# ViTAE-Transformer/SAMRS

Measured on AMD Instinct MI355X. Metric: images/sec (1024^2, vit_h, 32 boxes/img) SAM box->mask, higher is better.
Workload: dtype f16

## Files before the change

include/samrs_hip.h:

```cpp
#ifndef SAMRS_HIP_H
#define SAMRS_HIP_H

#include <stdint.h>

#ifdef __cplusplus
extern "C" {
#endif

#define SAMRS_ABI_VERSION 5

enum samrs_status {
    SAMRS_OK = 0,
    SAMRS_ERR_NOT_SET = -1,
    SAMRS_ERR_BAD_SHAPE = -2,
    SAMRS_ERR_BAD_ARG = -3,
    SAMRS_ERR_HIP = -4,
    SAMRS_ERR_BAD_WEIGHTS = -5,
    SAMRS_ERR_CAPACITY = -6,
    SAMRS_ERR_PRECISION = -7,
    SAMRS_ERR_RANGE = -8
};

enum samrs_precision {
    SAMRS_PREC_BF16 = 0,
    SAMRS_PREC_F16 = 1
};

typedef struct samrs_config {
    int32_t embed_dim;
    int32_t depth;
    int32_t num_heads;
    int32_t n_global;
    int32_t global_attn_indexes[8];
    int32_t img_size;
    int32_t patch_size;
    int32_t window_size;
    int32_t out_chans;
    int32_t max_images;
    int32_t max_prompts;
    int32_t max_points;
    int32_t precision;
} samrs_config;

typedef struct samrs_engine samrs_engine_t;

samrs_engine_t* samrs_create(const samrs_config* cfg, int device, char* err, int err_len);
void samrs_destroy(samrs_engine_t* e);
const char* samrs_last_error(const samrs_engine_t* e);
int samrs_abi_version(void);

int samrs_load_weight(samrs_engine_t* e, const char* name, const float* host_data,
                      const int64_t* shape, int ndim);
int samrs_finalize_weights(samrs_engine_t* e, void* stream);

int samrs_set_images(samrs_engine_t* e, const uint8_t* images, int n_images, int in_h, int in_w,
                     int slot0, void* stream);
int samrs_set_images_ragged(samrs_engine_t* e, const uint8_t* const* images, const int* in_h,
                            const int* in_w, int n_images, int slot0, void* stream);
int samrs_get_embedding(samrs_engine_t* e, int slot, float* out_chw, void* stream);
int samrs_set_embedding(samrs_engine_t* e, int slot, const float* emb_chw, void* stream);
int samrs_reset_image(samrs_engine_t* e, int slot);
int samrs_get_slot_info(const samrs_engine_t* e, int slot, int32_t* is_set, int32_t* split, int32_t* split_depth);

int samrs_predict(samrs_engine_t* e, int slot, int n_prompts,
                  const float* boxes, const float* point_coords, const int32_t* point_labels,
                  int n_points, const float* mask_input, int multimask, int return_logits,
                  int in_h, int in_w, int orig_h, int orig_w,
                  void* masks_out, float* iou_out, float* lowres_out, void* stream);

int samrs_predict_multi(samrs_engine_t* e, int n_images, const int* slots, const int* prompt_offsets,
                        const float* boxes, const float* point_coords, const int32_t* point_labels, int n_points,
                        const float* mask_input, int multimask, int return_logits,
                        const int* in_hw, const int* orig_hw, void* const* masks_out, float* iou_out, float* lowres_out,
                        void* stream);

int samrs_paint(samrs_engine_t* e, const uint8_t* masks, const int32_t* labels, int n,
                int orig_h, int orig_w, uint8_t* seg_mask, int64_t* areas_out,
                int64_t* class_pixels, int64_t* class_instances, int n_classes, void* stream);

int samrs_select_best(samrs_engine_t* e, const uint8_t* masks, const float* iou, int n, int n_sel, int h, int w,
                      uint8_t* best_out, float* quality_out, int64_t* areas_out, void* stream);

int samrs_gt_match(samrs_engine_t* e, const uint8_t* masks, int n, int h, int w, const uint8_t* label_rgb,
                   const uint8_t* colors, int64_t* inter_out, int64_t* gt_area_out, uint8_t* gt_masks_out, void* stream);

int samrs_rle_encode(samrs_engine_t* e, const uint8_t* masks, int n, int h, int w, uint8_t* out, int64_t out_capacity,
                     int64_t* cursor, int64_t* table, void* stream);

int samrs_scene_claim(samrs_engine_t* e, const uint8_t* masks, const int32_t* ranks, const int32_t* labels, int n, int h, int w,
                      int x0, int y0, int H, int W, int32_t* order, int64_t* areas_out,
                      int64_t* class_pixels, int64_t* class_instances, int n_classes, void* stream);
int samrs_scene_resolve(samrs_engine_t* e, const int32_t* order, const int32_t* labels_by_rank, int n_ranks, int H, int W,
                        uint8_t* seg, void* stream);
int samrs_rle_encode_placed(samrs_engine_t* e, const uint8_t* masks, int n, int h, int w, int x0, int y0, int H, int W,
                            uint8_t* out, int64_t out_capacity, int64_t* cursor, int64_t* table, void* stream);

enum samrs_region_mode { SAMRS_REGION_HOLES = 1, SAMRS_REGION_ISLANDS = 2, SAMRS_REGION_BOTH = 3 };
int samrs_clean_masks(samrs_engine_t* e, uint8_t* masks, int n, int h, int w, int min_area, int mode,
                      int64_t* areas_out, int64_t* changed_out, void* stream);

int samrs_png_encode_labels(samrs_engine_t* e, const uint8_t* maps, int n, int h, int w, const uint8_t* lut, uint8_t* out,
                            int64_t out_capacity, int64_t* cursor, int64_t* table, void* stream);

int samrs_resample_pass_u8(const uint8_t* in, uint8_t* out, const int32_t* bounds, const int32_t* coef,
                           int ksize, int in_len, int out_len, int other, int horizontal, void* stream);

int samrs_set_option(samrs_engine_t* e, const char* name, int value);
int samrs_get_option(const samrs_engine_t* e, const char* name, int* value);

int samrs_audit_site_count(const samrs_engine_t* e, int* n_sites);
int samrs_audit_site_name(const samrs_engine_t* e, int site, char* name, int name_len, int* columns);
int samrs_audit_read_profile(samrs_engine_t* e, int64_t* rows, int reset);
int samrs_audit_read_columns(samrs_engine_t* e, int site, double* sumsq, float* max_abs, int64_t* n_rows);

int samrs_rbox_mask_prompt(const int32_t* pts, int n, int n_vertices, int h, int w, int th, int tw,
                           int img_size, int out_size, float* out, void* stream);
enum samrs_fill_rule { SAMRS_FILL_CV2_LE_451 = 0, SAMRS_FILL_CV2_GE_452 = 1 };
int samrs_rbox_mask_prompt_rule(const int32_t* pts, int n, int n_vertices, int h, int w, int th, int tw,
                                int img_size, int out_size, int fill_rule, float* out, void* stream);


#ifdef __cplusplus
}
#endif
#endif
```

include/samrs_hip_internal.h:

```cpp
#ifndef SAMRS_HIP_INTERNAL_H
#define SAMRS_HIP_INTERNAL_H

#include "samrs_hip.h"

#ifdef __cplusplus
extern "C" {
#endif

int samrs_debug_encoder_prefix(samrs_engine_t* e, const uint8_t* images, int n_images, int in_h,
                               int in_w, int n_blocks, float* x_out, void* stream);

int samrs_debug_outlier_columns(samrs_engine_t* e, int block, int gemm, int32_t* out32);

void samrs_debug_set_gemm_variant(int variant);
void samrs_debug_set_gemm_skew(int xcd_units, int cu_units);
int samrs_debug_has_experiments(void);

int samrs_debug_copy_buffer(samrs_engine_t* e, const char* name, void* dst, size_t bytes, void* stream);

int samrs_debug_time_dominant_kernel(samrs_engine_t* e, int enable);
int samrs_debug_dominant_kernel_time(samrs_engine_t* e, float* avg_ms, int* launches, int* M, int* N, int* K);

int samrs_k_gemm(int prec, const void* A_et, const void* B_et, void* C, const float* bias,
                 const float* add2d, int add2d_period, int M, int N, int K,
                 int out_f32, int gelu, int accumulate, void* stream);
int samrs_k_gemm_f32(const float* A, int lda, const float* W, const float* bias, float* C, int ldc,
                     int M, int N, int K, int relu, int accumulate, void* stream);
int samrs_k_gemm_stats(int prec, const void* A_et, const void* B_et, float* C, const float* bias, void* xh_et, float* stats,
                       int M, int N, int K, void* stream);
int samrs_k_ln_rowstat(const float* stats, float* rowstat, int rows, float eps, void* stream);
int samrs_k_gemm_fold(int prec, const void* xh_et, const void* Wf_et, void* C_et, const float* bias_f, const float* cvec,
                      const float* rowstat, int M, int N, int K, int gelu, void* stream);
int samrs_k_ln_fold_weight(int prec, const float* W, const float* gamma, const float* beta, const float* bias, void* Wf_et,
                           float* cvec, float* bias_f, int N, int K, void* stream);
int samrs_k_rowstats_convert(int prec, const float* X, void* xh_et, float* stats, int rows, int D, void* stream);
int samrs_k_convert(int prec, const float* in, void* out_et, int64_t n, void* stream);
int samrs_k_layernorm(int prec, const float* X, const float* gamma, const float* beta, float eps,
                      void* out_et, float* out_f32, int rows_out, int D, int window_mode,
                      int n_images, int grid, int window, void* stream);
int samrs_k_window_attention(int prec, const void* qkv_et, const float* qkv_bias, const float* rel_h,
                             const float* rel_w, void* out_et, int n_images, int grid, int window,
                             int heads, int head_dim, void* stream);
int samrs_k_global_attention(int prec, const void* qkv_et, const float* rel_h, const float* rel_w,
                             void* out_et, int n_images, int grid, int heads, int head_dim,
                             void* stream);
int samrs_k_neck_im2col(const void* in_et, void* A_et, int n_images, int grid, int C, void* stream);
int samrs_k_postprocess(const float* lowres, int n_masks, int in_h, int in_w, int orig_h,
                        int orig_w, int img_size, int return_logits, void* out, void* stream);
int samrs_k_gemm_gln(int prec, const void* A_et, const void* B_et, void* C_et, const float* bias,
                     const float* gamma_beta, int M, int N, int K, const void* A_lo_et, const void* B_lo_et, void* stream);
int samrs_k_gemm_split3(int prec, const void* A_et, const void* A_lo_et, const void* B_et, const void* B_lo_et, void* C,
                        const float* bias, int M, int N, int K, int out_f32, int accumulate, int split_from_n, void* stream);
int samrs_k_upscale2_masks(int prec, const void* u1, const void* w_et, const void* w_lo_et, const float* bias,
                           const float* hyper, float* low, int n, int grid, int n_mask_tokens,
                           int sel0, int n_sel, void* stream);
int samrs_k_upscaler_fused(int prec, const void* keys_et, const void* keys_lo_et, const void* w1_et, const void* w1_lo_et,
                           const float* b1, const float* ln, const void* w2_et, const void* w2_lo_et, const float* b2,
                           const float* hyper, float* low, int n, int grid, int n_mask_tokens, int sel0, int n_sel, void* stream);
int samrs_k_prompt_tokens(const float* boxes, const float* point_coords, const int32_t* point_labels, int n_prompts, int n_points,
                          float img_size, const float* gauss, const float* point_emb, const float* not_a_point, const float* iou_token,
                          const float* mask_tokens, float* tokens, float* tokens2, int T, void* stream);
int samrs_k_dense_pe(const float* gauss, float* pe, int grid, void* stream);
int samrs_k_mask_embed(const float* w0, const float* b0, const float* ln1w, const float* ln1b, const float* w3, const float* b3,
                       const float* ln4w, const float* ln4b, const float* w6, const float* b6, const float* mask_in, float* dense,
                       int n, int grid, void* stream);
int samrs_k_fill_slot_table(const int32_t* start_host, const int32_t* slot_host, int n_runs, int32_t* out, void* stream);
int samrs_k_make_keys(int prec, const float* emb, const float* dense, const float* vec, float* out_f32, void* out_et, int n_batches,
                      int tokens, int C, const int32_t* slot_of, void* stream);
int samrs_k_token_self_attn(const float* q, const float* k, const float* v, float* o, int n, int T, int C, int heads, void* stream);
int64_t samrs_k_t2i_workspace_floats(int n, int T);
int samrs_k_t2i_attention(int prec, const float* qp, const void* kp_et, const void* vp_et, int ld, int64_t bstride, float* out,
                          float* workspace, int n, int T, int tokens, int Ci, int heads, const int32_t* slot_of, void* stream);
int samrs_k_i2t_attention(int prec, const void* qi_et, int ld, int64_t bstride, const float* kt, const float* vt, void* out_et, int n,
                          int T, int tokens, int Ci, int heads, void* stream);
int samrs_k_i2t_fused(int prec, const void* qi_et, int ld, int64_t q_bstride, const float* kt, const float* vt, const void* w_et,
                      const void* w_lo_et, const float* bias, const float* resid, int64_t r_bstride, const float* gamma,
                      const float* beta, float eps, float* outF, void* outE, void* outE_lo, int n, int T, int tokens, int Ci, int C,
                      const int32_t* slot_of, void* stream);
int samrs_k_group_ln_gelu(int prec, const float* in, const float* gamma, const float* beta, float eps, void* out_et, int64_t rows,
                          int groups, int gsize, void* stream);
int samrs_k_mask_product(int prec, const void* up2_et, const float* hyper, float* low, int n, int grid, int n_mask_tokens, int sel0,
                         int n_sel, void* stream);
int samrs_k_attention_mx(int prec, int global, const void* qkv_et, const float* qkv_bias, const float* rel_h, const float* rel_w,
                         void* out_et, void* out_lo_et, int n_images, int grid, int heads, int head_dim, void* q_hi, void* q_lo,
                         void* s_hi, void* s_lo, void* stream);
int64_t samrs_k_mx_scale_bytes(int rows, int Kp, int is_b);
int samrs_k_layernorm_mx(int prec, const float* X, const float* gamma, const float* beta, float eps, void* out_et, int rows, int D,
                         void* q_hi, void* q_lo, void* s_hi, void* s_lo, void* stream);
int samrs_k_mx4_pack(int prec, const float* x, const void* hi_in, const void* lo_in, void* out_hi, void* q_hi, void* q_lo, void* s_hi,
                     void* s_lo, int rows, int K, int G, int GP, int is_b, void* stream);
int samrs_k_gemm_mx(int prec, const void* A, const void* B, void* C, const float* bias, int M, int N, int K, int Kp, const void* a4_lo,
                    const void* a4_hi, const void* sa_lo, const void* sa_hi, const void* b4_hi, const void* b4_lo, const void* sb_hi,
                    const void* sb_lo, int out_f32, int accumulate, int split_from_n, void* stream);
int samrs_k_gemm_mx_gelu_mxout(int prec, const void* A, const void* B, void* C_et, const float* bias, int M, int N, int K, int Kp,
                               const void* a4_lo, const void* a4_hi, const void* sa_lo, const void* sa_hi, const void* b4_hi, const void* b4_lo,
                               const void* sb_hi, const void* sb_lo, int gelu, void* o4_hi, void* o4_lo, void* so_hi, void* so_lo, void* stream);
int samrs_k_convert_split(int prec, const float* in, void* out_hi_et, void* out_lo_et, int64_t n, void* stream);
int samrs_k_range_profile(int prec, const void* x_et, long n, int cols, int ld, int64_t* row48, void* stream);
int samrs_k_column_stats(int prec, const void* x_et, int M, int K, int ld, float* partials, double* sumsq, uint32_t* maxbits, void* stream);
int samrs_k_audit_rows_per_partial(void);
int samrs_k_region_labels(const uint8_t* masks, int n, int h, int w, int complement, int32_t* labels_out, void* stream);

#ifdef __cplusplus
}
#endif
#endif
```

samrs_amd/csrc/decoder_kernels.hip:

```cpp
#include "common.h"
#include "kernels.h"

namespace {

constexpr float TWO_PI = 6.283185307179586f;

__device__ __forceinline__ float pe_channel(const float* __restrict__ gauss, float cx01, float cy01, int ch, int half) {
    const int f = ch < half ? ch : ch - half;
    const float vx = 2.0f * cx01 - 1.0f, vy = 2.0f * cy01 - 1.0f;
    const float a = TWO_PI * (vx * gauss[f] + vy * gauss[half + f]);
    return ch < half ? sinf(a) : cosf(a);
}

__global__ void prompt_tokens_kernel(PromptParams p, float* __restrict__ tokens, float* __restrict__ tokens2, int T, int C) {
    const int j = blockIdx.x, b = blockIdx.y, ch = threadIdx.x;
    const int half = C / 2;
    const bool has_pts = p.point_coords != nullptr;
    const bool has_box = p.boxes != nullptr;
    const int npt = has_pts ? p.n_points + (has_box ? 0 : 1) : 0;
    float v;
    if (j == 0) {
        v = p.iou_token[ch];
    } else if (j < 5) {
        v = p.mask_tokens[(j - 1) * C + ch];
    } else if (j < 5 + npt) {
        const int k = j - 5;
        int label = -1;
        float x = 0.f, y = 0.f;
        if (k < p.n_points) {
            label = p.point_labels[b * p.n_points + k];
            x = p.point_coords[(b * p.n_points + k) * 2 + 0] + 0.5f;
            y = p.point_coords[(b * p.n_points + k) * 2 + 1] + 0.5f;
        }
        if (label == -1) {
            v = p.not_a_point[ch];
        } else {
            v = pe_channel(p.gauss, x / p.img_size, y / p.img_size, ch, half);
            if (label == 0) v += p.point_emb[0][ch];
            else if (label == 1) v += p.point_emb[1][ch];
        }
    } else {
        const int corner = j - 5 - npt;
        const float x = p.boxes[b * 4 + 2 * corner + 0] + 0.5f;
        const float y = p.boxes[b * 4 + 2 * corner + 1] + 0.5f;
        v = pe_channel(p.gauss, x / p.img_size, y / p.img_size, ch, half) + p.point_emb[2 + corner][ch];
    }
    tokens[((size_t)b * T + j) * C + ch] = v;
    if (tokens2) tokens2[((size_t)b * T + j) * C + ch] = v;
}

__global__ void dense_pe_kernel(const float* __restrict__ gauss, float* __restrict__ pe, int g, int C) {
    const int t = blockIdx.x, ch = threadIdx.x;
    const int y = t / g, x = t % g;
    pe[(size_t)t * C + ch] = pe_channel(gauss, ((float)x + 0.5f) / (float)g, ((float)y + 0.5f) / (float)g, ch, C / 2);
}

__global__ __launch_bounds__(256) void mask_embed_kernel(MaskEmbedParams p, const float* __restrict__ mask_in,
                                                         float* __restrict__ dense, int grid) {
    __shared__ float act2[16][16];
    const int t = threadIdx.x;
    const int b = blockIdx.y;
    const int tok0 = blockIdx.x * 16;
    {
        const int tl = t >> 4, c2 = t & 15;
        const int tok = tok0 + tl;
        const int ty = tok / grid, tx = tok % grid;
        const int S = 4 * grid;
        const float* in = mask_in + (size_t)b * S * S + (size_t)(4 * ty) * S + 4 * tx;
        float out2 = p.b3[c2];
#pragma unroll
        for (int sy = 0; sy < 2; ++sy)
#pragma unroll
            for (int sx = 0; sx < 2; ++sx) {
                float a[4];
                float mean = 0.f;
#pragma unroll
                for (int c = 0; c < 4; ++c) {
                    float s = p.b0[c];
#pragma unroll
                    for (int ky = 0; ky < 2; ++ky)
#pragma unroll
                        for (int kx = 0; kx < 2; ++kx)
// ... 154 lines not shown
        const int key_ = (k0_) + 4 * u_ + kq;                                                    \
        dk_[u_] = dv_[u_] = make_uint4(0u, 0u, 0u, 0u);                                          \
        if (key_ < kend) {                                                                       \
            dk_[u_] = *reinterpret_cast<const uint4*>(kb + (size_t)key_ * ld);                   \
            dv_[u_] = *reinterpret_cast<const uint4*>(vb + (size_t)key_ * ld);                   \
        }                                                                                        \
    }
    T2I_LOAD(kk, vv, kbeg)
    for (int k0 = kbeg; k0 < kend; k0 += 4 * U) {
        T2I_LOAD(kn, vn, k0 + 4 * U)
#pragma unroll
        for (int u = 0; u < U; ++u) {
            const bool valid = k0 + 4 * u + kq < kend;
            const uint32_t kw[4] = {kk[u].x, kk[u].y, kk[u].z, kk[u].w};
            const uint32_t vw[4] = {vv[u].x, vv[u].y, vv[u].z, vv[u].w};
            float kf[8], vf[8];
#pragma unroll
            for (int c = 0; c < 4; ++c) {
                kf[2 * c] = ET<PREC>::to_float((uint16_t)(kw[c] & 0xffffu));
                kf[2 * c + 1] = ET<PREC>::to_float((uint16_t)(kw[c] >> 16));
                vf[2 * c] = ET<PREC>::to_float((uint16_t)(vw[c] & 0xffffu));
                vf[2 * c + 1] = ET<PREC>::to_float((uint16_t)(vw[c] >> 16));
            }
#pragma unroll
            for (int t = 0; t < T2I_TG; ++t) {
                float sc = 0.f;
#pragma unroll
                for (int c = 0; c < 8; ++c) sc += q[t][c] * kf[c];
                sc += __builtin_bit_cast(float, __builtin_amdgcn_update_dpp(0, __builtin_bit_cast(int, sc), 0xB1, 0xF, 0xF, true));
                sc = valid ? sc : T2I_NEG;
                const float mn = fmaxf(m[t], sc);
                const float corr = __builtin_amdgcn_exp2f(m[t] - mn);
                const float pj = valid ? __builtin_amdgcn_exp2f(sc - mn) : 0.f;
                l[t] = l[t] * corr + pj;
#pragma unroll
                for (int c = 0; c < 8; ++c) acc[t][c] = acc[t][c] * corr + pj * vf[c];
                m[t] = mn;
            }
        }
#pragma unroll
        for (int u = 0; u < U; ++u) { kk[u] = kn[u]; vv[u] = vn[u]; }
    }
#undef T2I_LOAD
#pragma unroll
    for (int off = 16; off <= 32; off <<= 1) {
#pragma unroll
        for (int t = 0; t < T2I_TG; ++t) {
            const float mo = __shfl_xor(m[t], off, 64), lo = __shfl_xor(l[t], off, 64);
            const float mn = fmaxf(m[t], mo);
            const float fs = __builtin_amdgcn_exp2f(m[t] - mn), fo = __builtin_amdgcn_exp2f(mo - mn);
            l[t] = l[t] * fs + lo * fo;
#pragma unroll
            for (int c = 0; c < 8; ++c) acc[t][c] = acc[t][c] * fs + __shfl_xor(acc[t][c], off, 64) * fo;
            m[t] = mn;
        }
    }
    if (lane < 16) {
#pragma unroll
        for (int t = 0; t < T2I_TG; ++t) {
            float* r = sm[wave][t][ch];
            r[0] = m[t]; r[1] = l[t];
#pragma unroll
            for (int c = 0; c < 8; ++c) r[2 + c] = acc[t][c];
        }
    }
    __syncthreads();
    if (threadIdx.x < T2I_TG * 16) {
        const int t = threadIdx.x >> 4, c16 = threadIdx.x & 15;
        float mm = sm[0][t][c16][0];
#pragma unroll
        for (int w = 1; w < 4; ++w) mm = fmaxf(mm, sm[w][t][c16][0]);
        float ll = 0.f, a[8] = {0.f, 0.f, 0.f, 0.f, 0.f, 0.f, 0.f, 0.f};
#pragma unroll
        for (int w = 0; w < 4; ++w) {
            const float f = __builtin_amdgcn_exp2f(sm[w][t][c16][0] - mm);
            ll += sm[w][t][c16][1] * f;
#pragma unroll
            for (int c = 0; c < 8; ++c) a[c] += sm[w][t][c16][2 + c] * f;
        }
        float* r = part + ((((size_t)b * gridDim.z + blockIdx.z) * gridDim.x + split) * (T2I_TG * 16) + threadIdx.x) * T2I_REC;
        r[0] = mm; r[1] = ll;
#pragma unroll
        for (int c = 0; c < 8; ++c) r[2 + c] = a[c];
    }
}

__global__ __launch_bounds__(T2I_TG * 16) void t2i_merge_kernel(const float* __restrict__ part, float* __restrict__ o,
                                                                int splits, int T, int Ci) {
    const int b = blockIdx.x, tg = blockIdx.y;
    const int t = tg * T2I_TG + (threadIdx.x >> 4), ch = threadIdx.x & 15;
    if (t >= T) return;
    const float* base = part + (((size_t)b * gridDim.y + tg) * splits * (T2I_TG * 16) + threadIdx.x) * T2I_REC;
    const size_t sstride = (size_t)(T2I_TG * 16) * T2I_REC;
    float mm = T2I_NEG;
    for (int s = 0; s < splits; ++s) mm = fmaxf(mm, base[s * sstride]);
    float ll = 0.f, a[8] = {0.f, 0.f, 0.f, 0.f, 0.f, 0.f, 0.f, 0.f};
    for (int s = 0; s < splits; ++s) {
        const float* r = base + s * sstride;
        const float f = __builtin_amdgcn_exp2f(r[0] - mm);
        ll += r[1] * f;
#pragma unroll
        for (int c = 0; c < 8; ++c) a[c] += r[2 + c] * f;
    }
    const float inv = 1.0f / ll;
    float* orow = o + ((size_t)b * T + t) * Ci + ch * 8;
#pragma unroll
    for (int c = 0; c < 8; ++c) orow[c] = a[c] * inv;
}

constexpr int I2T_HS = 20;
template <int PREC>
__global__ __launch_bounds__(256) void i2t_attention_kernel(const uint16_t* __restrict__ qi, int ld, long bstride,
                                                            const float* __restrict__ kt, const float* __restrict__ vt,
                                                            uint16_t* __restrict__ out, int T, int tokens, int Ci) {
    constexpr int HD = 16;
    extern __shared__ float sm[];
    const int heads = Ci / HD;
    const int RS = heads * I2T_HS;
    float* sk = sm;
    float* sv = sm + T * RS;
    const int b = blockIdx.y;
    for (int i = threadIdx.x; i < T * Ci; i += 256) {
        const int j = i / Ci, c = i % Ci;
        sk[j * RS + (c / HD) * I2T_HS + c % HD] = kt[(size_t)b * T * Ci + i];
        sv[j * RS + (c / HD) * I2T_HS + c % HD] = vt[(size_t)b * T * Ci + i];
    }
    __syncthreads();
    const int tok = blockIdx.x * (256 / heads) + threadIdx.x / heads;
    const int h = threadIdx.x % heads;
    if (tok >= tokens) return;
    const uint16_t* qrow = qi + ((size_t)b * bstride + tok) * ld + h * HD;
    const uint4 q0 = *reinterpret_cast<const uint4*>(qrow);
    const uint4 q1 = *reinterpret_cast<const uint4*>(qrow + 8);
    const uint32_t qw[8] = {q0.x, q0.y, q0.z, q0.w, q1.x, q1.y, q1.z, q1.w};
    float qf[HD];
#pragma unroll
    for (int c = 0; c < 8; ++c) {
        qf[2 * c] = ET<PREC>::to_float((uint16_t)(qw[c] & 0xffffu)) * 0.25f;
        qf[2 * c + 1] = ET<PREC>::to_float((uint16_t)(qw[c] >> 16)) * 0.25f;
    }
    float m = -INFINITY, l = 0.f, acc[HD];
#pragma unroll
    for (int c = 0; c < HD; ++c) acc[c] = 0.f;
    for (int j = 0; j < T; ++j) {
        float kr[HD], vr[HD];
#pragma unroll
        for (int c4 = 0; c4 < HD / 4; ++c4) {
            const float4 k4 = *reinterpret_cast<const float4*>(sk + j * RS + h * I2T_HS + 4 * c4);
            const float4 v4 = *reinterpret_cast<const float4*>(sv + j * RS + h * I2T_HS + 4 * c4);
            kr[4 * c4] = k4.x; kr[4 * c4 + 1] = k4.y; kr[4 * c4 + 2] = k4.z; kr[4 * c4 + 3] = k4.w;
            vr[4 * c4] = v4.x; vr[4 * c4 + 1] = v4.y; vr[4 * c4 + 2] = v4.z; vr[4 * c4 + 3] = v4.w;
        }
        float s = 0.f;
#pragma unroll
        for (int c = 0; c < HD; ++c) s += qf[c] * kr[c];
        const float mn = fmaxf(m, s);
        const float corr = __expf(m - mn), pj = __expf(s - mn);
        l = l * corr + pj;
#pragma unroll
        for (int c = 0; c < HD; ++c) acc[c] = acc[c] * corr + pj * vr[c];
        m = mn;
    }
    const float inv = 1.0f / l;
    uint4 o0, o1;
    o0.x = pack2<PREC>(acc[0] * inv, acc[1] * inv);   o0.y = pack2<PREC>(acc[2] * inv, acc[3] * inv);
    o0.z = pack2<PREC>(acc[4] * inv, acc[5] * inv);   o0.w = pack2<PREC>(acc[6] * inv, acc[7] * inv);
// ... 294 lines not shown
    for (int g = 0; g < U2_GROUPS_PER_WAVE; ++g) {
        uint4 c0 = a0, c1 = a1, l0 = make_uint4(0u, 0u, 0u, 0u), l1 = l0;
        if constexpr (SPLIT) {
            split2_pack<PREC>(f[0].x, f[0].y, c0.x, l0.x); split2_pack<PREC>(f[0].z, f[0].w, c0.y, l0.y);
            split2_pack<PREC>(f[1].x, f[1].y, c0.z, l0.z); split2_pack<PREC>(f[1].z, f[1].w, c0.w, l0.w);
            split2_pack<PREC>(f[2].x, f[2].y, c1.x, l1.x); split2_pack<PREC>(f[2].z, f[2].w, c1.y, l1.y);
            split2_pack<PREC>(f[3].x, f[3].y, c1.z, l1.z); split2_pack<PREC>(f[3].z, f[3].w, c1.w, l1.w);
        }
        if (g + 1 < U2_GROUPS_PER_WAVE) {
            if constexpr (SPLIT) {
                const float* nb = fbase + (size_t)(g + 1) * 16 * 64;
                f[0] = *reinterpret_cast<const float4*>(nb); f[1] = *reinterpret_cast<const float4*>(nb + 4);
                f[2] = *reinterpret_cast<const float4*>(nb + 32); f[3] = *reinterpret_cast<const float4*>(nb + 36);
            } else {
                a0 = *reinterpret_cast<const uint4*>(abase + (size_t)(g + 1) * 16 * 64);
                a1 = *reinterpret_cast<const uint4*>(abase + (size_t)(g + 1) * 16 * 64 + 32);
            }
        }
        float part[NSEL][4];
#pragma unroll
        for (int c = 0; c < NSEL; ++c)
#pragma unroll
            for (int q = 0; q < 4; ++q) part[c][q] = 0.f;
#pragma unroll
        for (int i = 0; i < 8; ++i) {
            f32x4_t acc = {0.f, 0.f, 0.f, 0.f};
            if constexpr (SPLIT) {
                acc = ET<PREC>::mfma16(wf[i][0], l0, acc);
                acc = ET<PREC>::mfma16(wf[i][1], l1, acc);
                acc = ET<PREC>::mfma16(wl[i][0], c0, acc);
                acc = ET<PREC>::mfma16(wl[i][1], c1, acc);
            }
            acc = ET<PREC>::mfma16(wf[i][0], c0, acc);
            acc = ET<PREC>::mfma16(wf[i][1], c1, acc);
            const float2_t g01 = gelu_erf2(float2_t{acc[0] + bv[i][0], acc[1] + bv[i][1]});
            const float2_t g23 = gelu_erf2(float2_t{acc[2] + bv[i][2], acc[3] + bv[i][3]});
#pragma unroll
            for (int c = 0; c < NSEL; ++c) {
                const float* h = hy[c] + (i & 1) * 4;
                part[c][i >> 1] += h[0] * g01.x + h[1] * g01.y + h[2] * g23.x + h[3] * g23.y;
            }
        }
        const int row = row0 + g * 16 + fr;
        const int t = row >> 2, s1 = row & 3;
        const int y = t / grid, x = t % grid;
        const int Y = 4 * y + 2 * (s1 >> 1) + (fq >> 1), X = 4 * x + 2 * (s1 & 1) + (fq & 1);
#pragma unroll
        for (int c = 0; c < NSEL; ++c) {
            float mine = 0.f;
#pragma unroll
            for (int q = 0; q < 4; ++q) {
                float v = part[c][q];
                v += __shfl_xor(v, 16, 64);
                v += __shfl_xor(v, 32, 64);
                mine = (q == fq) ? v : mine;
            }
            low[(((size_t)b * NSEL + c) * S + Y) * S + X] = mine;
        }
    }
}

struct Lin {
    int i0, i1;
    float w0, w1;
};
__device__ __forceinline__ Lin lin_coord(int dst, float scale, int in_size) {
    float src = scale * ((float)dst + 0.5f) - 0.5f;
    src = src < 0.f ? 0.f : src;
    Lin r;
    r.i0 = (int)src;
    r.i0 = r.i0 < in_size - 1 ? r.i0 : in_size - 1;
    r.i1 = r.i0 + (r.i0 < in_size - 1 ? 1 : 0);
    r.w1 = src - (float)r.i0;
    r.w0 = 1.0f - r.w1;
    return r;
}
__device__ __forceinline__ float stage1(const float* __restrict__ low, int LS, float s1, int Y1, int X1) {
    const Lin ly = lin_coord(Y1, s1, LS), lx = lin_coord(X1, s1, LS);
    const float* r0 = low + (size_t)ly.i0 * LS;
    const float* r1 = low + (size_t)ly.i1 * LS;
    return ly.w0 * (lx.w0 * r0[lx.i0] + lx.w1 * r0[lx.i1]) + ly.w1 * (lx.w0 * r1[lx.i0] + lx.w1 * r1[lx.i1]);
}

__global__ __launch_bounds__(256) void postprocess_kernel(const float* __restrict__ low_all, int LS, int in_h, int in_w,
                                                          int H, int W, int img_size, int return_logits,
                                                          void* __restrict__ out) {
    const int W4 = (W + 3) / 4;
    const long t = (long)blockIdx.x * 256 + threadIdx.x;
    if (t >= (long)W4 * H) return;
    const int Y = (int)(t / W4), X0 = (int)(t % W4) * 4;
    const int mi = blockIdx.y;
    const float* low = low_all + (size_t)mi * LS * LS;
    const float s1 = (float)LS / (float)img_size;
    const bool identity = (H == in_h) && (W == in_w);
    float v[4];
    if (identity && 4 * LS == img_size && X0 + 3 < W) {
        const Lin ly = lin_coord(Y, s1, LS);
        const float* r0 = low + (size_t)ly.i0 * LS;
        const float* r1 = low + (size_t)ly.i1 * LS;
        const Lin la = lin_coord(X0, s1, LS), lb = lin_coord(X0 + 1, s1, LS), lc = lin_coord(X0 + 2, s1, LS), ld = lin_coord(X0 + 3, s1, LS);
        const float a00 = r0[la.i0], a01 = r0[la.i1], a10 = r1[la.i0], a11 = r1[la.i1];
        const float c00 = r0[lc.i0], c01 = r0[lc.i1], c10 = r1[lc.i0], c11 = r1[lc.i1];
        v[0] = ly.w0 * (la.w0 * a00 + la.w1 * a01) + ly.w1 * (la.w0 * a10 + la.w1 * a11);
        v[1] = ly.w0 * (lb.w0 * a00 + lb.w1 * a01) + ly.w1 * (lb.w0 * a10 + lb.w1 * a11);
        v[2] = ly.w0 * (lc.w0 * c00 + lc.w1 * c01) + ly.w1 * (lc.w0 * c10 + lc.w1 * c11);
        v[3] = ly.w0 * (ld.w0 * c00 + ld.w1 * c01) + ly.w1 * (ld.w0 * c10 + ld.w1 * c11);
    } else if (identity) {
#pragma unroll
        for (int e = 0; e < 4; ++e) v[e] = (X0 + e < W) ? stage1(low, LS, s1, Y, X0 + e) : 0.f;
    } else {
        const float sy = (float)in_h / (float)H, sx = (float)in_w / (float)W;
        const Lin ly = lin_coord(Y, sy, in_h);
#pragma unroll
        for (int e = 0; e < 4; ++e) {
            if (X0 + e < W) {
                const Lin lx = lin_coord(X0 + e, sx, in_w);
                const float a = lx.w0 * stage1(low, LS, s1, ly.i0, lx.i0) + lx.w1 * stage1(low, LS, s1, ly.i0, lx.i1);
                const float b = lx.w0 * stage1(low, LS, s1, ly.i1, lx.i0) + lx.w1 * stage1(low, LS, s1, ly.i1, lx.i1);
                v[e] = ly.w0 * a + ly.w1 * b;
            } else {
                v[e] = 0.f;
            }
        }
    }
    const size_t obase = ((size_t)mi * H + Y) * W + X0;
    if (return_logits) {
        float* o = reinterpret_cast<float*>(out) + obase;
        for (int e = 0; e < 4 && X0 + e < W; ++e) o[e] = v[e];
    } else {
        uint8_t* o = reinterpret_cast<uint8_t*>(out) + obase;
        if ((W & 3) == 0) {
            const uint32_t pk = (v[0] > 0.f ? 1u : 0u) | (v[1] > 0.f ? 1u << 8 : 0u) | (v[2] > 0.f ? 1u << 16 : 0u) |
                                (v[3] > 0.f ? 1u << 24 : 0u);
            *reinterpret_cast<uint32_t*>(o) = pk;
        } else {
            for (int e = 0; e < 4 && X0 + e < W; ++e) o[e] = v[e] > 0.f ? 1 : 0;
        }
    }
}

__global__ void paint_kernel(const uint8_t* __restrict__ masks, const int32_t* __restrict__ labels, int n, long hw,
                             uint8_t* __restrict__ seg) {
    const long p = (long)blockIdx.x * blockDim.x + threadIdx.x;
    if (p >= hw) return;
    for (int j = n - 1; j >= 0; --j) {
        if (masks[(size_t)j * hw + p]) {
            seg[p] = (uint8_t)labels[j];
            return;
        }
    }
}
__global__ void area_kernel(const uint8_t* __restrict__ masks, long hw, unsigned long long* __restrict__ areas) {
    const int j = blockIdx.y;
    const uint8_t* m = masks + (size_t)j * hw;
    unsigned int cnt = 0;
    for (long p = (long)blockIdx.x * blockDim.x + threadIdx.x; p < hw; p += (long)gridDim.x * blockDim.x) cnt += m[p] ? 1u : 0u;
    float c = (float)cnt;
    c = wave_sum(c);
    if ((threadIdx.x & 63) == 0 && c > 0.f) atomicAdd(&areas[j], (unsigned long long)c);
}
constexpr int PA_CHUNK = 64;
__device__ __forceinline__ uint32_t nonzero_bytes(uint32_t w) {
    return (((w & 0x7F7F7F7Fu) + 0x7F7F7F7Fu) | w) & 0x80808080u;
}
__global__ __launch_bounds__(256) void paint_area_kernel(const uint8_t* __restrict__ masks, const int32_t* __restrict__ labels,
                                                         int n, long hw, uint8_t* __restrict__ seg,
                                                         unsigned long long* __restrict__ areas) {
    __shared__ unsigned int cnt_s[PA_CHUNK];
    const long p0 = ((long)blockIdx.x * 256 + threadIdx.x) * 16;
    const bool in = p0 < hw;
    uint32_t done[4] = {0u, 0u, 0u, 0u}, res[4] = {0u, 0u, 0u, 0u};
    for (int jhi = n; jhi > 0; jhi -= PA_CHUNK) {
        const int jlo = jhi > PA_CHUNK ? jhi - PA_CHUNK : 0;
        if (threadIdx.x < PA_CHUNK) cnt_s[threadIdx.x] = 0u;
        __syncthreads();
        for (int j = jhi - 1; j >= jlo; --j) {
            unsigned int cnt = 0;
            if (in) {
                const uint4 m = *reinterpret_cast<const uint4*>(masks + (size_t)j * hw + p0);
                const uint32_t w[4] = {m.x, m.y, m.z, m.w};
                const uint32_t lab = (uint32_t)(uint8_t)labels[j] * 0x01010101u;
#pragma unroll
                for (int k = 0; k < 4; ++k) {
                    const uint32_t t = nonzero_bytes(w[k]);
                    cnt += __popc(t);
                    const uint32_t mm = (t >> 7) * 0xFFu, fresh = mm & ~done[k];
                    res[k] = (res[k] & ~fresh) | (fresh & lab);
                    done[k] |= mm;
                }
            }
            float c = wave_sum((float)cnt);
            if ((threadIdx.x & 63) == 0 && c > 0.f) atomicAdd(&cnt_s[j - jlo], (unsigned int)c);
        }
        __syncthreads();
        if (threadIdx.x < jhi - jlo && cnt_s[threadIdx.x]) atomicAdd(&areas[jlo + threadIdx.x], (unsigned long long)cnt_s[threadIdx.x]);
        __syncthreads();
    }
    if (in && (done[0] | done[1] | done[2] | done[3])) {
        uint4* sp = reinterpret_cast<uint4*>(seg + p0);
        uint4 o = *sp;
        o.x = (o.x & ~done[0]) | res[0]; o.y = (o.y & ~done[1]) | res[1];
        o.z = (o.z & ~done[2]) | res[2]; o.w = (o.w & ~done[3]) | res[3];
        *sp = o;
    }
}
__global__ __launch_bounds__(256) void select_best_kernel(const uint8_t* __restrict__ masks, const float* __restrict__ iou, int nsel,
                                                          long hw, uint8_t* __restrict__ out, float* __restrict__ quality,
                                                          unsigned long long* __restrict__ areas) {
    const int j = blockIdx.y;
    int best = 0;
    float bq = iou[(size_t)j * nsel];
    for (int c = 1; c < nsel; ++c) {
        const float q = iou[(size_t)j * nsel + c];
        if (q > bq) { bq = q; best = c; }
    }
    if (blockIdx.x == 0 && threadIdx.x == 0) quality[j] = bq;
    const uint8_t* src = masks + ((size_t)j * nsel + best) * hw;
    uint8_t* dst = out + (size_t)j * hw;
    unsigned int cnt = 0;
    const bool vec = (hw % 16 == 0) && ((((uintptr_t)src) | ((uintptr_t)dst)) & 15) == 0;
    if (vec) {
        const long n16 = hw / 16;
        for (long i = (long)blockIdx.x * 256 + threadIdx.x; i < n16; i += (long)gridDim.x * 256) {
            const uint4 m = reinterpret_cast<const uint4*>(src)[i];
            reinterpret_cast<uint4*>(dst)[i] = m;
            cnt += __popc(nonzero_bytes(m.x)) + __popc(nonzero_bytes(m.y)) + __popc(nonzero_bytes(m.z)) + __popc(nonzero_bytes(m.w));
        }
    } else {
        for (long i = (long)blockIdx.x * 256 + threadIdx.x; i < hw; i += (long)gridDim.x * 256) {
            const uint8_t m = src[i];
            dst[i] = m;
            cnt += m ? 1u : 0u;
        }
    }
    const float c = wave_sum((float)cnt);
    if ((threadIdx.x & 63) == 0 && c > 0.f) atomicAdd(&areas[j], (unsigned long long)c);
}

constexpr int GM_CHUNK = 64;
__global__ __launch_bounds__(256) void gt_match_kernel(const uint8_t* __restrict__ masks, int n, long hw,
                                                       const uint8_t* __restrict__ label_rgb, const uint8_t* __restrict__ colors,
                                                       unsigned long long* __restrict__ inter, unsigned long long* __restrict__ gt_area,
                                                       uint8_t* __restrict__ gt_masks) {
    __shared__ unsigned int cnt_s[GM_CHUNK];
    const long p0 = ((long)blockIdx.x * 256 + threadIdx.x) * 16;
    const bool full = p0 + 16 <= hw;
    uint32_t key[16];
    if (full && (((uintptr_t)(label_rgb + p0 * 3)) & 15) == 0) {
        const uint4* lp = reinterpret_cast<const uint4*>(label_rgb + p0 * 3);
        const uint4 a = lp[0], b = lp[1], c = lp[2];
        const uint32_t wv[12] = {a.x, a.y, a.z, a.w, b.x, b.y, b.z, b.w, c.x, c.y, c.z, c.w};
#pragma unroll
        for (int k = 0; k < 16; ++k) {
            uint32_t v = 0;
#pragma unroll
            for (int ch = 0; ch < 3; ++ch) {
                const int byte = 3 * k + ch;
                v |= ((wv[byte >> 2] >> (8 * (byte & 3))) & 0xFFu) << (8 * ch);
            }
            key[k] = v;
        }
    } else {
#pragma unroll
        for (int k = 0; k < 16; ++k) {
            const long p = p0 + k;
            key[k] = p < hw ? (uint32_t)label_rgb[p * 3] | ((uint32_t)label_rgb[p * 3 + 1] << 8) | ((uint32_t)label_rgb[p * 3 + 2] << 16)
                            : 0xFFFFFFFFu;
        }
    }
    for (int jlo = 0; jlo < n; jlo += GM_CHUNK) {
        const int jhi = jlo + GM_CHUNK < n ? jlo + GM_CHUNK : n;
        if (threadIdx.x < GM_CHUNK) cnt_s[threadIdx.x] = 0u;
        __syncthreads();
        for (int j = jlo; j < jhi; ++j) {
            const uint32_t want = (uint32_t)colors[3 * j] | ((uint32_t)colors[3 * j + 1] << 8) | ((uint32_t)colors[3 * j + 2] << 16);
// ... 170 lines not shown
            if (Y >= th || X >= tw) { pv[a][c] = -1000.0; continue; }
            const RTap ay = rbox_tap(Y, h, th), ax = rbox_tap(X, w, tw);
            const double m00 = rbox_inside(P, ax.i0, ay.i0) ? 1000.0 : -1000.0;
            const double m01 = rbox_inside(P, ax.i1, ay.i0) ? 1000.0 : -1000.0;
            const double m10 = rbox_inside(P, ax.i0, ay.i1) ? 1000.0 : -1000.0;
            const double m11 = rbox_inside(P, ax.i1, ay.i1) ? 1000.0 : -1000.0;
            const double r0 = m00 * (double)ax.w0 + m01 * (double)ax.w1;
            const double r1 = m10 * (double)ax.w0 + m11 * (double)ax.w1;
            pv[a][c] = r0 * (double)ay.w0 + r1 * (double)ay.w1;
        }
    const double t0 = pv[0][0] * (double)bx.w0 + pv[0][1] * (double)bx.w1;
    const double t1 = pv[1][0] * (double)bx.w0 + pv[1][1] * (double)bx.w1;
    out[(size_t)b * out_size * out_size + pix] = (float)(t0 * (double)by.w0 + t1 * (double)by.w1);
}

}

hipError_t launch_resample_pass(const uint8_t* in, uint8_t* out, const int32_t* bounds, const int32_t* coef, int ksize,
                                int in_len, int out_len, int other, int horizontal, hipStream_t s) {
    const long total = (long)out_len * other * 3;
    resample_pass_kernel<<<(int)((total + 255) / 256), 256, 0, s>>>(in, out, bounds, coef, ksize, in_len, out_len, other, horizontal);
    return hipGetLastError();
}

hipError_t launch_prompt_tokens(const PromptParams& p, float* tokens, float* tokens2, int T, hipStream_t s) {
    dim3 g(T, p.n_prompts), b(256);
    prompt_tokens_kernel<<<g, b, 0, s>>>(p, tokens, tokens2, T, 256);
    return hipGetLastError();
}
hipError_t launch_dense_pe(const float* gauss, float* pe, int grid, hipStream_t s) {
    dense_pe_kernel<<<grid * grid, 256, 0, s>>>(gauss, pe, grid, 256);
    return hipGetLastError();
}
hipError_t launch_mask_embed(const MaskEmbedParams& p, const float* mask_in, float* dense, int n, int grid, hipStream_t s) {
    dim3 g(grid * grid / 16, n);
    mask_embed_kernel<<<g, 256, 0, s>>>(p, mask_in, dense, grid);
    return hipGetLastError();
}
hipError_t launch_fill_slot_table(const int* start, const int* slot, int n_runs, int* out, hipStream_t s) {
    for (int k0 = 0; k0 < n_runs; k0 += SLOT_RUNS_MAX) {
        SlotRuns r{};
        const int nr = n_runs - k0 < SLOT_RUNS_MAX ? n_runs - k0 : SLOT_RUNS_MAX;
        for (int k = 0; k < nr; ++k) { r.start[k] = start[k0 + k]; r.slot[k] = slot[k0 + k]; }
        r.start[nr] = start[k0 + nr];
        fill_slot_table_kernel<<<nr, 64, 0, s>>>(r, out);
    }
    return hipGetLastError();
}
hipError_t launch_make_keys(int prec, const float* emb, const float* dense, const float* vec, float* out_f32,
                            void* out_et, int n_batches, int tokens, int C, hipStream_t s, const int* slot_of) {
    const long per4 = (long)tokens * C / 4, tot4 = per4 * n_batches;
    const int blocks = (int)((tot4 + 255) / 256);
    if (prec == PREC_BF16)
        make_keys_kernel<PREC_BF16><<<blocks, 256, 0, s>>>(emb, slot_of, dense, vec, out_f32, (uint16_t*)out_et, per4, tot4, C / 4);
    else
        make_keys_kernel<PREC_F16><<<blocks, 256, 0, s>>>(emb, slot_of, dense, vec, out_f32, (uint16_t*)out_et, per4, tot4, C / 4);
    return hipGetLastError();
}
hipError_t launch_add_f32(const float* a, const float* b, float* out, long n, hipStream_t s) {
    if (n % 4) return hipErrorInvalidValue;
    add_f32_kernel<<<(int)((n / 4 + 255) / 256), 256, 0, s>>>(a, b, out, n / 4);
    return hipGetLastError();
}
hipError_t launch_token_self_attn(const float* q, const float* k, const float* v, float* o, int n, int T, int C,
                                  int heads, hipStream_t s) {
    if (C / heads != 32 || T > TOK_MAX) return hipErrorInvalidValue;
    token_self_attn_kernel<32><<<n, 256, 3 * T * C * sizeof(float), s>>>(q, k, v, o, T, C, heads);
    return hipGetLastError();
}
size_t t2i_workspace_floats(int n, int T) {
    return (size_t)n * ((T + T2I_TG - 1) / T2I_TG) * T2I_MAX_SPLITS * (T2I_TG * 16) * T2I_REC;
}
hipError_t launch_t2i_attention(int prec, const float* qp, const void* kp, const void* vp, int ld, long bstride,
                                float* o, float* workspace, int n, int T, int tokens, int Ci, int heads, hipStream_t s,
                                const int* slot_of) {
    if (Ci != 128 || heads != 8 || T > TOK_MAX || !workspace) return hipErrorInvalidValue;
    int splits = (tokens + 255) / 256;
    splits = splits < 1 ? 1 : (splits > T2I_MAX_SPLITS ? T2I_MAX_SPLITS : splits);
    const int kpw = ((tokens + splits * 4 - 1) / (splits * 4) + 15) / 16 * 16;
    const int tgs = (T + T2I_TG - 1) / T2I_TG;
    dim3 g(splits, n, tgs), b(256);
    const uint16_t* k = (const uint16_t*)kp;
    const uint16_t* v = (const uint16_t*)vp;
    if (prec == PREC_BF16) t2i_partial_kernel<PREC_BF16><<<g, b, 0, s>>>(qp, k, v, ld, bstride, slot_of, workspace, T, tokens, Ci, kpw);
    else t2i_partial_kernel<PREC_F16><<<g, b, 0, s>>>(qp, k, v, ld, bstride, slot_of, workspace, T, tokens, Ci, kpw);
    t2i_merge_kernel<<<dim3(n, tgs), T2I_TG * 16, 0, s>>>(workspace, o, splits, T, Ci);
    return hipGetLastError();
}
hipError_t launch_i2t_attention(int prec, const void* qi, int ld, long bstride, const float* kt, const float* vt,
                                void* out, int n, int T, int tokens, int Ci, int heads, hipStream_t s) {
    if (Ci / heads != 16 || 256 % heads) return hipErrorInvalidValue;
    const int per = 256 / heads;
    dim3 g((tokens + per - 1) / per, n), b(256);
    const size_t sh = 2 * (size_t)T * heads * I2T_HS * sizeof(float);
    if (prec == PREC_BF16)
        i2t_attention_kernel<PREC_BF16><<<g, b, sh, s>>>((const uint16_t*)qi, ld, bstride, kt, vt, (uint16_t*)out, T, tokens, Ci);
    else
        i2t_attention_kernel<PREC_F16><<<g, b, sh, s>>>((const uint16_t*)qi, ld, bstride, kt, vt, (uint16_t*)out, T, tokens, Ci);
    return hipGetLastError();
}
hipError_t launch_i2t_fused(int prec, const void* qi, int ld, long q_bstride, const float* kt, const float* vt, const void* w,
                            const void* w_lo, const float* bias, const float* resid, long r_bstride, const float* gamma,
                            const float* beta, float eps, float* outF, void* outE, void* outE_lo, int n, int T, int tokens, int Ci,
                            int C, hipStream_t s, const int* slot_of) {
    if (Ci != 128 || C != 256 || T < 1 || T > TOK_MAX || tokens % I2TF_ROWS) return hipErrorInvalidValue;
    const int groups = tokens / I2TF_ROWS;
    int gpb = 4;
    while (gpb > 1 && groups % gpb) gpb >>= 1;
    dim3 g(groups / gpb, n), b(256);
    const bool split = w_lo != nullptr;
    const size_t sh = (size_t)(2 * T * 8 * I2T_HS + 3 * 256 + 2 * 4 * I2TF_ROWS) * sizeof(float) +
                      (size_t)(split ? 2 : 1) * I2TF_ROWS * I2TF_AST * 2;
#define I2TF_LAUNCH(P, S)                                                                                                       \
    i2t_fused_kernel<P, S><<<g, b, sh, s>>>((const uint16_t*)qi, ld, q_bstride, slot_of, kt, vt, (const uint16_t*)w, (const uint16_t*)w_lo, \
                                           bias, resid, r_bstride, gamma, beta, eps, outF, (uint16_t*)outE, (uint16_t*)outE_lo, T, \
                                           tokens, gpb)
    if (prec == PREC_BF16) { if (split) I2TF_LAUNCH(PREC_BF16, true); else I2TF_LAUNCH(PREC_BF16, false); }
    else { if (split) I2TF_LAUNCH(PREC_F16, true); else I2TF_LAUNCH(PREC_F16, false); }
#undef I2TF_LAUNCH
    return hipGetLastError();
}
hipError_t launch_group_ln_gelu(int prec, const float* in, const float* gamma, const float* beta, float eps,
                                void* out, long rows, int groups, int gsize, hipStream_t s) {
    if (groups != 4 || gsize != 64) return hipErrorInvalidValue;
    const int blocks = (int)((rows + 3) / 4);
    if (prec == PREC_BF16) group_ln_gelu_kernel<PREC_BF16><<<blocks, 256, 0, s>>>(in, gamma, beta, eps, (uint16_t*)out, rows);
    else group_ln_gelu_kernel<PREC_F16><<<blocks, 256, 0, s>>>(in, gamma, beta, eps, (uint16_t*)out, rows);
    return hipGetLastError();
}
hipError_t launch_mask_product(int prec, const void* up2, const float* hyper, float* low, int n, int grid,
                               int n_mask_tokens, int sel0, int n_sel, hipStream_t s) {
    if (n_sel > 4 || n_sel < 1) return hipErrorInvalidValue;
    const int S = 4 * grid;
    dim3 g(S * S / 256, n), b(256);
    if (prec == PREC_BF16) mask_product_kernel<PREC_BF16><<<g, b, 0, s>>>((const uint16_t*)up2, hyper, low, grid, n_mask_tokens, sel0, n_sel);
    else mask_product_kernel<PREC_F16><<<g, b, 0, s>>>((const uint16_t*)up2, hyper, low, grid, n_mask_tokens, sel0, n_sel);
    return hipGetLastError();
}
hipError_t launch_upscale2_masks(int prec, const void* u1, const void* w, const void* w_lo, const float* bias, const float* hyper,
                                 float* low, int n, int grid, int n_mask_tokens, int sel0, int n_sel, hipStream_t s) {
    const int rows_per_block = 4 * 16 * U2_GROUPS_PER_WAVE;
    if ((grid * grid * 4) % rows_per_block || (n_sel != 1 && n_sel != 3)) return hipErrorInvalidValue;
    dim3 g(grid * grid * 4 / rows_per_block, n), b(256);
    const uint16_t* ww = (const uint16_t*)w;
    const uint16_t* wl = (const uint16_t*)w_lo;
#define U2_LAUNCH(P, NS, SP) upscale2_mask_kernel<P, NS, SP><<<g, b, 0, s>>>(u1, ww, wl, bias, hyper, low, grid, n_mask_tokens, sel0)
#define U2_SEL(P, SP) do { if (n_sel == 1) U2_LAUNCH(P, 1, SP); else U2_LAUNCH(P, 3, SP); } while (0)
    if (prec == PREC_BF16) { if (w_lo) U2_SEL(PREC_BF16, true); else U2_SEL(PREC_BF16, false); }
    else { if (w_lo) U2_SEL(PREC_F16, true); else U2_SEL(PREC_F16, false); }
#undef U2_SEL
#undef U2_LAUNCH
    return hipGetLastError();
}
hipError_t launch_postprocess(const float* low, int n_masks, int in_h, int in_w, int orig_h, int orig_w,
                              int img_size, int return_logits, void* out, hipStream_t s) {
    const long work = (long)((orig_w + 3) / 4) * orig_h;
    dim3 g((unsigned)((work + 255) / 256), n_masks), b(256);
    postprocess_kernel<<<g, b, 0, s>>>(low, img_size / 4, in_h, in_w, orig_h, orig_w, img_size, return_logits, out);
    return hipGetLastError();
}
hipError_t launch_paint(const uint8_t* masks, const int32_t* labels, int n, int h, int w, uint8_t* seg,
                        unsigned long long* areas, unsigned long long* class_pixels,
                        unsigned long long* class_instances, int n_classes, hipStream_t s) {
    const long hw = (long)h * w;
    const bool fused = seg && areas && hw % 16 == 0 && (((uintptr_t)masks | (uintptr_t)seg) & 15) == 0;
    if (seg && !fused) paint_kernel<<<(int)((hw + 255) / 256), 256, 0, s>>>(masks, labels, n, hw, seg);
    if (areas) {
        HIP_CHECK_RET(hipMemsetAsync(areas, 0, sizeof(unsigned long long) * n, s));
        if (fused) {
            paint_area_kernel<<<(int)((hw / 16 + 255) / 256), 256, 0, s>>>(masks, labels, n, hw, seg, areas);
        } else {
            dim3 g(64, n);
            area_kernel<<<g, 256, 0, s>>>(masks, hw, areas);
        }
        if (class_pixels || class_instances)
            class_stats_kernel<<<1, 64, 0, s>>>(areas, labels, n, class_pixels, class_instances, n_classes);
    }
    return hipGetLastError();
}

hipError_t launch_select_best(const uint8_t* masks, const float* iou, int n, int nsel, int h, int w, uint8_t* out, float* quality,
                              unsigned long long* areas, hipStream_t s) {
    if (n < 1 || nsel < 1 || h < 1 || w < 1) return hipErrorInvalidValue;
    const long hw = (long)h * w;
    HIP_CHECK_RET(hipMemsetAsync(areas, 0, sizeof(unsigned long long) * n, s));
    int chunks = (int)((hw / 16 + 255) / 256);
    chunks = chunks < 1 ? 1 : (chunks > 64 ? 64 : chunks);
    select_best_kernel<<<dim3(chunks, n), 256, 0, s>>>(masks, iou, nsel, hw, out, quality, areas);
    return hipGetLastError();
}

hipError_t launch_gt_match(const uint8_t* masks, int n, int h, int w, const uint8_t* label_rgb, const uint8_t* colors,
                           unsigned long long* inter, unsigned long long* gt_area, uint8_t* gt_masks, hipStream_t s) {
    const long hw = (long)h * w;
    if (n < 1 || h < 1 || w < 1 || hw >= (1l << 30)) return hipErrorInvalidValue;
    HIP_CHECK_RET(hipMemsetAsync(inter, 0, sizeof(unsigned long long) * n, s));
    HIP_CHECK_RET(hipMemsetAsync(gt_area, 0, sizeof(unsigned long long) * n, s));
    const int blocks = (int)(((hw + 15) / 16 + 255) / 256);
    gt_match_kernel<<<blocks, 256, 0, s>>>(masks, n, hw, label_rgb, colors, inter, gt_area, gt_masks);
    return hipGetLastError();
}

hipError_t launch_rbox_prompt(const int32_t* pts, int n, int nv, int h, int w, int th, int tw, int img_size, int out_size,
                              float* out, hipStream_t s, int fill_rule) {
    if (n < 1 || nv < 3 || nv > RBOX_MAXV || h < 1 || w < 1 || th < 1 || tw < 1 || th > img_size || tw > img_size || out_size < 1 ||
        fill_rule < 0 || fill_rule > 1)
        return hipErrorInvalidValue;
    dim3 g((out_size * out_size + 255) / 256, n), b(256);
    rbox_prompt_kernel<<<g, b, 0, s>>>(pts, nv, h, w, th, tw, img_size, out_size, out, fill_rule);
    return hipGetLastError();
}
```

samrs_amd/csrc/engine.hip:

```cpp
#include <algorithm>
#include <cmath>
#include <cstdarg>
#include <cstdio>
#include <cstring>
#include <map>
#include <mutex>
#include <utility>
#include <cstdlib>
#include <string>
#include <vector>

#include "../../include/samrs_hip.h"
#include "../../include/samrs_hip_internal.h"
#include "common.h"
#include "kernels.h"

namespace {

struct DevTensor {
    float* p = nullptr;
    std::vector<int64_t> shape;
    size_t numel = 0;
};

// ... 1230 lines not shown
static int encode_stack(samrs_engine_t* e, const uint8_t* images, int n, int in_h, int in_w, int slot0, void* stream,
                        int n_blocks, bool do_neck) {
    if (!e || !images) return fail(e, SAMRS_ERR_BAD_ARG, "samrs_set_images: null argument");
    if (n < 1 || n > e->cfg.max_images) return fail(e, SAMRS_ERR_CAPACITY, "n_images/slot out of range (max_images=%d)", e->cfg.max_images);
    std::vector<const uint8_t*> ptr(n);
    std::vector<int> hs(n, in_h), ws(n, in_w);
    for (int i = 0; i < n; ++i) ptr[i] = images + (size_t)i * (in_h > 0 ? in_h : 0) * (in_w > 0 ? in_w : 0) * 3;
    return encode(e, ptr.data(), hs.data(), ws.data(), n, slot0, stream, n_blocks, do_neck);
}

int samrs_set_images(samrs_engine_t* e, const uint8_t* images, int n, int in_h, int in_w, int slot0, void* stream) {
    return encode_stack(e, images, n, in_h, in_w, slot0, stream, 1 << 30, true);
}

int samrs_set_images_ragged(samrs_engine_t* e, const uint8_t* const* images, const int* in_h, const int* in_w, int n,
                            int slot0, void* stream) {
    return encode(e, images, in_h, in_w, n, slot0, stream, 1 << 30, true);
}

int samrs_debug_encoder_prefix(samrs_engine_t* e, const uint8_t* images, int n, int in_h, int in_w, int n_blocks,
                               float* x_out, void* stream) {
    if (!x_out) return fail(e, SAMRS_ERR_BAD_ARG, "samrs_debug_encoder_prefix: null output");
    const int rc = encode_stack(e, images, n, in_h, in_w, 0, stream, n_blocks, false);
    if (rc) return rc;
    CK(e, hipMemcpyAsync(x_out, e->X, sizeof(float) * (size_t)n * e->tokens * e->D, hipMemcpyDeviceToDevice, (hipStream_t)stream));
    return SAMRS_OK;
}

int samrs_get_embedding(samrs_engine_t* e, int slot, float* out_chw, void* stream) {
    if (!e || !out_chw) return fail(e, SAMRS_ERR_BAD_ARG, "samrs_get_embedding: null argument");
    if (slot < 0 || slot >= e->cfg.max_images) return fail(e, SAMRS_ERR_CAPACITY, "slot out of range");
    if (!e->slot_set[slot]) return fail(e, SAMRS_ERR_NOT_SET, "An image must be set with .set_image(...) to generate an embedding.");
    ON_DEVICE(e);
    CK(e, launch_transpose_f32(e->EMB + (size_t)slot * e->tokens * e->C, out_chw, e->tokens, e->C, (hipStream_t)stream));
    return SAMRS_OK;
}

static int prepare_slot_keys(samrs_engine_t* e, int slot0, int n, hipStream_t s) {
    const int C = e->C, Ci = C / 2, tokens = e->tokens, prec = e->prec;
    const DecLayer& L = e->layers[0];
    for (int i = 0; i < n; ++i) {
        const size_t o = (size_t)(slot0 + i) * tokens * C;
        CK(e, launch_make_keys(prec, e->EMB + o, nullptr, W(e, "prompt_encoder.no_mask_embed.weight"), e->K0F + o, e->K0E + o, 1, tokens, C, s));
    }
    CK(e, launch_gemm_et(prec, e->K0E + (size_t)slot0 * tokens * C, L.kvq_w, e->KVQ0 + (size_t)slot0 * tokens * 3 * Ci, L.kvq_b, L.kvq_pe,
                         tokens, n * tokens, 3 * Ci, C, false, false, false, s));
    return SAMRS_OK;
}

int samrs_set_embedding(samrs_engine_t* e, int slot, const float* emb_chw, void* stream) {
    if (!e || !emb_chw) return fail(e, SAMRS_ERR_BAD_ARG, "samrs_set_embedding: null argument");
    if (!e->finalized) return fail(e, SAMRS_ERR_BAD_WEIGHTS, "weights not finalized");
    if (slot < 0 || slot >= e->cfg.max_images) return fail(e, SAMRS_ERR_CAPACITY, "slot out of range");
    ON_DEVICE(e);
    CK(e, launch_transpose_f32(emb_chw, e->EMB + (size_t)slot * e->tokens * e->C, e->C, e->tokens, (hipStream_t)stream));
    { const int rc = prepare_slot_keys(e, slot, 1, (hipStream_t)stream); if (rc != SAMRS_OK) return rc; }
    e->slot_set[slot] = 1;
    e->slot_split[slot] = -1;
    e->slot_depth[slot] = 0;
    return SAMRS_OK;
}

int samrs_get_slot_info(const samrs_engine_t* e, int slot, int32_t* is_set, int32_t* split, int32_t* split_depth) {
    if (!e) return SAMRS_ERR_BAD_ARG;
    if (slot < 0 || slot >= e->cfg.max_images) return SAMRS_ERR_CAPACITY;
    if (is_set) *is_set = e->slot_set[slot];
    if (split) *split = e->slot_set[slot] ? e->slot_split[slot] : 0;
    if (split_depth) *split_depth = e->slot_set[slot] ? e->slot_depth[slot] : 0;
    return SAMRS_OK;
}

int samrs_reset_image(samrs_engine_t* e, int slot) {
    if (!e) return SAMRS_ERR_BAD_ARG;
    if (slot < 0 || slot >= e->cfg.max_images) return fail(e, SAMRS_ERR_CAPACITY, "slot out of range");
    e->slot_set[slot] = 0;
    return SAMRS_OK;
}

struct PredictImage {
    int slot, p0, p1, in_h, in_w, orig_h, orig_w;
    void* masks;
};

static int predict_chunk(samrs_engine_t* e, const PredictImage* seg, int n_seg, int n, const float* boxes, const float* point_coords,
                         const int32_t* point_labels, int n_points, const float* mask_input, int multimask,
                         int return_logits, float* iou_out, float* lowres_out, void* stream);

static std::string slot_note(int slot) { return " (slot " + std::to_string(slot) + ")"; }

static int check_multimask_grade(samrs_engine_t* e, int slot, bool multi) {
    if (e->allow_reduced || !e->grade_multimask || slot < 0 || slot >= e->cfg.max_images || !e->slot_set[slot]) return SAMRS_OK;
    const int sm = e->slot_split[slot];
    const int need_depth = sm < 0 ? 0 : (sm & (SPLIT_ATTN | SPLIT_MLP | SPLIT_LIN2)) ? e->cfg.depth : (3 * e->cfg.depth + 3) / 4;
    if (sm >= 0 && (!(sm & e->grade_multimask) || e->slot_depth[slot] < need_depth ||
                    (e->split & (SPLIT_OI | SPLIT_UP)) != (SPLIT_OI | SPLIT_UP)))
        return fail(e, SAMRS_ERR_PRECISION, "multimask_output=True on an embedding encoded with split=%d over %d of %d blocks (decoder split=%d): "
                    "this model's multimask outputs need a block-GEMM split bit (64 or 16) at its automatic depth and the decoder "
                    "bits 4 | 8 to hold IoU >= 0.999; re-encode the image in the engine's default mode, or set option "
                    "\"allow_reduced\" = 1%s", sm, e->slot_depth[slot], need_depth, e->split, multi ? slot_note(slot).c_str() : "");
    return SAMRS_OK;
}

static int check_predict(samrs_engine_t* e, const PredictImage* im, int n_img, bool multi, const float* boxes, const float* point_coords,
                         const int32_t* point_labels, int n_points, const float* mask_input) {
    if (!e->finalized) return fail(e, SAMRS_ERR_BAD_WEIGHTS, "weights not finalized");
    const samrs_config& c = e->cfg;
    for (int i = 0; i < n_img; ++i) {
        const int slot = im[i].slot;
        if (slot < 0 || slot >= c.max_images)
            return multi ? fail(e, SAMRS_ERR_CAPACITY, "image %d: slot %d out of range (max_images=%d)", i, slot, c.max_images)
                         : fail(e, SAMRS_ERR_CAPACITY, "slot out of range");
        if (!e->slot_set[slot])
            return multi ? fail(e, SAMRS_ERR_NOT_SET, "An image must be set with .set_image(...) before mask prediction "
                                "(image %d: slot %d is not set).", i, slot)
                         : fail(e, SAMRS_ERR_NOT_SET, "An image must be set with .set_image(...) before mask prediction.");
    }
    if (!boxes && !point_coords && !mask_input) return fail(e, SAMRS_ERR_BAD_ARG, "at least one prompt (points, boxes or mask_input) is required");
    if (point_coords && !point_labels) return fail(e, SAMRS_ERR_BAD_ARG, "point_labels must be supplied if point_coords is supplied.");
    if (point_coords && (n_points < 1 || n_points > c.max_points)) return fail(e, SAMRS_ERR_CAPACITY, "n_points=%d exceeds max_points=%d", n_points, c.max_points);
    for (int i = 0; i < n_img; ++i)
        if (im[i].in_h < 1 || im[i].in_w < 1 || im[i].in_h > c.img_size || im[i].in_w > c.img_size || im[i].orig_h < 1 || im[i].orig_w < 1)
            return multi ? fail(e, SAMRS_ERR_BAD_SHAPE, "image %d: bad input/original size", i) : fail(e, SAMRS_ERR_BAD_SHAPE, "bad input/original size");
    return SAMRS_OK;
}

static int predict_images(samrs_engine_t* e, const PredictImage* im, int n_img, const float* boxes, const float* point_coords,
                          const int32_t* point_labels, int n_points, const float* mask_input, int multimask, int return_logits,
                          float* iou_out, float* lowres_out, void* stream) {
    const int cap = e->cfg.max_prompts;
    const size_t nsel = multimask ? 3 : 1;
    const int np = point_coords ? n_points : 0;
    const int n = n_img ? im[n_img - 1].p1 : 0;
    std::vector<PredictImage> seg;
    int first = 0;
    for (int off = 0; off < n; off += cap) {
        const int m = (n - off) < cap ? (n - off) : cap;
        seg.clear();
        for (int i = first; i < n_img && im[i].p0 < off + m; ++i) {
            const int a = im[i].p0 > off ? im[i].p0 : off, b = im[i].p1 < off + m ? im[i].p1 : off + m;
            if (b <= a) continue;
            PredictImage sgm = im[i];
            const size_t mask_stride = nsel * (size_t)im[i].orig_h * (size_t)im[i].orig_w * (return_logits ? 4 : 1);
            sgm.p0 = a - off; sgm.p1 = b - off;
            sgm.masks = im[i].masks ? (void*)((unsigned char*)im[i].masks + (size_t)(a - im[i].p0) * mask_stride) : nullptr;
            seg.push_back(sgm);
        }
        while (first < n_img && im[first].p1 <= off + m) ++first;
        const int rc = predict_chunk(
            e, seg.data(), (int)seg.size(), m, boxes ? boxes + (size_t)off * 4 : nullptr,
            point_coords ? point_coords + (size_t)off * np * 2 : nullptr, point_labels ? point_labels + (size_t)off * np : nullptr,
            n_points, mask_input ? mask_input + (size_t)off * 256 * 256 : nullptr, multimask, return_logits,
            iou_out ? iou_out + (size_t)off * nsel : nullptr, lowres_out ? lowres_out + (size_t)off * nsel * 256 * 256 : nullptr, stream);
        if (rc) return rc;
    }
    return SAMRS_OK;
}

int samrs_predict(samrs_engine_t* e, int slot, int n, const float* boxes, const float* point_coords,
                  const int32_t* point_labels, int n_points, const float* mask_input, int multimask,
                  int return_logits, int in_h, int in_w, int orig_h, int orig_w, void* masks_out, float* iou_out,
                  float* lowres_out, void* stream) {
    if (!e) return SAMRS_ERR_BAD_ARG;
    if (n < 1) return fail(e, SAMRS_ERR_BAD_ARG, "n_prompts must be >= 1");
    if (multimask) { const int rc = check_multimask_grade(e, slot, false); if (rc != SAMRS_OK) return rc; }
    const PredictImage im{slot, 0, n, in_h, in_w, orig_h, orig_w, masks_out};
    { const int rc = check_predict(e, &im, 1, false, boxes, point_coords, point_labels, n_points, mask_input); if (rc != SAMRS_OK) return rc; }
    return predict_images(e, &im, 1, boxes, point_coords, point_labels, n_points, mask_input, multimask, return_logits, iou_out,
                          lowres_out, stream);
}

int samrs_predict_multi(samrs_engine_t* e, int n_images, const int* slots, const int* prompt_offsets, const float* boxes,
                        const float* point_coords, const int32_t* point_labels, int n_points, const float* mask_input, int multimask,
                        int return_logits, const int* in_hw, const int* orig_hw, void* const* masks_out, float* iou_out,
                        float* lowres_out, void* stream) {
    if (!e) return SAMRS_ERR_BAD_ARG;
    if (n_images < 1 || !slots || !prompt_offsets || !in_hw || !orig_hw)
        return fail(e, SAMRS_ERR_BAD_ARG, "samrs_predict_multi: n_images must be >= 1 and slots, prompt_offsets, in_hw, orig_hw non-null");
    if (prompt_offsets[0] != 0) return fail(e, SAMRS_ERR_BAD_ARG, "samrs_predict_multi: prompt_offsets[0] must be 0, got %d", prompt_offsets[0]);
    std::vector<PredictImage> im((size_t)n_images);
    for (int i = 0; i < n_images; ++i) {
        if (prompt_offsets[i + 1] < prompt_offsets[i])
            return fail(e, SAMRS_ERR_BAD_ARG, "samrs_predict_multi: prompt_offsets must not decrease (image %d: %d -> %d)", i,
                        prompt_offsets[i], prompt_offsets[i + 1]);
        im[i] = PredictImage{slots[i], prompt_offsets[i], prompt_offsets[i + 1], in_hw[2 * i], in_hw[2 * i + 1], orig_hw[2 * i],
                             orig_hw[2 * i + 1], masks_out ? masks_out[i] : nullptr};
    }
    if (multimask)
        for (int i = 0; i < n_images; ++i) { const int rc = check_multimask_grade(e, slots[i], true); if (rc != SAMRS_OK) return rc; }
    { const int rc = check_predict(e, im.data(), n_images, true, boxes, point_coords, point_labels, n_points, mask_input); if (rc != SAMRS_OK) return rc; }
    return predict_images(e, im.data(), n_images, boxes, point_coords, point_labels, n_points, mask_input, multimask, return_logits,
                          iou_out, lowres_out, stream);
}

static int predict_chunk(samrs_engine_t* e, const PredictImage* seg, int n_seg, int n, const float* boxes, const float* point_coords,
                         const int32_t* point_labels, int n_points, const float* mask_input, int multimask,
                         int return_logits, float* iou_out, float* lowres_out, void* stream) {
    const samrs_config& c = e->cfg;
    if (n < 1 || n > c.max_prompts) return fail(e, SAMRS_ERR_CAPACITY, "n_prompts=%d exceeds max_prompts=%d", n, c.max_prompts);
    hipStream_t s = (hipStream_t)stream;
    ON_DEVICE(e);
    const int C = e->C, Ci = C / 2, tokens = e->tokens, prec = e->prec, g = e->grid;
    const int npt = point_coords ? n_points + (boxes ? 0 : 1) : 0;
    const int T = 5 + npt + (boxes ? 2 : 0);
    const int BT = n * T;
    const int Mi = n * tokens;
    auto lin = [&](const float* A, int lda, const float* Wt, const float* b, float* Cout, int ldc, int M, int N, int K,
                   bool relu, bool acc) { return launch_gemm_f32(A, lda, Wt, b, Cout, ldc, M, N, K, relu, acc, s); };
    auto lin2 = [&](const float* A, const float* A2, int lda, const float* Wt, const float* b, float* Cout, int ldc, int M,
                    int N, int K) {
        F32Batch bt{};
        bt.A[0] = A; bt.A2[0] = A2; bt.W[0] = Wt; bt.bias[0] = b; bt.C[0] = Cout;
        return launch_gemm_f32_batch(bt, 1, lda, ldc, M, N, K, false, false, s);
    };
    auto ln_tok = [&](const float* gw, const float* gb) {
        return launch_layernorm(prec, e->Q, gw, gb, 1e-5f, nullptr, e->Q, BT, C, 0, g, 0, s);
    };

    PromptParams pp{};
    pp.boxes = boxes; pp.point_coords = point_coords; pp.point_labels = point_labels;
    pp.n_prompts = n; pp.n_points = point_coords ? n_points : 0;
    pp.img_size = (float)c.img_size;
    pp.gauss = W(e, "prompt_encoder.pe_layer.positional_encoding_gaussian_matrix");
    for (int i = 0; i < 4; ++i) pp.point_emb[i] = W(e, "prompt_encoder.point_embeddings." + std::to_string(i) + ".weight");
    pp.not_a_point = W(e, "prompt_encoder.not_a_point_embed.weight");
    pp.iou_token = W(e, "mask_decoder.iou_token.weight");
    pp.mask_tokens = W(e, "mask_decoder.mask_tokens.weight");
    CK(e, launch_prompt_tokens(pp, e->TOK0, e->Q, T, s));

    const bool shared0 = (mask_input == nullptr);
    const int* slot_tab = nullptr;
    const size_t slot0 = n_seg == 1 ? (size_t)seg[0].slot : 0;
    if (n_seg > 1) {
        if (!e->SLOT_OF) CK(e, dalloc(e, &e->SLOT_OF, (size_t)c.max_prompts));
        std::vector<int> start((size_t)n_seg + 1), slot((size_t)n_seg);
        for (int k = 0; k < n_seg; ++k) { start[k] = seg[k].p0; slot[k] = seg[k].slot; }
        start[n_seg] = seg[n_seg - 1].p1;
        CK(e, launch_fill_slot_table(start.data(), slot.data(), n_seg, e->SLOT_OF, s));
        slot_tab = e->SLOT_OF;
    }
    const float* emb = e->EMB + slot0 * tokens * C;
    const float* k0f = e->K0F + slot0 * tokens * C;
    const uint16_t* kvq0 = e->KVQ0 + slot0 * tokens * 3 * Ci;
    if (!shared0) {
        if (!e->DENSE) CK(e, dalloc(e, &e->DENSE, (size_t)c.max_prompts * tokens * C));
        MaskEmbedParams mp{W(e, "prompt_encoder.mask_downscaling.0.weight"), W(e, "prompt_encoder.mask_downscaling.0.bias"),
                           W(e, "prompt_encoder.mask_downscaling.1.weight"), W(e, "prompt_encoder.mask_downscaling.1.bias"),
                           W(e, "prompt_encoder.mask_downscaling.3.weight"), W(e, "prompt_encoder.mask_downscaling.3.bias"),
                           W(e, "prompt_encoder.mask_downscaling.4.weight"), W(e, "prompt_encoder.mask_downscaling.4.bias"),
                           W(e, "prompt_encoder.mask_downscaling.6.weight"), W(e, "prompt_encoder.mask_downscaling.6.bias")};
        CK(e, launch_mask_embed(mp, mask_input, e->DENSE, n, g, s));
        CK(e, launch_make_keys(prec, emb, e->DENSE, nullptr, e->KF, e->KE, n, tokens, C, s, slot_tab));
    }

    for (int li = 0; li < 2; ++li) {
        const DecLayer& L = e->layers[li];
        const bool sh = shared0 && li == 0;
        {
            F32Batch bt{};
            const float* pe = li > 0 ? e->TOK0 : nullptr;
            bt.A[0] = e->Q; bt.A2[0] = pe; bt.W[0] = L.self.qw; bt.bias[0] = L.self.qb; bt.C[0] = e->TQ;
            bt.A[1] = e->Q; bt.A2[1] = pe; bt.W[1] = L.self.kw; bt.bias[1] = L.self.kb; bt.C[1] = e->TK;
            bt.A[2] = e->Q; bt.A2[2] = nullptr; bt.W[2] = L.self.vw; bt.bias[2] = L.self.vb; bt.C[2] = e->TV;
            CK(e, launch_gemm_f32_batch(bt, 3, C, C, BT, C, C, false, false, s));
        }
        CK(e, launch_token_self_attn(e->TQ, e->TK, e->TV, e->TO, n, T, C, 8, s));
        CK(e, lin(e->TO, C, L.self.ow, L.self.ob, e->Q, C, BT, C, C, false, li > 0));
        CK(e, ln_tok(L.n1w, L.n1b));
        const long bstride = sh && !slot_tab ? 0 : tokens;
        const int* tab = sh ? slot_tab : nullptr;
        const uint16_t* kvq = sh ? kvq0 : e->KVQ;
        if (!sh) CK(e, launch_gemm_et(prec, e->KE, L.kvq_w, e->KVQ, L.kvq_b, L.kvq_pe, tokens, Mi, 3 * Ci, C, false, false, false, s));
        CK(e, lin2(e->Q, e->TOK0, C, L.t2i.qw, L.t2i.qb, e->QP, Ci, BT, Ci, C));
        CK(e, launch_t2i_attention(prec, e->QP, kvq, kvq + Ci, 3 * Ci, bstride, e->O128, e->T2IW, n, T, tokens, Ci, 8, s, tab));
        CK(e, lin(e->O128, Ci, L.t2i.ow, L.t2i.ob, e->Q, C, BT, C, Ci, false, true));
        CK(e, ln_tok(L.n2w, L.n2b));
        CK(e, lin(e->Q, C, L.m1w, L.m1b, e->MH, 2048, BT, 2048, C, true, false));
        CK(e, lin(e->MH, 2048, L.m2w, L.m2b, e->Q, C, BT, C, 2048, false, true));
        CK(e, ln_tok(L.n3w, L.n3b));
        {
            F32Batch bt{};
            bt.A[0] = e->Q; bt.A2[0] = e->TOK0; bt.W[0] = L.i2t.kw; bt.bias[0] = L.i2t.kb; bt.C[0] = e->KT;
            bt.A[1] = e->Q; bt.A2[1] = nullptr; bt.W[1] = L.i2t.vw; bt.bias[1] = L.i2t.vb; bt.C[1] = e->VT;
            CK(e, launch_gemm_f32_batch(bt, 2, C, Ci, BT, Ci, C, false, false, s));
        }
        if (e->decoder_fusion && tokens % 32 == 0) {
            CK(e, launch_i2t_fused(prec, kvq + 2 * Ci, 3 * Ci, bstride, e->KT, e->VT, L.i2t_ow,
                                   (e->split & SPLIT_OI) ? L.i2t_ow_lo : nullptr, L.i2t.ob, sh ? k0f : e->KF,
                                   bstride, L.n4w, L.n4b, 1e-5f, li == 1 ? nullptr : e->KF, e->KE,
                                   (li == 1 && (e->split & SPLIT_UP)) ? e->KE_lo : nullptr, n, T, tokens, Ci, C, s, tab));
        } else if (tab) {
            for (int k = 0; k < n_seg; ++k) {
                const size_t p0 = (size_t)seg[k].p0, ns = (size_t)(seg[k].p1 - seg[k].p0), sl = (size_t)seg[k].slot;
                CK(e, launch_i2t_attention(prec, e->KVQ0 + sl * tokens * 3 * Ci + 2 * Ci, 3 * Ci, 0, e->KT + p0 * T * Ci,
                                           e->VT + p0 * T * Ci, e->OI + p0 * tokens * Ci, (int)ns, T, tokens, Ci, 8, s));
                CK(e, launch_gemm_et(prec, e->OI + p0 * tokens * Ci, L.i2t_ow, e->KF + p0 * tokens * C, L.i2t.ob,
                                     e->K0F + sl * tokens * C, tokens, (int)ns * tokens, C, Ci, true, false, false, s));
            }
            CK(e, launch_layernorm(prec, e->KF, L.n4w, L.n4b, 1e-5f, e->KE, e->KF, Mi, C, 0, g, 0, s));
        } else {
            CK(e, launch_i2t_attention(prec, kvq + 2 * Ci, 3 * Ci, bstride, e->KT, e->VT, e->OI, n, T, tokens, Ci, 8, s));
            if (sh)
                CK(e, launch_gemm_et(prec, e->OI, L.i2t_ow, e->KF, L.i2t.ob, k0f, tokens, Mi, C, Ci, true, false, false, s));
            else
                CK(e, launch_gemm_et(prec, e->OI, L.i2t_ow, e->KF, L.i2t.ob, nullptr, 0, Mi, C, Ci, true, false, true, s));
            CK(e, launch_layernorm(prec, e->KF, L.n4w, L.n4b, 1e-5f, e->KE, e->KF, Mi, C, 0, g, 0, s));
        }
    }
    CK(e, lin2(e->Q, e->TOK0, C, e->fin.qw, e->fin.qb, e->QP, Ci, BT, Ci, C));
    CK(e, launch_gemm_et(prec, e->KE, e->fin_kv_w, e->KVQ, e->fin_kv_b, e->fin_pe, tokens, Mi, 2 * Ci, C, false, false, false, s));
    CK(e, launch_t2i_attention(prec, e->QP, e->KVQ, e->KVQ + Ci, 2 * Ci, tokens, e->O128, e->T2IW, n, T, tokens, Ci, 8, s));
    CK(e, lin(e->O128, Ci, e->fin.ow, e->fin.ob, e->Q, C, BT, C, Ci, false, true));
    CK(e, ln_tok(W(e, "mask_decoder.transformer.norm_final_attn.weight"), W(e, "mask_decoder.transformer.norm_final_attn.bias")));

    {
        const std::string hp = "mask_decoder.output_hypernetworks_mlps.", ip = "mask_decoder.iou_prediction_head.layers";
        const size_t hs = (size_t)c.max_prompts * C;
        F32Batch l0{}, l1{}, l2{};
        for (int i = 0; i < 5; ++i) {
            const std::string p = i < 4 ? hp + std::to_string(i) + ".layers" : ip;
            l0.A[i] = i < 4 ? e->Q + (size_t)(1 + i) * C : e->Q;
            l0.W[i] = W(e, p + ".0.weight"); l0.bias[i] = W(e, p + ".0.bias"); l0.C[i] = e->HY1 + i * hs;
            l1.A[i] = e->HY1 + i * hs;
            l1.W[i] = W(e, p + ".1.weight"); l1.bias[i] = W(e, p + ".1.bias"); l1.C[i] = e->HY2 + i * hs;
            if (i < 4) {
                l2.A[i] = e->HY2 + i * hs;
                l2.W[i] = W(e, p + ".2.weight"); l2.bias[i] = W(e, p + ".2.bias"); l2.C[i] = e->HYPER + i * (C / 8);
            }
        }
        CK(e, launch_gemm_f32_batch(l0, 5, T * C, C, n, C, C, true, false, s));
        CK(e, launch_gemm_f32_batch(l1, 5, C, C, n, C, C, true, false, s));
        CK(e, launch_gemm_f32_batch(l2, 4, C, 4 * (C / 8), n, C / 8, C, false, false, s));
        if (iou_out) {
            const int s0 = multimask ? 1 : 0, ns = multimask ? 3 : 1;
            CK(e, lin(e->HY2 + 4 * hs, C, W(e, ip + ".2.weight") + (size_t)s0 * C, W(e, ip + ".2.bias") + s0, iou_out, ns, n, ns, C, false, false));
        }
    }
    const bool fuse = e->decoder_fusion;
    const bool sp_up = fuse && (e->split & SPLIT_UP) && tokens % 32 == 0;
    const int sel0 = multimask ? 1 : 0, nsel = multimask ? 3 : 1;
    float* low = lowres_out ? lowres_out : e->LOW;
    const bool one_kernel = fuse && e->upscaler_fused && g % 16 == 0;
    if (one_kernel) {
        CK(e, launch_upscaler_fused(prec, e->KE, sp_up ? e->KE_lo : nullptr, e->up1_w, sp_up ? e->up1_w_lo : nullptr, e->up1_b, e->up_ln,
                                    e->up2_w, sp_up ? e->up2_w_lo : nullptr, e->up2_b, e->HYPER, low, n, g, 4, sel0, nsel, s));
    } else if (sp_up && Mi % 256 == 0 && (g * g * 4) % 1024 == 0) {
        CK(e, launch_gemm_et_gln(prec, e->KE, e->up1_w, e->U1raw, e->up1_b, e->up_ln, Mi, C, C, s, e->KE_lo, e->up1_w_lo));
    } else if (fuse && Mi % 256 == 0) {
        CK(e, launch_gemm_et_gln(prec, e->KE, e->up1_w, e->U1, e->up1_b, e->up_ln, Mi, C, C, s));
    } else {
        CK(e, launch_gemm_et(prec, e->KE, e->up1_w, e->U1raw, e->up1_b, nullptr, 0, Mi, C, C, true, false, false, s));
        CK(e, launch_group_ln_gelu(prec, e->U1raw, W(e, "mask_decoder.output_upscaling.1.weight"),
                                   W(e, "mask_decoder.output_upscaling.1.bias"), 1e-6f, e->U1, (long)Mi, 4, C / 4, s));
    }
    if (one_kernel) {
    } else if (sp_up && Mi % 256 == 0 && (g * g * 4) % 1024 == 0) {
        CK(e, launch_upscale2_masks(prec, e->U1raw, e->up2_w, e->up2_w_lo, e->up2_b, e->HYPER, low, n, g, 4, sel0, nsel, s));
    } else if (fuse && (g * g * 4) % 1024 == 0) {
        CK(e, launch_upscale2_masks(prec, e->U1, e->up2_w, nullptr, e->up2_b, e->HYPER, low, n, g, 4, sel0, nsel, s));
    } else {
        CK(e, launch_gemm_et(prec, e->U1, e->up2_w, e->U2, e->up2_b, nullptr, 0, Mi * 4, C / 2, C / 4, false, true, false, s));
        CK(e, launch_mask_product(prec, e->U2, e->HYPER, low, n, g, 4, sel0, nsel, s));
    }
    for (int k = 0; k < n_seg; ++k)
        if (seg[k].masks)
            CK(e, launch_postprocess(low + (size_t)seg[k].p0 * nsel * 256 * 256, (seg[k].p1 - seg[k].p0) * nsel, seg[k].in_h, seg[k].in_w,
                                     seg[k].orig_h, seg[k].orig_w, c.img_size, return_logits, seg[k].masks, s));
    return SAMRS_OK;
}

int samrs_paint(samrs_engine_t* e, const uint8_t* masks, const int32_t* labels, int n, int h, int w, uint8_t* seg,
                int64_t* areas, int64_t* cpix, int64_t* cins, int n_classes, void* stream) {
    if (!e || !masks || !labels || n < 1 || h < 1 || w < 1) return fail(e, SAMRS_ERR_BAD_ARG, "samrs_paint: bad argument");
    if ((cpix || cins) && !areas) return fail(e, SAMRS_ERR_BAD_ARG, "samrs_paint: class statistics need areas_out");
    ON_DEVICE(e);
    CK(e, launch_paint(masks, labels, n, h, w, seg, (unsigned long long*)areas, (unsigned long long*)cpix,
                       (unsigned long long*)cins, n_classes, (hipStream_t)stream));
    return SAMRS_OK;
}

void samrs_debug_set_gemm_variant(int v) { set_gemm_variant(v); }
void samrs_debug_set_gemm_skew(int xcd_units, int cu_units) { set_gemm_skew(xcd_units, cu_units); }
int samrs_debug_has_experiments(void) { return gemm_has_experiments() ? 1 : 0; }
int samrs_select_best(samrs_engine_t* e, const uint8_t* masks, const float* iou, int n, int n_sel, int h, int w, uint8_t* best_out,
                      float* quality_out, int64_t* areas_out, void* stream) {
    if (!e || !masks || !iou || !best_out || !quality_out || !areas_out || n < 1 || n_sel < 1 || h < 1 || w < 1)
        return fail(e, SAMRS_ERR_BAD_ARG, "samrs_select_best: bad argument");
    ON_DEVICE(e);
    CK(e, launch_select_best(masks, iou, n, n_sel, h, w, best_out, quality_out, (unsigned long long*)areas_out, (hipStream_t)stream));
    return SAMRS_OK;
}
int samrs_gt_match(samrs_engine_t* e, const uint8_t* masks, int n, int h, int w, const uint8_t* label_rgb, const uint8_t* colors,
                   int64_t* inter_out, int64_t* gt_area_out, uint8_t* gt_masks_out, void* stream) {
    if (!e || !masks || !label_rgb || !colors || !inter_out || !gt_area_out || n < 1 || h < 1 || w < 1)
        return fail(e, SAMRS_ERR_BAD_ARG, "samrs_gt_match: bad argument");
    if ((long long)h * w >= (1ll << 30)) return fail(e, SAMRS_ERR_BAD_ARG, "samrs_gt_match: h * w = %lld must stay below 2^30", (long long)h * w);
    ON_DEVICE(e);
    CK(e, launch_gt_match(masks, n, h, w, label_rgb, colors, (unsigned long long*)inter_out, (unsigned long long*)gt_area_out, gt_masks_out,
                          (hipStream_t)stream));
    return SAMRS_OK;
}

int samrs_set_option(samrs_engine_t* e, const char* name, int value) {
    if (!e || !name) return SAMRS_ERR_BAD_ARG;
    const std::string n(name);
    if (n == "decoder_fusion") e->decoder_fusion = value != 0;
    else if (n == "ln_fold") {
        if (value && !gemm_has_experiments())
            return fail(e, SAMRS_ERR_BAD_ARG, "ln_fold: the folded LayerNorm (measured slower: DESIGN.md 6) is built with make EXPERIMENTS=1 only");
        e->ln_fold = value != 0;
    }
    else if (n == "split") {
        if (e->finalized && (value & (SPLIT_ATTN_ANY | SPLIT_MLP | SPLIT_LIN2) & ~e->split_ready))
            return fail(e, SAMRS_ERR_BAD_ARG, "split bits 16 / 32 / 64 / 128 (block GEMMs) need their lo weights: set them before the weights are "
                                              "finalized (SAMRS_SPLIT or options={'split': ...})");
        e->split = value & SPLIT_ALL;
    }
    else if (n == "gemm_variant") e->gemm_variant = value;
    else if (n == "upscaler_fused") e->upscaler_fused = value != 0;
    else if (n == "split_passes") e->split_passes = value != 0;
    else if (n == "split_depth") e->split_depth = value > 0 ? value : 0;
    else if (n == "allow_reduced") e->allow_reduced = value != 0;
    else if (n == "gelu_fast") e->gelu_fast = value < 0 ? -1 : (value != 0);
    else if (n == "ln_tail") e->ln_tail = value > 0;
    else if (n == "operand_pad") e->operand_pad_on = value != 0;
    else if (n == "outlier_cols") e->outlier_on = value & 7;
    else if (n == "outlier_ratio_pct") {
        if (e->finalized) return fail(e, SAMRS_ERR_BAD_ARG, "outlier_ratio_pct: the columns are picked when the weights are finalized; set it before");
        if (value < 101) return fail(e, SAMRS_ERR_BAD_ARG, "outlier_ratio_pct must exceed 100 (a column's score as a percentage of the median score)");
        e->outlier_ratio_pct = value;
    }
    else if (n == "range_check") {
        if (value < 0 || value > 2) return fail(e, SAMRS_ERR_BAD_ARG, "range_check is 0 (off), 1 (count) or 2 (count, and samrs_set_images fails)");
        if (value && !e->range_counter) {
            ON_DEVICE(e);
            CK(e, dalloc(e, &e->range_counter, 1));
            CK(e, hipMemset(e->range_counter, 0, sizeof(unsigned long long)));
        }
        if (value == 2 && e->range_check != 2 && e->range_counter) {
            ON_DEVICE(e);
            CK(e, hipDeviceSynchronize());
            CK(e, hipMemcpy(&e->range_seen, e->range_counter, sizeof(unsigned long long), hipMemcpyDeviceToHost));
        }
        e->range_check = value;
    }
    else if (n == "saturated") {
        if (e->range_counter) {
            ON_DEVICE(e);
            CK(e, hipDeviceSynchronize());
            CK(e, hipMemset(e->range_counter, 0, sizeof(unsigned long long)));
        }
        e->range_seen = 0;
    }
    else if (n == "range_profile") {
        if (value < 0 || value > 2) return fail(e, SAMRS_ERR_BAD_ARG, "range_profile is 0 (off), 1 (range profile per site) or 2 (and column statistics)");
        e->range_profile = value;
        if (!value) e->audit_passes = 0;
    }
    else if (n == "audit_passes") {
        if (value < 0) return fail(e, SAMRS_ERR_BAD_ARG, "audit_passes is the number of encoder passes to profile (0 stops a running audit)");
        if (value > 0) {
// ... 319 lines not shown
    if (b.oc_n[gemm] > 0) {
        ON_DEVICE(e);
        CK(e, hipMemcpy(out32, b.oc_idx[gemm], sizeof(int32_t) * b.oc_n[gemm], hipMemcpyDeviceToHost));
    }
    return b.oc_n[gemm];
}
int samrs_audit_site_count(const samrs_engine_t* e, int* n_sites) {
    if (!e || !n_sites) return SAMRS_ERR_BAD_ARG;
    *n_sites = (int)e->audit_sites.size();
    return SAMRS_OK;
}
int samrs_audit_site_name(const samrs_engine_t* e, int site, char* name, int name_len, int* columns) {
    if (!e || !name || name_len < 1 || site < 0 || site >= (int)e->audit_sites.size()) return SAMRS_ERR_BAD_ARG;
    snprintf(name, (size_t)name_len, "%s", e->audit_sites[site].name.c_str());
    if (columns) *columns = e->audit_sites[site].columns;
    return SAMRS_OK;
}
int samrs_audit_read_profile(samrs_engine_t* e, int64_t* rows, int reset) {
    if (!e || !rows) return fail(e, SAMRS_ERR_BAD_ARG, "samrs_audit_read_profile: null argument");
    const size_t n = e->audit_sites.size() * AUDIT_PROFILE_WORDS;
    if (!e->audit_rows) {
        for (size_t i = 0; i < n; ++i) rows[i] = 0;
        return SAMRS_OK;
    }
    ON_DEVICE(e);
    CK(e, hipDeviceSynchronize());
    CK(e, hipMemcpy(rows, e->audit_rows, n * sizeof(int64_t), hipMemcpyDeviceToHost));
    return reset ? audit_reset(e) : SAMRS_OK;
}
int samrs_audit_read_columns(samrs_engine_t* e, int site, double* sumsq, float* max_abs, int64_t* n_rows) {
    if (!e || !sumsq || !max_abs || !n_rows) return fail(e, SAMRS_ERR_BAD_ARG, "samrs_audit_read_columns: null argument");
    if (site < 0 || site >= (int)e->audit_sites.size()) return fail(e, SAMRS_ERR_BAD_ARG, "samrs_audit_read_columns: site %d of %d", site, (int)e->audit_sites.size());
    const samrs_engine::AuditSite& a = e->audit_sites[site];
    if (a.columns == 0)
        return fail(e, SAMRS_ERR_BAD_ARG, "samrs_audit_read_columns: site %s has no column statistics (the block GEMMs' A operands have: qkv_in, proj_in, lin1_in, lin2_in)", a.name.c_str());
    if (!e->audit_sumsq || e->audit_col_rows[site] == 0)
        return fail(e, SAMRS_ERR_BAD_ARG, "samrs_audit_read_columns: no encoder pass has been profiled with option \"range_profile\" = 2 (or \"audit_passes\") since the last reset");
    ON_DEVICE(e);
    CK(e, hipDeviceSynchronize());
    std::vector<uint32_t> bits((size_t)a.columns);
    CK(e, hipMemcpy(sumsq, e->audit_sumsq + a.col_off, sizeof(double) * a.columns, hipMemcpyDeviceToHost));
    CK(e, hipMemcpy(bits.data(), e->audit_maxbits + a.col_off, sizeof(uint32_t) * a.columns, hipMemcpyDeviceToHost));
    for (int c = 0; c < a.columns; ++c) {
        uint32_t u;
        if (e->prec == PREC_BF16) u = bits[c] << 16;
        else {
            const uint32_t ex = bits[c] >> 10, m = bits[c] & 0x3ffu;
            if (ex == 31) u = 0x7f800000u | (m << 13);
            else if (ex) u = ((ex + 112) << 23) | (m << 13);
            else { const float f = (float)m * 5.9604644775390625e-8f ; memcpy(&u, &f, 4); }
        }
        memcpy(&max_abs[c], &u, 4);
    }
    *n_rows = (int64_t)e->audit_col_rows[site];
    return SAMRS_OK;
}
int samrs_k_range_profile(int prec, const void* x, long n, int cols, int ld, int64_t* row48, void* stream) {
    if (!x || !row48 || n < 0) return SAMRS_ERR_BAD_ARG;
    KRET(launch_range_profile(prec, x, n, cols, ld, reinterpret_cast<long long*>(row48), (hipStream_t)stream));
}
int samrs_k_column_stats(int prec, const void* x, int M, int K, int ld, float* partials, double* sumsq, uint32_t* maxbits, void* stream) {
    if (!x || !partials || !sumsq || !maxbits) return SAMRS_ERR_BAD_ARG;
    KRET(launch_column_stats(prec, x, M, K, ld, partials, sumsq, maxbits, (hipStream_t)stream));
}
int samrs_k_audit_rows_per_partial(void) { return AUDIT_ROWS_PER_PARTIAL; }
int samrs_rbox_mask_prompt(const int32_t* pts, int n, int n_vertices, int h, int w, int th, int tw, int img_size, int out_size,
                           float* out, void* stream) {
    if (!pts || !out) return SAMRS_ERR_BAD_ARG;
    KRET(launch_rbox_prompt(pts, n, n_vertices, h, w, th, tw, img_size, out_size, out, (hipStream_t)stream, SAMRS_FILL_CV2_LE_451));
}
int samrs_rbox_mask_prompt_rule(const int32_t* pts, int n, int n_vertices, int h, int w, int th, int tw, int img_size, int out_size,
                                int fill_rule, float* out, void* stream) {
    if (!pts || !out || (fill_rule != SAMRS_FILL_CV2_LE_451 && fill_rule != SAMRS_FILL_CV2_GE_452)) return SAMRS_ERR_BAD_ARG;
    KRET(launch_rbox_prompt(pts, n, n_vertices, h, w, th, tw, img_size, out_size, out, (hipStream_t)stream, fill_rule));
}
int samrs_k_neck_im2col(const void* in, void* A, int n_images, int grid, int C, void* stream) {
    if (!in || !A || n_images < 1 || grid < 1 || C < 8 || C % 8) return SAMRS_ERR_BAD_ARG;
    KRET(launch_neck_im2col(in, A, n_images, grid, C, (hipStream_t)stream));
}
int samrs_k_postprocess(const float* low, int n_masks, int in_h, int in_w, int orig_h, int orig_w, int img_size,
                        int return_logits, void* out, void* stream) {
    KRET(launch_postprocess(low, n_masks, in_h, in_w, orig_h, orig_w, img_size, return_logits, out, (hipStream_t)stream));
}
int samrs_k_region_labels(const uint8_t* masks, int n, int h, int w, int complement, int32_t* labels_out, void* stream) {
    KRET(launch_region_labels(masks, n, h, w, complement, labels_out, (hipStream_t)stream));
}
int samrs_k_gemm_gln(int prec, const void* A, const void* B, void* C, const float* bias, const float* gamma_beta, int M, int N,
                     int K, const void* A_lo, const void* B_lo, void* stream) {
    KRET(launch_gemm_et_gln(prec, A, B, C, bias, gamma_beta, M, N, K, (hipStream_t)stream, A_lo, B_lo));
}
int samrs_k_gemm_split3(int prec, const void* A, const void* A_lo, const void* B, const void* B_lo, void* C, const float* bias,
                        int M, int N, int K, int out_f32, int accumulate, int split_from_n, void* stream) {
    if (!gemm_split3_ok(M, N, K, out_f32 != 0)) return SAMRS_ERR_BAD_SHAPE;
    KRET(launch_gemm_et_split3(prec, A, A_lo, B, B_lo, C, bias, M, N, K, out_f32 != 0, accumulate != 0, (hipStream_t)stream, split_from_n));
}
int samrs_k_upscale2_masks(int prec, const void* u1, const void* w, const void* w_lo, const float* bias, const float* hyper,
                           float* low, int n, int grid, int n_mask_tokens, int sel0, int n_sel, void* stream) {
    KRET(launch_upscale2_masks(prec, u1, w, w_lo, bias, hyper, low, n, grid, n_mask_tokens, sel0, n_sel, (hipStream_t)stream));
}
int samrs_k_upscaler_fused(int prec, const void* keys, const void* keys_lo, const void* w1, const void* w1_lo, const float* b1,
                           const float* ln, const void* w2, const void* w2_lo, const float* b2, const float* hyper, float* low, int n,
                           int grid, int n_mask_tokens, int sel0, int n_sel, void* stream) {
    KRET(launch_upscaler_fused(prec, keys, keys_lo, w1, w1_lo, b1, ln, w2, w2_lo, b2, hyper, low, n, grid, n_mask_tokens, sel0, n_sel,
                               (hipStream_t)stream));
}
int64_t samrs_k_mx_scale_bytes(int rows, int Kp, int is_b) { return (int64_t)mx_scale_bytes(rows, Kp, is_b != 0); }
int samrs_k_mx4_pack(int prec, const float* x, const void* hi_in, const void* lo_in, void* out_hi, void* q_hi, void* q_lo, void* s_hi,
                     void* s_lo, int rows, int K, int G, int GP, int is_b, void* stream) {
    return launch_mx4_pack(prec, x, hi_in, lo_in, out_hi, q_hi, q_lo, s_hi, s_lo, rows, K, G, GP, (is_b & 1) != 0, (hipStream_t)stream,
                           (is_b & 2) ? 1 : (is_b & 4) ? 2 : 0) == hipSuccess
               ? SAMRS_OK : SAMRS_ERR_BAD_SHAPE;
}
int samrs_k_gemm_mx(int prec, const void* A, const void* B, void* C, const float* bias, int M, int N, int K, int Kp, const void* a4_lo,
                    const void* a4_hi, const void* sa_lo, const void* sa_hi, const void* b4_hi, const void* b4_lo, const void* sb_hi,
                    const void* sb_lo, int out_f32, int accumulate, int split_from_n, void* stream) {
    return launch_gemm_et_mx(prec, A, B, C, bias, M, N, K, Kp, a4_lo, a4_hi, sa_lo, sa_hi, b4_hi, b4_lo, sb_hi, sb_lo, out_f32 != 0,
                             accumulate != 0, split_from_n, (hipStream_t)stream) == hipSuccess ? SAMRS_OK : SAMRS_ERR_BAD_SHAPE;
}
int samrs_k_gemm_mx_gelu_mxout(int prec, const void* A, const void* B, void* C_et, const float* bias, int M, int N, int K, int Kp,
                               const void* a4_lo, const void* a4_hi, const void* sa_lo, const void* sa_hi, const void* b4_hi, const void* b4_lo,
                               const void* sb_hi, const void* sb_lo, int gelu, void* o4_hi, void* o4_lo, void* so_hi, void* so_lo, void* stream) {
    return launch_gemm_et_mx(prec, A, B, C_et, bias, M, N, K, Kp, a4_lo, a4_hi, sa_lo, sa_hi, b4_hi, b4_lo, sb_hi, sb_lo, false, false,
                             (gelu & 2) ? N : 0, (hipStream_t)stream, (gelu & 1) != 0, o4_hi, o4_lo, so_hi, so_lo) == hipSuccess
               ? SAMRS_OK : SAMRS_ERR_BAD_SHAPE;
}
int samrs_k_convert_split(int prec, const float* in, void* out_hi, void* out_lo, int64_t n, void* stream) {
    KRET(launch_convert(prec, in, out_hi, (long)n, (hipStream_t)stream, out_lo));
}
int samrs_k_prompt_tokens(const float* boxes, const float* point_coords, const int32_t* point_labels, int n_prompts, int n_points,
                          float img_size, const float* gauss, const float* point_emb, const float* not_a_point, const float* iou_token,
                          const float* mask_tokens, float* tokens, float* tokens2, int T, void* stream) {
    if (!tokens || !gauss || !point_emb || !not_a_point || !iou_token || !mask_tokens || n_prompts < 1) return SAMRS_ERR_BAD_ARG;
    if ((point_coords != nullptr) != (point_labels != nullptr) || (point_coords && n_points < 1)) return SAMRS_ERR_BAD_ARG;
    PromptParams pp{};
    pp.boxes = boxes; pp.point_coords = point_coords; pp.point_labels = point_labels;
    pp.n_prompts = n_prompts; pp.n_points = point_coords ? n_points : 0;
    pp.img_size = img_size;
    pp.gauss = gauss;
    for (int i = 0; i < 4; ++i) pp.point_emb[i] = point_emb + i * 256;
    pp.not_a_point = not_a_point; pp.iou_token = iou_token; pp.mask_tokens = mask_tokens;
    const int npt = point_coords ? n_points + (boxes ? 0 : 1) : 0;
    if (T != 5 + npt + (boxes ? 2 : 0)) return SAMRS_ERR_BAD_SHAPE;
    KRET(launch_prompt_tokens(pp, tokens, tokens2, T, (hipStream_t)stream));
}
int samrs_k_dense_pe(const float* gauss, float* pe, int grid, void* stream) {
    if (!gauss || !pe || grid < 1) return SAMRS_ERR_BAD_ARG;
    KRET(launch_dense_pe(gauss, pe, grid, (hipStream_t)stream));
}
int samrs_k_mask_embed(const float* w0, const float* b0, const float* ln1w, const float* ln1b, const float* w3, const float* b3,
                       const float* ln4w, const float* ln4b, const float* w6, const float* b6, const float* mask_in, float* dense,
                       int n, int grid, void* stream) {
    if (!mask_in || !dense || n < 1) return SAMRS_ERR_BAD_ARG;
    if (grid < 1 || (grid * grid) % 16) return SAMRS_ERR_BAD_SHAPE;
    const MaskEmbedParams mp{w0, b0, ln1w, ln1b, w3, b3, ln4w, ln4b, w6, b6};
    KRET(launch_mask_embed(mp, mask_in, dense, n, grid, (hipStream_t)stream));
}
int samrs_k_fill_slot_table(const int32_t* start_host, const int32_t* slot_host, int n_runs, int32_t* out, void* stream) {
    if (!start_host || !slot_host || !out || n_runs < 1) return SAMRS_ERR_BAD_ARG;
    KRET(launch_fill_slot_table(start_host, slot_host, n_runs, out, (hipStream_t)stream));
}
int samrs_k_make_keys(int prec, const float* emb, const float* dense, const float* vec, float* out_f32, void* out_et, int n_batches,
                      int tokens, int C, const int32_t* slot_of, void* stream) {
    if (!emb || (!dense && !vec) || !out_f32 || !out_et || n_batches < 1) return SAMRS_ERR_BAD_ARG;
    if (tokens < 1 || C < 4 || C % 4) return SAMRS_ERR_BAD_SHAPE;
    KRET(launch_make_keys(prec, emb, dense, vec, out_f32, out_et, n_batches, tokens, C, (hipStream_t)stream, slot_of));
}
// ... 36 lines not shown
```

samrs_amd/csrc/kernels.h:

```cpp
#pragma once
#include <hip/hip_runtime.h>
#include <stdint.h>

hipError_t launch_gemm_et(int prec, const void* A, const void* B, void* C, const float* bias,
                          const float* add2d, int add2d_period, int M, int N, int K, bool out_f32,
                          bool gelu, bool accumulate, hipStream_t s);
hipError_t launch_gemm_et_gln(int prec, const void* A, const void* B, void* C, const float* bias, const float* gamma_beta,
                              int M, int N, int K, hipStream_t s, const void* A_lo = nullptr, const void* B_lo = nullptr);
hipError_t launch_gemm_et_stats(int prec, const void* A, const void* B, float* C, const float* bias, void* Xh, float* stats,
                                int M, int N, int K, hipStream_t s);
hipError_t launch_gemm_et_fold(int prec, const void* Xh, const void* Wf, void* C, const float* bias_f, const float* cvec,
                               const float* rowstat, int M, int N, int K, bool gelu, hipStream_t s);
bool gemm_split3_ok(int M, int N, int K, bool out_f32 = false);
hipError_t launch_gemm_et_split3(int prec, const void* A, const void* A_lo, const void* B, const void* B_lo, void* C, const float* bias,
                                 int M, int N, int K, bool out_f32, bool accumulate, hipStream_t s, int split_from_n = 0,
                                 const float* add2d = nullptr, int add2d_period = 0);
void set_gemm_variant(int v);
bool gemm_has_experiments();
bool gemm_lntail_ok(int M, int N, int K);
hipError_t launch_gemm_et_lntail(int prec, const void* A, const void* B, float* C, const float* bias, int M, int N, int K,
                                 const float* gamma, const float* beta, float eps, void* out_et, unsigned int* counters, hipStream_t s);
int swap_gelu_form(int v);
int swap_gemm_ld(int ld);
bool gemm_ld_ok(int M, int N, int K, bool gelu);
// ... 15 lines not shown
hipError_t launch_gemm_f32_batch(const F32Batch& bt, int count, int lda, int ldc, int M, int N, int K, bool relu,
                                 bool accumulate, hipStream_t s);

hipError_t launch_patch_im2col(int prec, const uint8_t* img, void* A, int n_images, int in_h, int in_w,
                               int grid, int patch, hipStream_t s, void* A_lo = nullptr);
hipError_t launch_convert(int prec, const float* in, void* out, long n, hipStream_t s, void* out_lo = nullptr);
hipError_t launch_ln_fold_weight(int prec, const float* W, const float* gamma, const float* beta, const float* bias, void* Wf,
                                 float* cvec, float* bias_f, int N, int K, hipStream_t s);
hipError_t launch_rowstats_convert(int prec, const float* X, void* Xh, float* stats, int rows, int D, hipStream_t s);
hipError_t launch_ln_rowstat(const float* stats, float* rowstat, int rows, float eps, hipStream_t s);
hipError_t launch_layernorm(int prec, const float* X, const float* gamma, const float* beta, float eps,
                            void* out_et, float* out_f32, int rows_out, int D, int window_mode, int grid,
                            int window, hipStream_t s, void* out_lo = nullptr,
                            void* mx_q_hi = nullptr, void* mx_q_lo = nullptr, void* mx_s_hi = nullptr, void* mx_s_lo = nullptr,
                            int ld_out = 0 ,
                            const int* oc_idx = nullptr, int n_oc = 0);
hipError_t launch_outlier_weight_ext(int prec, const float* W, int N, int K, const int* idx, int n_oc, void* out, int ld, int col0, hipStream_t s);
hipError_t launch_outlier_side_weight(int prec, const float* W1, const float* b1, int D, const int* idx2, int n2, const int* idx1, int n1,
                                      void* out, int Ks, float* bias_out, hipStream_t s);
hipError_t launch_outlier_gather(const void* hi, const void* lo, int D, const int* idx, int n_oc, void* out, int rows, hipStream_t s);
hipError_t launch_outlier_side_gemm(int prec, const void* Y, int lda, const void* Ws, const float* bias, int M, int K, void* out, hipStream_t s);
hipError_t launch_weight_norms(const float* W, int N, int K, float* col_sq, float* row_sq, hipStream_t s);
hipError_t launch_window_attention(int prec, const void* qkv, const float* qkv_bias, const float* rel_h, const float* rel_w, void* out,
                                   int n_images, int grid, int window, int heads, int head_dim, hipStream_t s, void* out_lo = nullptr,
                                   void* mx_q_hi = nullptr, void* mx_q_lo = nullptr, void* mx_s_hi = nullptr, void* mx_s_lo = nullptr,
                                   uint32_t lo_heads = 0xffffffffu);
hipError_t launch_gelu_split(int prec, const float* in, void* hi, void* lo, long n, hipStream_t s);
hipError_t launch_range_scan(int prec, const void* x, long n, unsigned long long* counter, hipStream_t s,
                             int cols = 0, int ld = 0 );
hipError_t launch_global_attention(int prec, const void* qkv, const float* rel_h, const float* rel_w, void* out,
                                   int n_images, int grid, int heads, int head_dim, void* vt_ws, hipStream_t s, void* out_lo = nullptr,
                                   void* mx_q_hi = nullptr, void* mx_q_lo = nullptr, void* mx_s_hi = nullptr, void* mx_s_lo = nullptr);
hipError_t launch_neck_im2col(const void* in, void* A, int n_images, int grid, int C, hipStream_t s);
hipError_t launch_transpose_f32(const float* in, float* out, int rows, int cols, hipStream_t s);

constexpr int AUDIT_PROFILE_WORDS = 48;
constexpr int AUDIT_ROWS_PER_PARTIAL = 256;
hipError_t launch_range_profile(int prec, const void* x, long n, int cols, int ld, long long* row48, hipStream_t s);
size_t column_stats_partial_floats(int M, int K);
hipError_t launch_column_stats(int prec, const void* x, int M, int K, int ld, float* partials, double* sumsq, uint32_t* maxbits, hipStream_t s);

struct PromptParams {
    const float* boxes;
    const float* point_coords;
    const int32_t* point_labels;
    int n_prompts, n_points;
    float img_size;
    const float* gauss;
    const float* point_emb[4];
    const float* not_a_point;
    const float* iou_token;
    const float* mask_tokens;
};
hipError_t launch_prompt_tokens(const PromptParams& p, float* tokens, float* tokens2 , int T, hipStream_t s);
hipError_t launch_dense_pe(const float* gauss, float* pe , int grid, hipStream_t s);
struct MaskEmbedParams {
    const float *w0, *b0, *ln1w, *ln1b, *w3, *b3, *ln4w, *ln4b, *w6, *b6;
};
hipError_t launch_mask_embed(const MaskEmbedParams& p, const float* mask_in, float* dense, int n, int grid, hipStream_t s);
hipError_t launch_fill_slot_table(const int* start, const int* slot, int n_runs, int* out, hipStream_t s);
hipError_t launch_make_keys(int prec, const float* emb, const float* dense, const float* vec, float* out_f32,
                            void* out_et, int n_batches, int tokens, int C, hipStream_t s, const int* slot_of = nullptr);
hipError_t launch_add_f32(const float* a, const float* b, float* out, long n, hipStream_t s);
hipError_t launch_token_self_attn(const float* q, const float* k, const float* v, float* o, int n, int T, int C,
                                  int heads, hipStream_t s);
constexpr int T2I_MAX_SPLITS = 16;
size_t t2i_workspace_floats(int n_prompts, int T);
hipError_t launch_t2i_attention(int prec, const float* qp, const void* kp, const void* vp, int ld, long batch_stride_rows,
                                float* out, float* workspace, int n, int T, int tokens, int Ci, int heads, hipStream_t s,
                                const int* slot_of = nullptr);
hipError_t launch_i2t_attention(int prec, const void* qi, int ld, long batch_stride_rows, const float* kt,
                                const float* vt, void* out, int n, int T, int tokens, int Ci, int heads, hipStream_t s);
hipError_t launch_group_ln_gelu(int prec, const float* in, const float* gamma, const float* beta, float eps,
                                void* out, long rows, int groups, int gsize, hipStream_t s);
hipError_t launch_upscale2_masks(int prec, const void* u1, const void* w, const void* w_lo, const float* bias, const float* hyper,
                                 float* low, int n, int grid, int n_mask_tokens, int sel0, int n_sel, hipStream_t s);
hipError_t launch_mask_product(int prec, const void* up2, const float* hyper, float* low, int n, int grid,
                               int n_mask_tokens, int sel0, int n_sel, hipStream_t s);
hipError_t launch_postprocess(const float* low, int n_masks, int in_h, int in_w, int orig_h, int orig_w,
                              int img_size, int return_logits, void* out, hipStream_t s);
hipError_t launch_paint(const uint8_t* masks, const int32_t* labels, int n, int h, int w, uint8_t* seg,
                        unsigned long long* areas, unsigned long long* class_pixels,
                        unsigned long long* class_instances, int n_classes, hipStream_t s);
hipError_t launch_select_best(const uint8_t* masks, const float* iou, int n, int nsel, int h, int w, uint8_t* out, float* quality,
                              unsigned long long* areas, hipStream_t s);
hipError_t launch_gt_match(const uint8_t* masks, int n, int h, int w, const uint8_t* label_rgb, const uint8_t* colors,
                           unsigned long long* inter, unsigned long long* gt_area, uint8_t* gt_masks, hipStream_t s);
hipError_t launch_resample_pass(const uint8_t* in, uint8_t* out, const int32_t* bounds, const int32_t* coef, int ksize,
                                int in_len, int out_len, int other, int horizontal, hipStream_t s);
hipError_t launch_rbox_prompt(const int32_t* pts, int n, int nv, int h, int w, int th, int tw, int img_size, int out_size,
                              float* out, hipStream_t s,
                              int fill_rule = 0 );
hipError_t launch_i2t_fused(int prec, const void* qi, int ld, long q_bstride, const float* kt, const float* vt, const void* w,
                            const void* w_lo , const float* bias, const float* resid,
                            long r_bstride, const float* gamma, const float* beta, float eps, float* outF, void* outE,
                            void* outE_lo , int n, int T, int tokens, int Ci, int C, hipStream_t s,
                            const int* slot_of = nullptr);

bool gemm_mx_ok(int M, int N, int K, int Kp);
size_t mx_scale_bytes(int rows, int Kp, bool is_b);
hipError_t launch_gemm_et_mx(int prec, const void* A, const void* B, void* C, const float* bias, int M, int N, int K, int Kp,
                             const void* a4_lo, const void* a4_hi, const void* sa_lo, const void* sa_hi,
                             const void* b4_hi, const void* b4_lo, const void* sb_hi, const void* sb_lo,
                             bool out_f32, bool accumulate, int split_from_n, hipStream_t s,
                             bool gelu = false, void* o4_hi = nullptr, void* o4_lo = nullptr, void* so_hi = nullptr, void* so_lo = nullptr,
                             int ld = 0, bool ext = false);
hipError_t launch_mx4_pack(int prec, const float* x, const void* hi_in, const void* lo_in, void* out_hi, void* q_hi, void* q_lo,
                           void* s_hi, void* s_lo, int rows, int K, int G, int GP, bool is_b, hipStream_t s, int perm = 0 );

hipError_t launch_upscaler_fused(int prec, const void* keys, const void* keys_lo, const void* w1, const void* w1_lo, const float* b1,
                                 const float* ln, const void* w2, const void* w2_lo, const float* b2, const float* hyper, float* low,
                                 int n, int grid, int n_mask_tokens, int sel0, int n_sel, hipStream_t s);

size_t rle_scratch_bytes(int n, int h, int w);
hipError_t launch_rle_encode(const uint8_t* masks, int n, int h, int w, void* scratch, unsigned char* out, long long out_cap,
                             long long* cursor, long long* table, hipStream_t s);

size_t rle_placed_scratch_bytes(int n, int h, int w, int x0, int H, int W);
hipError_t launch_rle_encode_placed(const uint8_t* masks, int n, int h, int w, int x0, int y0, int H, int W, void* scratch,
                                    unsigned char* out, long long out_cap, long long* cursor, long long* table, hipStream_t s);

hipError_t launch_scene_claim(const uint8_t* masks, const int32_t* ranks, const int32_t* labels, int n, int h, int w, int x0, int y0,
                              int H, int W, int32_t* order, unsigned long long* areas, unsigned long long* class_pixels,
                              unsigned long long* class_instances, int n_classes, hipStream_t s);
hipError_t launch_scene_resolve(const int32_t* order, const int32_t* labels_by_rank, int n_ranks, int H, int W, uint8_t* seg,
                                hipStream_t s);

size_t png_scratch_bytes(int n, int h, int w);
hipError_t launch_png_encode(const uint8_t* maps, int n, int h, int w, const uint8_t* lut, void* scratch, unsigned char* out,
                             long long out_cap, long long* cursor, long long* table, hipStream_t s);

constexpr int REGION_CHUNK = 32;
size_t region_scratch_bytes(int n, int h, int w);
hipError_t launch_clean_masks(uint8_t* masks, int n, int h, int w, int min_area, int mode, void* scratch, long long* areas_out,
                              long long* changed_out, hipStream_t s);
hipError_t launch_region_labels(const uint8_t* masks, int n, int h, int w, int complement, int32_t* labels_out, hipStream_t s);
```

samrs_amd/driver.py:

```python
from __future__ import annotations

import contextlib
import os

import queue
import threading
from dataclasses import dataclass, field
from typing import Callable, Iterable, Iterator, List, Optional, Sequence, Tuple

import numpy as np
import torch


def shard(items: Sequence, rank: int, world: int) -> List:
    return list(sorted(items))[rank::world]


def box_chunks(n: int, batch_size: int) -> List[Tuple[int, int]]:
    out, start = [], 0
    end = min(n, start + batch_size)
    for _ in range(n // batch_size + 1):
        if start < end:
            out.append((start, end))
        start = end
        end = min(n, start + batch_size)
    return out


@dataclass
class ImageResult:
    seg_mask: torch.Tensor
    areas: torch.Tensor
    masks: Optional[torch.Tensor] = None


class SemanticGenerator:

    def __init__(self, predictor, n_classes: int, box_batch: int = 20):
        self.predictor = predictor
        self.n_classes = n_classes
        self.box_batch = box_batch
        dev = predictor.device
        self.class_pixels = torch.zeros(n_classes, dtype=torch.int64, device=dev)
        self.class_instances = torch.zeros(n_classes, dtype=torch.int64, device=dev)

    @torch.no_grad()
    def process_image(self, image: np.ndarray, boxes: np.ndarray, labels: np.ndarray, keep_masks: bool = False,
                      already_set: bool = False) -> ImageResult:
        p = self.predictor
        if not already_set:
            p.set_image(image)
        h, w = image.shape[:2]
        dev = p.device
        seg = torch.full((h, w), 255, dtype=torch.uint8, device=dev)
        gt = torch.from_numpy(np.asarray(boxes)).to(dev)
        lab = torch.from_numpy(np.asarray(labels).astype(np.int32)).to(dev)
        areas, kept = [], []
        for s, e in box_chunks(len(labels), self.box_batch):
            tb = p.transform.apply_boxes_torch(gt[s:e], (h, w))
            masks, _, _ = p.predict_torch(None, None, tb, None, multimask_output=False)
            a = p.model.engine.paint(masks[:, 0], lab[s:e], seg, self.class_pixels, self.class_instances)
            areas.append(a)
            if keep_masks:
                kept.append(masks[:, 0])
        return ImageResult(seg, torch.cat(areas) if areas else torch.zeros(0, dtype=torch.int64, device=dev),
                           torch.cat(kept) if kept else None)


def reduce_statistics(class_pixels: torch.Tensor, class_instances: torch.Tensor, group=None):
    import torch.distributed as dist
    if not (dist.is_available() and dist.is_initialized()) or dist.get_world_size(group) == 1:
        return class_pixels.clone(), class_instances.clone()
    buf = torch.cat([class_pixels, class_instances]).contiguous()
    dev = buf.device
    if dist.get_backend(group) != "nccl":
        buf = buf.cpu()
    dist.all_reduce(buf, op=dist.ReduceOp.SUM, group=group)
    buf = buf.to(dev)
    c = class_pixels.numel()
    return buf[:c].clone(), buf[c:].clone()


def agree_on_list(items: List, group=None, src: int = 0) -> List:
    import torch.distributed as dist
    if not (dist.is_available() and dist.is_initialized()) or dist.get_world_size(group) == 1:
        return list(items)
    box = [list(items) if dist.get_rank(group) == src else None]
    dist.broadcast_object_list(box, src=src, group=group)
    return box[0]


class InstancePrompter:

    MODES = ("point", "rbox_mask", "box")
# ... 291 lines not shown
    def _stage(self, b: int, items: List[WorkItem]):
        tiles = []
        same = True
        n_off = 0
        offs = []
        self.ev_in_free[b].synchronize()
        for i, it in enumerate(items):
            nb = len(it.labels)
            if nb > self.max_boxes:
                raise ValueError(f"{nb} boxes on one image > max_boxes={self.max_boxes}")
            self.pin_box[b][n_off:n_off + nb] = torch.as_tensor(np.asarray(it.boxes, dtype=np.float32).reshape(-1, self.BOX_WIDTH))
            self.pin_lab[b][n_off:n_off + nb] = torch.as_tensor(np.asarray(it.labels).astype(np.int32))
            offs.append((n_off, nb))
            n_off += nb
        with torch.cuda.stream(self.s_h2d):
            self.s_h2d.wait_event(self.ev_dec[b])
            self.dev_box[b][:n_off].copy_(self.pin_box[b][:n_off], non_blocking=True)
            self.dev_lab[b][:n_off].copy_(self.pin_lab[b][:n_off], non_blocking=True)
            for i, it in enumerate(items):
                img = it.image
                H, W = int(img.shape[0]), int(img.shape[1])
                native = (H == self.side and W == self.side)
                if isinstance(img, torch.Tensor) and img.is_cuda:
                    t = img
                    if native:
                        self.dev_in[b][i].copy_(t, non_blocking=True)
                        t = self.dev_in[b][i]
                elif native:
                    src = img if isinstance(img, torch.Tensor) else torch.from_numpy(np.ascontiguousarray(img))
                    if src.is_pinned():
                        self.dev_in[b][i].copy_(src, non_blocking=True)
                    else:
                        if self.pin_in is None:
                            self.pin_in = [torch.empty(self.batch, self.side, self.side, 3, dtype=torch.uint8).pin_memory()
                                           for _ in range(2)]
                        np.copyto(self.pin_in[b][i].numpy(), src.numpy())
                        self.dev_in[b][i].copy_(self.pin_in[b][i], non_blocking=True)
                    t = self.dev_in[b][i]
                else:
                    src = img if isinstance(img, torch.Tensor) else torch.from_numpy(np.ascontiguousarray(img))
                    t = src.to(self.dev)
                if not native:
                    t = self.transform.apply_image_device(t.contiguous())
                    t.record_stream(self.s_enc)
                    same = False
                tiles.append((t, (H, W)))
            self.ev_h2d[b].record(self.s_h2d)
        return tiles, same, offs

    def _encode(self, b: int, tiles, same: bool):
        n = len(tiles)
        with torch.cuda.stream(self.s_enc):
            self.s_enc.wait_event(self.ev_h2d[b])
            self.s_enc.wait_event(self.ev_dec[b])
            with self._mode():
                if same:
                    self.eng.set_images(self.dev_in[b][:n], b * self.batch)
                else:
                    self.eng.set_images_ragged([t for t, _ in tiles], b * self.batch)
            self.ev_enc[b].record(self.s_enc)
            self.ev_in_free[b].record(self.s_enc)

    multimask = False

    def _tile_prompts(self, b: int, tile, hw, off: int, nb: int):
        in_size = (int(tile.shape[0]), int(tile.shape[1]))
        return self._input_frame_boxes(self.dev_box[b][off:off + nb], hw, in_size), None, None, None

    def _decode_multi(self, b: int, tiles, offs):
        per = [self._tile_prompts(b, t, hw, off, nb) for (t, hw), (off, nb) in zip(tiles, offs)]
        args = [None if per[0][j] is None else torch.cat([p[j] for p in per]) for j in range(4)]
        masks, iou, _ = self.eng.predict_multi([b * self.batch + i for i in range(len(tiles))], [nb for _, nb in offs], *args,
                                               self.multimask, False, [(int(t.shape[0]), int(t.shape[1])) for t, _ in tiles],
                                               [tuple(hw) for _, hw in tiles])
        return list(zip(masks, iou))

    def _decode_tile(self, b: int, i: int, tile, hw, off: int, nb: int, out: _OutBuf, pre=None) -> None:
        eng, (H, W) = self.eng, hw
        in_size = (int(tile.shape[0]), int(tile.shape[1]))
        native = (H, W) == (self.side, self.side)
        seg = self.seg_dev[b][i] if native else torch.full((H, W), 255, dtype=torch.uint8, device=self.dev)
        kept = []
        for s, e in box_chunks(nb, self.box_batch):
            if pre is not None:
                masks = pre[0][s:e]
            else:
                tb = self._input_frame_boxes(self.dev_box[b][off + s:off + e], (H, W), in_size)
                masks, _, _ = eng.predict(b * self.batch + i, tb, None, None, None, False, False, in_size, (H, W))
            if self.min_region_area:
                eng.clean_masks(masks[:, 0], self.min_region_area, self.region_mode, areas_out=False,
                                changed_out=self.chg_dev[b][i, s:e])
            eng.paint(masks[:, 0], self.dev_lab[b][off + s:off + e], seg, self.class_pixels, self.class_instances,
                      areas_out=self.area_dev[b][i, s:e])
            if self.rle:
                eng.rle_encode(masks[:, 0], self.rle_dev[b], self.rle_cur[b], self.rle_tab[b][off + s:off + e])
            if self.keep_masks:
                kept.append(masks[:, 0].view(torch.uint8))
        if self.png and not native:
            eng.png_encode(seg, self.png_lut, self.png_dev[b], self.png_cur[b], self.png_tab[b][i:i + 1])
        if native:
            out.seg[i].copy_(seg, non_blocking=True)
        else:
            out.odd[i] = seg.cpu()
        out.masks[i] = torch.cat(kept).cpu() if (self.keep_masks and kept) else None

    def _input_frame_boxes(self, boxes: torch.Tensor, hw, in_size) -> torch.Tensor:
        if tuple(hw) == tuple(in_size):
            return boxes
        return self.transform.apply_boxes_torch(boxes, hw)

    def _decode(self, b: int, items, tiles, offs, out: _OutBuf):
        with torch.cuda.stream(self.s_dec):
            self.s_dec.wait_event(self.ev_enc[b])
            self.seg_dev[b].fill_(255)
            if self.rle:
                self.rle_cur[b].zero_()
            if self.png:
                self.png_cur[b].zero_()
            with self._mode():
                pre = self._decode_multi(b, tiles, offs) if self.batch_decode and sum(nb for _, nb in offs) else None
                for i, ((t, hw), (off, nb)) in enumerate(zip(tiles, offs)):
                    self._decode_tile(b, i, t, hw, off, nb, out, None if pre is None else pre[i])
            if self.png:
                self._encode_png(b, tiles)
            out.areas.copy_(self.area_dev[b], non_blocking=True)
            if self.min_region_area:
                out.changed.copy_(self.chg_dev[b], non_blocking=True)
            if self.rle:
                out.rle_tab.copy_(self.rle_tab[b], non_blocking=True)
                out.rle_cur.copy_(self.rle_cur[b], non_blocking=True)
            if self.png:
                out.png_tab.copy_(self.png_tab[b], non_blocking=True)
                out.png_cur.copy_(self.png_cur[b], non_blocking=True)
            self._extra_outputs(b, out)
            self.ev_dec[b].record(self.s_dec)
            out.done.record(self.s_dec)

    def _encode_png(self, b: int, tiles) -> None:
        native = [i for i, (_, hw) in enumerate(tiles) if tuple(hw) == (self.side, self.side)]
        runs: List[List[int]] = []
        for i in native:
            if runs and runs[-1][-1] == i - 1:
                runs[-1].append(i)
            else:
                runs.append([i])
        for r in runs:
            i0, i1 = r[0], r[-1] + 1
            self.eng.png_encode(self.seg_dev[b][i0:i1], self.png_lut, self.png_dev[b], self.png_cur[b], self.png_tab[b][i0:i1])

    def _extra_outputs(self, b: int, out: _OutBuf) -> None:
        pass

    def _fetch_extra(self, b: int, out: _OutBuf, n_boxes: int):
        return None

    def _extra_result(self, r: TileResult, i: int, off: int, nb: int, out: _OutBuf, extra) -> None:
        pass

    def _fetch_rle(self, b: int, out: _OutBuf, n_boxes: int):
        tab, out.rle_bytes = self._fetch_strings(self.rle_dev[b], out.rle_cur, out.rle_tab, out.rle_bytes, n_boxes)
        return tab, out.rle_bytes.numpy()

    def _fetch_png(self, b: int, out: _OutBuf, n_tiles: int):
        tab, out.png_bytes = self._fetch_strings(self.png_dev[b], out.png_cur, out.png_tab.view(-1, 2), out.png_bytes, 2 * n_tiles,
                                                 what="PNG buffer too small: a file", knob="png_buffer_mb")
        return tab.reshape(-1, 2, 2), out.png_bytes.numpy()

    def _fetch_strings(self, dev: torch.Tensor, cur: torch.Tensor, tab_host: torch.Tensor, host: torch.Tensor, n_boxes: int,
                       what: str = "RLE buffer too small: a mask", knob: str = "rle_buffer_mb"):
        total = int(cur[0])
        tab = tab_host[:n_boxes].numpy()
        if n_boxes and int(tab[:, 1].min()) < 0:
            need = int((-tab[:, 1] - 1).max())
            raise RuntimeError(f"{what} needs {need} bytes and the batch already holds {total}; raise "
                               f"{knob} (now {dev.numel() >> 20})")
        if host.numel() < total:
# ... 249 lines not shown
```

samrs_amd/engine.py:

```python
from __future__ import annotations

import contextlib
import ctypes as C
import os
from typing import Dict, List, Optional, Sequence, Tuple

import numpy as np
import torch

from .synth import SamConfig

_HERE = os.path.dirname(os.path.abspath(__file__))
LIB_PATH = os.path.join(_HERE, "csrc", "libsamrs_hip.so")

PREC_BF16, PREC_F16 = 0, 1
PRECISIONS = {"bf16": PREC_BF16, "f16": PREC_F16, "fp16": PREC_F16}

ABI_VERSION = 5
REGION_MODES = {"holes": 1, "islands": 2, "both": 3}
SPLIT_PATCH, SPLIT_NECK, SPLIT_OI, SPLIT_UP, SPLIT_DEFAULT = 1, 2, 4, 8, 15
SPLIT_ATTN, SPLIT_MLP, SPLIT_ATTN_V, SPLIT_LIN2, SPLIT_ALL = 16, 32, 64, 128, 255

OK, ERR_NOT_SET, ERR_BAD_SHAPE, ERR_BAD_ARG, ERR_HIP, ERR_BAD_WEIGHTS, ERR_CAPACITY, ERR_PRECISION, ERR_RANGE = 0, -1, -2, -3, -4, -5, -6, -7, -8


class samrs_config(C.Structure):
    _fields_ = [
        ("embed_dim", C.c_int32), ("depth", C.c_int32), ("num_heads", C.c_int32),
        ("n_global", C.c_int32), ("global_attn_indexes", C.c_int32 * 8),
        ("img_size", C.c_int32), ("patch_size", C.c_int32), ("window_size", C.c_int32),
        ("out_chans", C.c_int32), ("max_images", C.c_int32), ("max_prompts", C.c_int32),
        ("max_points", C.c_int32), ("precision", C.c_int32),
    ]


_lib = None

PREDICT_MULTI_ARGTYPES = [C.c_void_p, C.c_int, C.POINTER(C.c_int), C.POINTER(C.c_int), C.c_void_p, C.c_void_p, C.c_void_p, C.c_int,
                          C.c_void_p, C.c_int, C.c_int, C.POINTER(C.c_int), C.POINTER(C.c_int), C.POINTER(C.c_void_p), C.c_void_p,
                          C.c_void_p, C.c_void_p]


def load_library() -> C.CDLL:
    global _lib
    if _lib is not None:
        return _lib
    path = os.environ.get("SAMRS_LIB_PATH", LIB_PATH)
    if not os.path.exists(path):
        raise ImportError(
            f"{path} not found: build it with `make -C samrs_amd/csrc` (or __graft_entry__.build()). "
            "samrs_amd has no CPU / PyTorch fallback by design.")
    lib = C.CDLL(path)
    vp, ip, fp = C.c_void_p, C.c_int, C.c_float
    lib.samrs_abi_version.restype = ip
    lib.samrs_create.restype = vp
    lib.samrs_create.argtypes = [C.POINTER(samrs_config), ip, C.c_char_p, ip]
    lib.samrs_destroy.argtypes = [vp]
    lib.samrs_destroy.restype = None
    lib.samrs_last_error.argtypes = [vp]
    lib.samrs_last_error.restype = C.c_char_p
    lib.samrs_load_weight.argtypes = [vp, C.c_char_p, vp, C.POINTER(C.c_int64), ip]
    lib.samrs_finalize_weights.argtypes = [vp, vp]
    lib.samrs_set_images.argtypes = [vp, vp, ip, ip, ip, ip, vp]
    lib.samrs_set_images_ragged.argtypes = [vp, C.POINTER(vp), C.POINTER(ip), C.POINTER(ip), ip, ip, vp]
    lib.samrs_get_embedding.argtypes = [vp, ip, vp, vp]
    lib.samrs_set_embedding.argtypes = [vp, ip, vp, vp]
    lib.samrs_reset_image.argtypes = [vp, ip]
    lib.samrs_predict.argtypes = [vp, ip, ip, vp, vp, vp, ip, vp, ip, ip, ip, ip, ip, ip, vp, vp, vp, vp]
    lib.samrs_predict_multi.argtypes = PREDICT_MULTI_ARGTYPES
    lib.samrs_paint.argtypes = [vp, vp, vp, ip, ip, ip, vp, vp, vp, vp, ip, vp]
    lib.samrs_debug_encoder_prefix.argtypes = [vp, vp, ip, ip, ip, ip, vp, vp]
    lib.samrs_debug_encoder_prefix.restype = ip
    lib.samrs_debug_time_dominant_kernel.argtypes = [vp, ip]
    lib.samrs_debug_time_dominant_kernel.restype = ip
    lib.samrs_debug_dominant_kernel_time.argtypes = [vp, C.POINTER(C.c_float), C.POINTER(ip), C.POINTER(ip), C.POINTER(ip), C.POINTER(ip)]
    lib.samrs_debug_dominant_kernel_time.restype = ip
    lib.samrs_resample_pass_u8.argtypes = [vp, vp, vp, vp, ip, ip, ip, ip, ip, vp]
    lib.samrs_resample_pass_u8.restype = ip
    lib.samrs_rbox_mask_prompt.argtypes = [vp, ip, ip, ip, ip, ip, ip, ip, ip, vp, vp]
    lib.samrs_rbox_mask_prompt.restype = ip
    lib.samrs_rbox_mask_prompt_rule.argtypes = [vp, ip, ip, ip, ip, ip, ip, ip, ip, ip, vp, vp]
    lib.samrs_rbox_mask_prompt_rule.restype = ip
    lib.samrs_k_gemm.argtypes = [ip, vp, vp, vp, vp, vp, ip, ip, ip, ip, ip, ip, ip, vp]
    lib.samrs_k_gemm_f32.argtypes = [vp, ip, vp, vp, vp, ip, ip, ip, ip, ip, ip, vp]
    lib.samrs_k_gemm_stats.argtypes = [ip, vp, vp, vp, vp, vp, vp, ip, ip, ip, vp]
    lib.samrs_k_gemm_fold.argtypes = [ip, vp, vp, vp, vp, vp, vp, ip, ip, ip, ip, vp]
    lib.samrs_k_ln_rowstat.argtypes = [vp, vp, ip, fp, vp]
    lib.samrs_k_ln_fold_weight.argtypes = [ip, vp, vp, vp, vp, vp, vp, vp, ip, ip, vp]
    lib.samrs_k_rowstats_convert.argtypes = [ip, vp, vp, vp, ip, ip, vp]
    lib.samrs_set_option.argtypes = [vp, C.c_char_p, ip]
    lib.samrs_get_option.argtypes = [vp, C.c_char_p, C.POINTER(ip)]
    lib.samrs_rle_encode.argtypes = [vp, vp, ip, ip, ip, vp, C.c_int64, vp, vp, vp]
    lib.samrs_scene_claim.argtypes = [vp, vp, vp, vp, ip, ip, ip, ip, ip, ip, ip, vp, vp, vp, vp, ip, vp]
    lib.samrs_scene_resolve.argtypes = [vp, vp, vp, ip, ip, ip, vp, vp]
    lib.samrs_rle_encode_placed.argtypes = [vp, vp, ip, ip, ip, ip, ip, ip, ip, vp, C.c_int64, vp, vp, vp]
    for name in ("samrs_scene_claim", "samrs_scene_resolve", "samrs_rle_encode_placed"):
        getattr(lib, name).restype = ip
    lib.samrs_k_convert_split.argtypes = [ip, vp, vp, vp, C.c_int64, vp]
    lib.samrs_select_best.argtypes = [vp, vp, vp, ip, ip, ip, ip, vp, vp, vp, vp]
    lib.samrs_gt_match.argtypes = [vp, vp, ip, ip, ip, vp, vp, vp, vp, vp, vp]
    lib.samrs_clean_masks.argtypes = [vp, vp, ip, ip, ip, ip, ip, vp, vp, vp]
    lib.samrs_clean_masks.restype = ip
    lib.samrs_k_region_labels.argtypes = [vp, ip, ip, ip, ip, vp, vp]
    lib.samrs_k_region_labels.restype = ip
    lib.samrs_png_encode_labels.argtypes = [vp, vp, ip, ip, ip, vp, vp, C.c_int64, vp, vp, vp]
    lib.samrs_k_upscaler_fused.argtypes = [ip, vp, vp, vp, vp, vp, vp, vp, vp, vp, vp, vp, ip, ip, ip, ip, ip, vp]
    lib.samrs_k_convert.argtypes = [ip, vp, vp, C.c_int64, vp]
    lib.samrs_k_layernorm.argtypes = [ip, vp, vp, vp, fp, vp, vp, ip, ip, ip, ip, ip, ip, vp]
    lib.samrs_k_window_attention.argtypes = [ip, vp, vp, vp, vp, vp, ip, ip, ip, ip, ip, vp]
    lib.samrs_k_global_attention.argtypes = [ip, vp, vp, vp, vp, ip, ip, ip, ip, vp]
    lib.samrs_k_postprocess.argtypes = [vp, ip, ip, ip, ip, ip, ip, ip, vp, vp]
    lib.samrs_k_neck_im2col.argtypes = [vp, vp, ip, ip, ip, vp]
    lib.samrs_k_neck_im2col.restype = ip
    lib.samrs_k_gemm_gln.argtypes = [ip, vp, vp, vp, vp, vp, ip, ip, ip, vp, vp, vp]
    lib.samrs_k_upscale2_masks.argtypes = [ip, vp, vp, vp, vp, vp, vp, ip, ip, ip, ip, ip, vp]
    lib.samrs_k_gemm_split3.argtypes = [ip, vp, vp, vp, vp, vp, vp, ip, ip, ip, ip, ip, ip, vp]
    i64 = C.c_int64
    lib.samrs_k_mx_scale_bytes.argtypes = [ip, ip, ip]
    lib.samrs_k_mx_scale_bytes.restype = i64
    lib.samrs_k_mx4_pack.argtypes = [ip, vp, vp, vp, vp, vp, vp, vp, vp, ip, ip, ip, ip, ip, vp]
    lib.samrs_k_gemm_mx.argtypes = [ip, vp, vp, vp, vp, ip, ip, ip, ip, vp, vp, vp, vp, vp, vp, vp, vp, ip, ip, ip, vp]
    lib.samrs_k_layernorm_mx.argtypes = [ip, vp, vp, vp, fp, vp, ip, ip, vp, vp, vp, vp, vp]
    lib.samrs_k_attention_mx.argtypes = [ip, ip, vp, vp, vp, vp, vp, vp, ip, ip, ip, ip, vp, vp, vp, vp, vp]
    lib.samrs_k_gemm_mx_gelu_mxout.argtypes = [ip, vp, vp, vp, vp, ip, ip, ip, ip, vp, vp, vp, vp, vp, vp, vp, vp, ip, vp, vp, vp, vp, vp]
    for name in ("samrs_k_mx4_pack", "samrs_k_gemm_mx", "samrs_k_layernorm_mx", "samrs_k_attention_mx", "samrs_k_gemm_mx_gelu_mxout"):
        getattr(lib, name).restype = ip
    lib.samrs_k_prompt_tokens.argtypes = [vp, vp, vp, ip, ip, fp, vp, vp, vp, vp, vp, vp, vp, ip, vp]
    lib.samrs_k_dense_pe.argtypes = [vp, vp, ip, vp]
    lib.samrs_k_mask_embed.argtypes = [vp] * 12 + [ip, ip, vp]
    lib.samrs_k_fill_slot_table.argtypes = [C.POINTER(C.c_int32), C.POINTER(C.c_int32), ip, vp, vp]
    lib.samrs_k_make_keys.argtypes = [ip, vp, vp, vp, vp, vp, ip, ip, ip, vp, vp]
    lib.samrs_k_token_self_attn.argtypes = [vp, vp, vp, vp, ip, ip, ip, ip, vp]
    lib.samrs_k_t2i_workspace_floats.argtypes = [ip, ip]
    lib.samrs_k_t2i_workspace_floats.restype = i64
    lib.samrs_k_t2i_attention.argtypes = [ip, vp, vp, vp, ip, i64, vp, vp, ip, ip, ip, ip, ip, vp, vp]
    lib.samrs_k_i2t_attention.argtypes = [ip, vp, ip, i64, vp, vp, vp, ip, ip, ip, ip, ip, vp]
    lib.samrs_k_i2t_fused.argtypes = [ip, vp, ip, i64, vp, vp, vp, vp, vp, vp, i64, vp, vp, fp, vp, vp, vp, ip, ip, ip, ip, ip, vp, vp]
    lib.samrs_k_group_ln_gelu.argtypes = [ip, vp, vp, vp, fp, vp, i64, ip, ip, vp]
    lib.samrs_k_mask_product.argtypes = [ip, vp, vp, vp, ip, ip, ip, ip, ip, vp]
    for name in ("samrs_k_prompt_tokens", "samrs_k_dense_pe", "samrs_k_mask_embed", "samrs_k_fill_slot_table", "samrs_k_make_keys",
                 "samrs_k_token_self_attn", "samrs_k_t2i_attention", "samrs_k_i2t_attention", "samrs_k_i2t_fused",
                 "samrs_k_group_ln_gelu", "samrs_k_mask_product", "samrs_debug_copy_buffer", "samrs_debug_outlier_columns"):
        getattr(lib, name).restype = ip
    lib.samrs_debug_copy_buffer.argtypes = [vp, C.c_char_p, vp, C.c_size_t, vp]
    lib.samrs_debug_outlier_columns.argtypes = [vp, ip, ip, C.POINTER(C.c_int32)]
    lib.samrs_get_slot_info.argtypes = [vp, ip, C.POINTER(C.c_int32), C.POINTER(C.c_int32), C.POINTER(C.c_int32)]
    lib.samrs_audit_site_count.argtypes = [vp, C.POINTER(ip)]
    lib.samrs_audit_site_name.argtypes = [vp, ip, C.c_char_p, ip, C.POINTER(ip)]
    lib.samrs_audit_read_profile.argtypes = [vp, vp, ip]
    lib.samrs_audit_read_columns.argtypes = [vp, ip, vp, vp, C.POINTER(C.c_int64)]
    lib.samrs_k_range_profile.argtypes = [ip, vp, C.c_long, ip, ip, vp, vp]
    lib.samrs_k_column_stats.argtypes = [ip, vp, ip, ip, ip, vp, vp, vp, vp]
    lib.samrs_k_audit_rows_per_partial.argtypes = []
    for name in ("samrs_audit_site_count", "samrs_audit_site_name", "samrs_audit_read_profile", "samrs_audit_read_columns",
                 "samrs_k_range_profile", "samrs_k_column_stats", "samrs_k_audit_rows_per_partial"):
        getattr(lib, name).restype = ip
    for name in ("samrs_load_weight", "samrs_finalize_weights", "samrs_set_images", "samrs_set_images_ragged", "samrs_get_embedding",
                 "samrs_set_embedding", "samrs_reset_image", "samrs_predict", "samrs_predict_multi", "samrs_paint", "samrs_k_gemm",
                 "samrs_k_gemm_f32", "samrs_k_convert", "samrs_k_layernorm", "samrs_k_window_attention",
                 "samrs_k_global_attention", "samrs_k_postprocess", "samrs_k_gemm_gln", "samrs_k_upscale2_masks",
                 "samrs_k_gemm_stats", "samrs_k_gemm_fold", "samrs_k_ln_fold_weight", "samrs_k_rowstats_convert", "samrs_k_ln_rowstat",
                 "samrs_set_option", "samrs_get_option", "samrs_rle_encode", "samrs_k_convert_split", "samrs_select_best", "samrs_gt_match",
                 "samrs_png_encode_labels", "samrs_k_upscaler_fused", "samrs_k_gemm_split3", "samrs_get_slot_info"):
        getattr(lib, name).restype = ip
    if lib.samrs_abi_version() != ABI_VERSION:
        raise ImportError("libsamrs_hip.so ABI version mismatch; rebuild it")
    _lib = lib
    return lib


def _ptr(t: Optional[torch.Tensor]) -> Optional[int]:
    return None if t is None else t.data_ptr()


def _stream() -> int:
    return torch.cuda.current_stream().cuda_stream


class EngineError(RuntimeError):
    pass


def multi_call_args(slots: Sequence[int], counts: Sequence[int], input_sizes: Sequence[Sequence[int]],
                    original_sizes: Sequence[Sequence[int]], n_rows: int) -> Tuple[List[int], List[int], List[int], List[int]]:
    n_img = len(slots)
    if n_img < 1:
        raise ValueError("predict_multi needs at least one image")
    if not (len(counts) == len(input_sizes) == len(original_sizes) == n_img):
        raise ValueError(f"predict_multi: {n_img} slots but {len(counts)} prompt counts, {len(input_sizes)} input sizes and "
                         f"{len(original_sizes)} original sizes")
    offsets = [0]
    for c in counts:
        if int(c) < 0:
            raise ValueError(f"predict_multi: negative prompt count {c}")
# ... 347 lines not shown
        assert m.is_contiguous() and iou.is_contiguous() and iou.dtype == torch.float32 and tuple(iou.shape) == (n, c)
        best = best_out if best_out is not None else torch.empty(n, h, w, dtype=torch.uint8, device=self.device)
        qual = quality_out if quality_out is not None else torch.empty(n, dtype=torch.float32, device=self.device)
        areas = areas_out if areas_out is not None else torch.empty(n, dtype=torch.int64, device=self.device)
        assert best.is_contiguous() and qual.is_contiguous() and areas.is_contiguous() and areas.dtype == torch.int64
        with torch.cuda.device(self.device):
            self._check(self.lib.samrs_select_best(self.handle, m.data_ptr(), iou.data_ptr(), n, c, h, w, best.data_ptr(),
                                                   qual.data_ptr(), areas.data_ptr(), _stream()))
        return best, qual, areas

    def clean_masks(self, masks: torch.Tensor, min_area: int, mode="both", areas_out=None, changed_out=None):
        m = masks.view(torch.uint8) if masks.dtype == torch.bool else masks
        if m.dim() != 3 or m.dtype != torch.uint8:
            raise ValueError(f"masks must be bool / uint8 [n, H, W], got {masks.dtype} {tuple(masks.shape)}")
        if not (m.is_cuda and m.is_contiguous()):
            raise ValueError("masks must be a contiguous tensor on the engine's device (they are rewritten in place)")
        code = REGION_MODES.get(mode) if isinstance(mode, str) else int(mode)
        if code is None:
            raise ValueError(f"mode must be one of {sorted(REGION_MODES)}, got {mode!r}")
        n, h, w = m.shape
        outs = []
        for name, t in (("areas_out", areas_out), ("changed_out", changed_out)):
            if t is False:
                t = None
            elif t is None:
                t = torch.empty(n, dtype=torch.int64, device=self.device)
            elif not (isinstance(t, torch.Tensor) and t.dtype == torch.int64 and t.is_cuda and t.is_contiguous() and t.numel() == n):
                raise ValueError(f"{name} must be a contiguous int64 [{n}] tensor on the engine's device, None or False")
            outs.append(t)
        with torch.cuda.device(self.device):
            self._check(self.lib.samrs_clean_masks(self.handle, m.data_ptr(), n, h, w, int(min_area), code, _ptr(outs[0]),
                                                   _ptr(outs[1]), _stream()))
        return masks, outs[0], outs[1]

    def region_labels(self, masks: torch.Tensor, complement: bool = False) -> torch.Tensor:
        m = masks.view(torch.uint8) if masks.dtype == torch.bool else masks
        assert m.dim() == 3 and m.dtype == torch.uint8 and m.is_cuda and m.is_contiguous()
        n, h, w = m.shape
        out = torch.empty(n, h, w, dtype=torch.int32, device=self.device)
        with torch.cuda.device(self.device):
            self._check(self.lib.samrs_k_region_labels(m.data_ptr(), n, h, w, int(bool(complement)), out.data_ptr(), _stream()))
        return out

    def gt_match(self, masks: torch.Tensor, label_rgb: torch.Tensor, colors: torch.Tensor, inter_out: Optional[torch.Tensor] = None,
                 gt_area_out: Optional[torch.Tensor] = None, gt_masks_out: Optional[torch.Tensor] = None):
        m = masks.view(torch.uint8) if masks.dtype == torch.bool else masks
        if m.dim() != 3:
            raise ValueError(f"masks must be [n, H, W], got {tuple(m.shape)}")
        n, h, w = m.shape
        if tuple(label_rgb.shape) != (h, w, 3) or label_rgb.dtype != torch.uint8:
            raise ValueError(f"label_rgb must be uint8 [{h}, {w}, 3] (the masks' size), got {label_rgb.dtype} {tuple(label_rgb.shape)}")
        if tuple(colors.shape) != (n, 3) or colors.dtype != torch.uint8:
            raise ValueError(f"colors must be uint8 [{n}, 3], got {colors.dtype} {tuple(colors.shape)}")
        for t in (m, label_rgb, colors):
            assert t.is_cuda and t.is_contiguous()
        inter = inter_out if inter_out is not None else torch.empty(n, dtype=torch.int64, device=self.device)
        gta = gt_area_out if gt_area_out is not None else torch.empty(n, dtype=torch.int64, device=self.device)
        for t in (inter, gta):
            assert t.dtype == torch.int64 and t.is_cuda and t.is_contiguous() and t.numel() == n
        if gt_masks_out is not None:
            assert gt_masks_out.dtype == torch.uint8 and gt_masks_out.is_cuda and gt_masks_out.is_contiguous()
            assert gt_masks_out.numel() == n * h * w
        with torch.cuda.device(self.device):
            self._check(self.lib.samrs_gt_match(self.handle, m.data_ptr(), n, h, w, label_rgb.data_ptr(), colors.data_ptr(),
                                                inter.data_ptr(), gta.data_ptr(), _ptr(gt_masks_out), _stream()))
        return inter, gta, gt_masks_out

    def paint(self, masks: torch.Tensor, labels: torch.Tensor, seg: torch.Tensor,
              class_pixels: Optional[torch.Tensor] = None, class_instances: Optional[torch.Tensor] = None,
              areas_out: Optional[torch.Tensor] = None) -> torch.Tensor:
        m = masks.view(torch.uint8) if masks.dtype == torch.bool else masks
        m = m.reshape(-1, m.shape[-2], m.shape[-1]).contiguous()
        n, h, w = m.shape
        labels = labels.to(dtype=torch.int32, device=self.device).contiguous()
        if areas_out is not None:
            assert areas_out.dtype == torch.int64 and areas_out.is_contiguous() and areas_out.numel() == n and areas_out.is_cuda
        areas = areas_out if areas_out is not None else torch.empty(n, dtype=torch.int64, device=self.device)
        ncls = 0 if class_pixels is None else class_pixels.numel()
        with torch.cuda.device(self.device):
            self._check(self.lib.samrs_paint(self.handle, m.data_ptr(), labels.data_ptr(), n, h, w, seg.data_ptr(),
                                             areas.data_ptr(), _ptr(class_pixels), _ptr(class_instances), ncls, _stream()))
        return areas

    def _check_scene(self, rc: int) -> None:
        if rc == ERR_BAD_ARG:
            raise EngineError(self.lib.samrs_last_error(self.handle).decode())
        self._check(rc)

    def scene_claim(self, masks: torch.Tensor, ranks: torch.Tensor, window: Sequence[int], order: torch.Tensor,
                    labels: Optional[torch.Tensor] = None, class_pixels: Optional[torch.Tensor] = None,
                    class_instances: Optional[torch.Tensor] = None, areas_out: Optional[torch.Tensor] = None) -> torch.Tensor:
        m = masks.view(torch.uint8) if masks.dtype == torch.bool else masks
        m = (m if m.dim() == 3 else m.reshape(-1, m.shape[-2], m.shape[-1])).contiguous()
        n, h, w = m.shape
        x0, y0, ww, wh = (int(v) for v in window)
        if (ww, wh) != (w, h):
            raise ValueError(f"window {tuple(window)} does not have the masks' size {w} x {h}")
        assert order.dtype == torch.int32 and order.dim() == 2 and order.is_cuda and order.is_contiguous()
        H, W = int(order.shape[0]), int(order.shape[1])
        ranks = ranks.to(dtype=torch.int32, device=self.device).contiguous()
        assert ranks.numel() == n
        if labels is not None:
            labels = labels.to(dtype=torch.int32, device=self.device).contiguous()
            assert labels.numel() == n
        if areas_out is not None:
            assert areas_out.dtype == torch.int64 and areas_out.is_contiguous() and areas_out.numel() == n and areas_out.is_cuda
        areas = areas_out if areas_out is not None else torch.empty(n, dtype=torch.int64, device=self.device)
        ncls = 0 if class_pixels is None else class_pixels.numel()
        with torch.cuda.device(self.device):
            self._check_scene(self.lib.samrs_scene_claim(self.handle, m.data_ptr(), ranks.data_ptr(), _ptr(labels), n, h, w, x0, y0, H, W,
                                                         order.data_ptr(), areas.data_ptr(), _ptr(class_pixels), _ptr(class_instances),
                                                         ncls, _stream()))
        return areas

    def scene_resolve(self, order: torch.Tensor, labels_by_rank: torch.Tensor, seg: Optional[torch.Tensor] = None) -> torch.Tensor:
        assert order.dtype == torch.int32 and order.dim() == 2 and order.is_cuda and order.is_contiguous()
        H, W = int(order.shape[0]), int(order.shape[1])
        lab = labels_by_rank.to(dtype=torch.int32, device=self.device).contiguous()
        if seg is None:
            seg = torch.empty(H, W, dtype=torch.uint8, device=self.device)
        assert seg.dtype == torch.uint8 and seg.is_cuda and seg.is_contiguous() and tuple(seg.shape) == (H, W)
        with torch.cuda.device(self.device):
            self._check_scene(self.lib.samrs_scene_resolve(self.handle, order.data_ptr(), lab.data_ptr() if lab.numel() else None,
                                                           lab.numel(), H, W, seg.data_ptr(), _stream()))
        return seg

    def rle_encode_placed(self, masks: torch.Tensor, window: Sequence[int], size: Sequence[int], out: torch.Tensor,
                          cursor: torch.Tensor, table: torch.Tensor) -> None:
        m = masks.view(torch.uint8) if masks.dtype == torch.bool else masks
        m = (m if m.dim() == 3 else m.reshape(-1, m.shape[-2], m.shape[-1])).contiguous()
        n, h, w = m.shape
        x0, y0, ww, wh = (int(v) for v in window)
        if (ww, wh) != (w, h):
            raise ValueError(f"window {tuple(window)} does not have the masks' size {w} x {h}")
        assert out.dtype == torch.uint8 and out.is_cuda and out.is_contiguous() and out.data_ptr() % 16 == 0
        assert cursor.dtype == torch.int64 and cursor.is_cuda and table.dtype == torch.int64 and table.is_cuda
        assert table.is_contiguous() and table.numel() >= 3 * n
        with torch.cuda.device(self.device):
            self._check_scene(self.lib.samrs_rle_encode_placed(self.handle, m.data_ptr(), n, h, w, x0, y0, int(size[0]), int(size[1]),
                                                               out.data_ptr(), out.numel(), cursor.data_ptr(), table.data_ptr(),
                                                               _stream()))
```

Before: 144.0.

## Fuse mask threshold upsampling with paint and add live-layout t2i attention kernel

Adds a predict_paint entry point whose kernel upsamples low-res logits, thresholds them, writes the masks, and paints the segmentation map and areas in one pass. This removes the separate postprocess and paint launches and the re-read of the full-resolution masks. The driver uses it by default when no mask cleaning is needed. The diff also adds a register-resident token-to-image attention partial kernel, selected by default through an environment variable, and rewrites the bilinear quarter-scale arithmetic with explicit FMAs.

```diff
diff --git a/include/samrs_hip.h b/include/samrs_hip.h
--- a/include/samrs_hip.h
+++ b/include/samrs_hip.h
@@ -78,6 +78,14 @@
                 int orig_h, int orig_w, uint8_t* seg_mask, int64_t* areas_out,
                 int64_t* class_pixels, int64_t* class_instances, int n_classes, void* stream);
 
+int samrs_predict_paint(samrs_engine_t* e, int slot, int n_prompts,
+                        const float* boxes, const float* point_coords, const int32_t* point_labels,
+                        int n_points, const float* mask_input,
+                        int in_h, int in_w, int orig_h, int orig_w,
+                        uint8_t* masks_out, float* iou_out, float* lowres_out,
+                        const int32_t* labels, uint8_t* seg_mask, int64_t* areas_out,
+                        int64_t* class_pixels, int64_t* class_instances, int n_classes, void* stream);
+
 int samrs_select_best(samrs_engine_t* e, const uint8_t* masks, const float* iou, int n, int n_sel, int h, int w,
                       uint8_t* best_out, float* quality_out, int64_t* areas_out, void* stream);
 
diff --git a/include/samrs_hip_internal.h b/include/samrs_hip_internal.h
--- a/include/samrs_hip_internal.h
+++ b/include/samrs_hip_internal.h
@@ -47,6 +47,8 @@
 int samrs_k_neck_im2col(const void* in_et, void* A_et, int n_images, int grid, int C, void* stream);
 int samrs_k_postprocess(const float* lowres, int n_masks, int in_h, int in_w, int orig_h,
                         int orig_w, int img_size, int return_logits, void* out, void* stream);
+int samrs_k_threshold_paint(const float* lowres, int n, int h, int w, int img_size, const int32_t* labels, uint8_t* masks_out,
+                            uint8_t* seg, int64_t* areas, void* stream);
 int samrs_k_gemm_gln(int prec, const void* A_et, const void* B_et, void* C_et, const float* bias,
                      const float* gamma_beta, int M, int N, int K, const void* A_lo_et, const void* B_lo_et, void* stream);
 int samrs_k_gemm_split3(int prec, const void* A_et, const void* A_lo_et, const void* B_et, const void* B_lo_et, void* C,
diff --git a/samrs_amd/csrc/decoder_kernels.hip b/samrs_amd/csrc/decoder_kernels.hip
--- a/samrs_amd/csrc/decoder_kernels.hip
+++ b/samrs_amd/csrc/decoder_kernels.hip
@@ -1,3 +1,5 @@
+#include <cstdlib>
+
 #include "common.h"
 #include "kernels.h"
 
@@ -318,6 +320,138 @@
         r[0] = mm; r[1] = ll;
 #pragma unroll
         for (int c = 0; c < 8; ++c) r[2 + c] = a[c];
+    }
+}
+
+template <int PREC, int NT, bool MASKED>
+__device__ __forceinline__ void t2i_live_update(const uint4& kk, const uint4& vv, bool valid, const float (&q)[NT][8],
+                                                float (&acc)[NT][8], float (&m)[NT], float (&l)[NT]) {
+#pragma clang fp contract(off)
+    const uint32_t kw[4] = {kk.x, kk.y, kk.z, kk.w};
+    const uint32_t vw[4] = {vv.x, vv.y, vv.z, vv.w};
+    float kf[8], vf[8];
+#pragma unroll
+    for (int c = 0; c < 4; ++c) {
+        kf[2 * c] = ET<PREC>::to_float((uint16_t)(kw[c] & 0xffffu));
+        kf[2 * c + 1] = ET<PREC>::to_float((uint16_t)(kw[c] >> 16));
+        vf[2 * c] = ET<PREC>::to_float((uint16_t)(vw[c] & 0xffffu));
+        vf[2 * c + 1] = ET<PREC>::to_float((uint16_t)(vw[c] >> 16));
+    }
+#pragma unroll
+    for (int t = 0; t < NT; ++t) {
+        float p[8];
+#pragma unroll
+        for (int c = 0; c < 8; ++c) p[c] = q[t][c] * kf[c];
+        float sc = 0.f + p[0];
+#pragma unroll
+        for (int c = 1; c < 8; ++c) sc = sc + p[c];
+        sc = sc + __builtin_bit_cast(float, __builtin_amdgcn_update_dpp(0, __builtin_bit_cast(int, sc), 0xB1, 0xF, 0xF, true));
+        if (MASKED) sc = valid ? sc : T2I_NEG;
+        const float mn = fmaxf(m[t], sc);
+        const float corr = __builtin_amdgcn_exp2f(m[t] - mn);
+        float pj = __builtin_amdgcn_exp2f(sc - mn);
+        if (MASKED) pj = valid ? pj : 0.f;
+        l[t] = __builtin_fmaf(l[t], corr, pj);
+#pragma unroll
+        for (int c = 0; c < 8; ++c) acc[t][c] = __builtin_fmaf(pj, vf[c], acc[t][c] * corr);
+        m[t] = mn;
+    }
+}
+
+template <int PREC, int NT>
+__global__ __launch_bounds__(256, 2) void t2i_partial_live_kernel(const float* __restrict__ qp, const uint16_t* __restrict__ kp,
+                                                               const uint16_t* __restrict__ vp, int ld, long bstride,
+                                                               const int* __restrict__ slot_of, float* __restrict__ part, int T,
+                                                               int tokens, int Ci, int kpw, int tg, int tgs) {
+    __shared__ float sm[4][NT][16][T2I_REC];
+    const int split = blockIdx.x, b = blockIdx.y, t0 = tg * T2I_TG;
+    const int lane = threadIdx.x & 63, wave = threadIdx.x >> 6;
+    const int ch = lane & 15, kq = lane >> 4;
+    float q[NT][8], acc[NT][8], m[NT], l[NT];
+#pragma unroll
+    for (int t = 0; t < NT; ++t) {
+        m[t] = T2I_NEG;
+        l[t] = 0.f;
+        const float* qr = qp + ((size_t)b * T + t0 + t) * Ci + ch * 8;
+#pragma unroll
+        for (int c = 0; c < 8; ++c) {
+            q[t][c] = qr[c] * (0.25f * 1.44269504088896340736f);
+            acc[t][c] = 0.f;
+        }
+    }
+    const int kbeg = (split * 4 + wave) * kpw;
+    const int kend = kbeg + kpw < tokens ? kbeg + kpw : tokens;
+    const int kbat = slot_of ? slot_of[b] : b;
+    const uint16_t* kb = kp + (size_t)kbat * bstride * ld + ch * 8;
+    const uint16_t* vb = vp + (size_t)kbat * bstride * ld + ch * 8;
+    constexpr int U = 2;
+    uint4 kk[U], vv[U], kn[U], vn[U];
+#define T2I_LOAD(dk_, dv_, k0_)                                                                  \
+    _Pragma("unroll") for (int u_ = 0; u_ < U; ++u_) {                                           \
+        const int key_ = (k0_) + 4 * u_ + kq;                                                    \
+        dk_[u_] = dv_[u_] = make_uint4(0u, 0u, 0u, 0u);                                          \
+        if (key_ < kend) {                                                                       \
+            dk_[u_] = *reinterpret_cast<const uint4*>(kb + (size_t)key_ * ld);                   \
+            dv_[u_] = *reinterpret_cast<const uint4*>(vb + (size_t)key_ * ld);                   \
+        }                                                                                        \
+    }
+    T2I_LOAD(kk, vv, kbeg)
+    int k0 = kbeg;
+    for (; k0 + 4 * U <= kend; k0 += 4 * U) {
+        T2I_LOAD(kn, vn, k0 + 4 * U)
+#pragma unroll
+        for (int u = 0; u < U; ++u) t2i_live_update<PREC, NT, false>(kk[u], vv[u], true, q, acc, m, l);
+#pragma unroll
+        for (int u = 0; u < U; ++u) { kk[u] = kn[u]; vv[u] = vn[u]; }
+    }
+    if (k0 < kend) {
+#pragma unroll
+        for (int u = 0; u < U; ++u) t2i_live_update<PREC, NT, true>(kk[u], vv[u], k0 + 4 * u + kq < kend, q, acc, m, l);
+    }
+#undef T2I_LOAD
+    {
+#pragma clang fp contract(off)
+#pragma unroll
+        for (int off = 16; off <= 32; off <<= 1) {
+#pragma unroll
+            for (int t = 0; t < NT; ++t) {
+                const float mo = __shfl_xor(m[t], off, 64), lo = __shfl_xor(l[t], off, 64);
+                const float mn = fmaxf(m[t], mo);
+                const float fs = __builtin_amdgcn_exp2f(m[t] - mn), fo = __builtin_amdgcn_exp2f(mo - mn);
+                l[t] = off == 16 ? __builtin_fmaf(lo, fo, l[t] * fs) : __builtin_fmaf(l[t], fs, lo * fo);
+#pragma unroll
+                for (int c = 0; c < 8; ++c) acc[t][c] = __builtin_fmaf(acc[t][c], fs, __shfl_xor(acc[t][c], off, 64) * fo);
+                m[t] = mn;
+            }
+        }
+        if (lane < 16) {
+#pragma unroll
+            for (int t = 0; t < NT; ++t) {
+                float* r = sm[wave][t][ch];
+                r[0] = m[t]; r[1] = l[t];
+#pragma unroll
+                for (int c = 0; c < 8; ++c) r[2 + c] = acc[t][c];
+            }
+        }
+        __syncthreads();
+        if (threadIdx.x < NT * 16) {
+            const int t = threadIdx.x >> 4, c16 = threadIdx.x & 15;
+            float mm = sm[0][t][c16][0];
+#pragma unroll
+            for (int w = 1; w < 4; ++w) mm = fmaxf(mm, sm[w][t][c16][0]);
+            float ll = 0.f, a[8] = {0.f, 0.f, 0.f, 0.f, 0.f, 0.f, 0.f, 0.f};
+#pragma unroll
+            for (int w = 0; w < 4; ++w) {
+                const float f = __builtin_amdgcn_exp2f(sm[w][t][c16][0] - mm);
+                ll = __builtin_fmaf(sm[w][t][c16][1], f, ll);
+#pragma unroll
+                for (int c = 0; c < 8; ++c) a[c] = __builtin_fmaf(sm[w][t][c16][2 + c], f, a[c]);
+            }
+            float* r = part + ((((size_t)b * tgs + tg) * gridDim.x + split) * (T2I_TG * 16) + threadIdx.x) * T2I_REC;
+            r[0] = mm; r[1] = ll;
+#pragma unroll
+            for (int c = 0; c < 8; ++c) r[2 + c] = a[c];
+        }
     }
 }
 
@@ -778,6 +912,20 @@
     return ly.w0 * (lx.w0 * r0[lx.i0] + lx.w1 * r0[lx.i1]) + ly.w1 * (lx.w0 * r1[lx.i0] + lx.w1 * r1[lx.i1]);
 }
 
+__device__ __forceinline__ void quad_quarter_scale(float yw0, float yw1, float aw0, float aw1, float bw0, float bw1, float cw0,
+                                                   float cw1, float dw0, float dw1, float a00, float a01, float a10, float a11,
+                                                   float c00, float c01, float c10, float c11, float v[4]) {
+#pragma clang fp contract(off)
+    const float A0 = __builtin_fmaf(aw0, a00, aw1 * a01), A1 = __builtin_fmaf(aw0, a10, aw1 * a11);
+    v[0] = __builtin_fmaf(yw1, A1, yw0 * A0);
+    const float B0 = __builtin_fmaf(bw1, a01, bw0 * a00), B1 = __builtin_fmaf(bw0, a10, bw1 * a11);
+    v[1] = __builtin_fmaf(yw0, B0, yw1 * B1);
+    const float C0 = cw0 * c00 + cw1 * c01, C1 = cw0 * c10 + cw1 * c11;
+    v[2] = yw0 * C0 + yw1 * C1;
+    const float D0 = __builtin_fmaf(dw1, c01, dw0 * c00), D1 = __builtin_fmaf(dw0, c10, dw1 * c11);
+    v[3] = yw0 * D0 + yw1 * D1;
+}
+
 __global__ __launch_bounds__(256) void postprocess_kernel(const float* __restrict__ low_all, int LS, int in_h, int in_w,
                                                           int H, int W, int img_size, int return_logits,
                                                           void* __restrict__ out) {
@@ -797,10 +945,7 @@
         const Lin la = lin_coord(X0, s1, LS), lb = lin_coord(X0 + 1, s1, LS), lc = lin_coord(X0 + 2, s1, LS), ld = lin_coord(X0 + 3, s1, LS);
         const float a00 = r0[la.i0], a01 = r0[la.i1], a10 = r1[la.i0], a11 = r1[la.i1];
         const float c00 = r0[lc.i0], c01 = r0[lc.i1], c10 = r1[lc.i0], c11 = r1[lc.i1];
-        v[0] = ly.w0 * (la.w0 * a00 + la.w1 * a01) + ly.w1 * (la.w0 * a10 + la.w1 * a11);
-        v[1] = ly.w0 * (lb.w0 * a00 + lb.w1 * a01) + ly.w1 * (lb.w0 * a10 + lb.w1 * a11);
-        v[2] = ly.w0 * (lc.w0 * c00 + lc.w1 * c01) + ly.w1 * (lc.w0 * c10 + lc.w1 * c11);
-        v[3] = ly.w0 * (ld.w0 * c00 + ld.w1 * c01) + ly.w1 * (ld.w0 * c10 + ld.w1 * c11);
+        quad_quarter_scale(ly.w0, ly.w1, la.w0, la.w1, lb.w0, lb.w1, lc.w0, lc.w1, ld.w0, ld.w1, a00, a01, a10, a11, c00, c01, c10, c11, v);
     } else if (identity) {
 #pragma unroll
         for (int e = 0; e < 4; ++e) v[e] = (X0 + e < W) ? stage1(low, LS, s1, Y, X0 + e) : 0.f;
@@ -887,6 +1032,105 @@
             }
             float c = wave_sum((float)cnt);
             if ((threadIdx.x & 63) == 0 && c > 0.f) atomicAdd(&cnt_s[j - jlo], (unsigned int)c);
+        }
+        __syncthreads();
+        if (threadIdx.x < jhi - jlo && cnt_s[threadIdx.x]) atomicAdd(&areas[jlo + threadIdx.x], (unsigned long long)cnt_s[threadIdx.x]);
+        __syncthreads();
+    }
+    if (in && (done[0] | done[1] | done[2] | done[3])) {
+        uint4* sp = reinterpret_cast<uint4*>(seg + p0);
+        uint4 o = *sp;
+        o.x = (o.x & ~done[0]) | res[0]; o.y = (o.y & ~done[1]) | res[1];
+        o.z = (o.z & ~done[2]) | res[2]; o.w = (o.w & ~done[3]) | res[3];
+        *sp = o;
+    }
+}
+
+constexpr int TP_JB = 4;
+struct TpTaps {
+    float4 r0, r1;
+    float l0, l1, h0, h1;
+};
+__global__ __launch_bounds__(256) void threshold_paint_kernel(const float* __restrict__ low_all, int LS, int img_size, int H, int W,
+                                                              const int32_t* __restrict__ labels, int n, uint8_t* __restrict__ masks,
+                                                              uint8_t* __restrict__ seg, unsigned long long* __restrict__ areas) {
+    __shared__ unsigned int cnt_s[PA_CHUNK];
+    const long hw = (long)H * W;
+    const long p0 = ((long)blockIdx.x * 256 + threadIdx.x) * 16;
+    const bool in = p0 < hw;
+    const long pc = in ? p0 : 0;
+    const int Y = (int)(pc / W), X0 = (int)(pc % W);
+    const float s1 = (float)LS / (float)img_size;
+    const Lin ly = lin_coord(Y, s1, LS);
+    const Lin la = lin_coord(X0, s1, LS), lb = lin_coord(X0 + 1, s1, LS), lc = lin_coord(X0 + 2, s1, LS), ld = lin_coord(X0 + 3, s1, LS);
+    const Lin ma = lin_coord(X0 + 4, s1, LS), mb = lin_coord(X0 + 5, s1, LS), mc = lin_coord(X0 + 6, s1, LS), md = lin_coord(X0 + 7, s1, LS);
+    const int c0 = X0 >> 2;
+    const int cl = c0 > 0 ? c0 - 1 : 0, ch = c0 + 4 < LS ? c0 + 4 : LS - 1;
+    const bool left = la.i0 != c0 - 1;
+    const size_t o0 = (size_t)ly.i0 * LS, o1 = (size_t)ly.i1 * LS, per = (size_t)LS * LS;
+    auto load = [&](int j, TpTaps& t) {
+        const float* r0 = low_all + (size_t)j * per + o0;
+        const float* r1 = low_all + (size_t)j * per + o1;
+        t.r0 = *reinterpret_cast<const float4*>(r0 + c0);
+        t.r1 = *reinterpret_cast<const float4*>(r1 + c0);
+        t.l0 = r0[cl]; t.h0 = r0[ch];
+        t.l1 = r1[cl]; t.h1 = r1[ch];
+    };
+    uint32_t done[4] = {0u, 0u, 0u, 0u}, res[4] = {0u, 0u, 0u, 0u};
+    for (int jlo = 0; jlo < n; jlo += PA_CHUNK) {
+        const int jhi = jlo + PA_CHUNK < n ? jlo + PA_CHUNK : n;
+        if (threadIdx.x < PA_CHUNK) cnt_s[threadIdx.x] = 0u;
+        __syncthreads();
+        TpTaps cur[TP_JB], nxt[TP_JB];
+#pragma unroll
+        for (int u = 0; u < TP_JB; ++u) load(jlo + u < jhi ? jlo + u : jhi - 1, cur[u]);
+        for (int j0 = jlo; j0 < jhi; j0 += TP_JB) {
+            const bool more = j0 + TP_JB < jhi;
+            if (more) {
+#pragma unroll
+                for (int u = 0; u < TP_JB; ++u) load(j0 + TP_JB + u < jhi ? j0 + TP_JB + u : jhi - 1, nxt[u]);
+            }
+#pragma unroll
+            for (int u = 0; u < TP_JB; ++u) {
+                const int j = j0 + u;
+                if (j < jhi) {
+                    const TpTaps& t = cur[u];
+                    const float t0[6] = {t.l0, t.r0.x, t.r0.y, t.r0.z, t.r0.w, t.h0};
+                    const float t1[6] = {t.l1, t.r1.x, t.r1.y, t.r1.z, t.r1.w, t.h1};
+                    uint32_t w[4];
+#pragma unroll
+                    for (int q = 0; q < 4; ++q) {
+                        float v[4];
+                        if (q == 0)
+                            quad_quarter_scale(ly.w0, ly.w1, la.w0, la.w1, lb.w0, lb.w1, lc.w0, lc.w1, ld.w0, ld.w1,
+                                               left ? t0[1] : t0[0], left ? t0[2] : t0[1], left ? t1[1] : t1[0], left ? t1[2] : t1[1],
+                                               t0[1], t0[2], t1[1], t1[2], v);
+                        else
+                            quad_quarter_scale(ly.w0, ly.w1, ma.w0, ma.w1, mb.w0, mb.w1, mc.w0, mc.w1, md.w0, md.w1, t0[q], t0[q + 1],
+                                               t1[q], t1[q + 1], t0[q + 1], t0[q + 2], t1[q + 1], t1[q + 2], v);
+                        w[q] = (v[0] > 0.f ? 1u : 0u) | (v[1] > 0.f ? 1u << 8 : 0u) | (v[2] > 0.f ? 1u << 16 : 0u) |
+                               (v[3] > 0.f ? 1u << 24 : 0u);
+                    }
+                    unsigned int cnt = 0;
+                    const uint32_t lab = (uint32_t)(uint8_t)labels[j] * 0x01010101u;
+                    if (in) {
+                        *reinterpret_cast<uint4*>(masks + (size_t)j * hw + p0) = make_uint4(w[0], w[1], w[2], w[3]);
+#pragma unroll
+                        for (int k = 0; k < 4; ++k) {
+                            cnt += __popc(w[k]);
+                            const uint32_t mm = w[k] * 0xFFu;
+                            res[k] = (res[k] & ~mm) | (mm & lab);
+                            done[k] |= mm;
+                        }
+                    }
+                    float c = wave_sum((float)cnt);
+                    if ((threadIdx.x & 63) == 0 && c > 0.f) atomicAdd(&cnt_s[j - jlo], (unsigned int)c);
+                }
+            }
+            if (more) {
+#pragma unroll
+                for (int u = 0; u < TP_JB; ++u) cur[u] = nxt[u];
+            }
         }
         __syncthreads();
         if (threadIdx.x < jhi - jlo && cnt_s[threadIdx.x]) atomicAdd(&areas[jlo + threadIdx.x], (unsigned long long)cnt_s[threadIdx.x]);
@@ -1223,8 +1467,24 @@
     dim3 g(splits, n, tgs), b(256);
     const uint16_t* k = (const uint16_t*)kp;
     const uint16_t* v = (const uint16_t*)vp;
-    if (prec == PREC_BF16) t2i_partial_kernel<PREC_BF16><<<g, b, 0, s>>>(qp, k, v, ld, bstride, slot_of, workspace, T, tokens, Ci, kpw);
-    else t2i_partial_kernel<PREC_F16><<<g, b, 0, s>>>(qp, k, v, ld, bstride, slot_of, workspace, T, tokens, Ci, kpw);
+    static const int live = [] { const char* e = getenv("SAMRS_T2I_LAYOUT"); return (e && atoi(e) == 0) ? 0 : 1; }();
+    if (!live) {
+        if (prec == PREC_BF16) t2i_partial_kernel<PREC_BF16><<<g, b, 0, s>>>(qp, k, v, ld, bstride, slot_of, workspace, T, tokens, Ci, kpw);
+        else t2i_partial_kernel<PREC_F16><<<g, b, 0, s>>>(qp, k, v, ld, bstride, slot_of, workspace, T, tokens, Ci, kpw);
+    } else {
+        for (int tg = 0; tg < tgs; ++tg) {
+            const int nt = T - tg * T2I_TG < T2I_TG ? T - tg * T2I_TG : T2I_TG;
+            const dim3 gl(splits, n);
+#define T2I_LIVE(P, NT) t2i_partial_live_kernel<P, NT><<<gl, b, 0, s>>>(qp, k, v, ld, bstride, slot_of, workspace, T, tokens, Ci, kpw, tg, tgs)
+#define T2I_LIVE_NT(NT) case NT: if (prec == PREC_BF16) T2I_LIVE(PREC_BF16, NT); else T2I_LIVE(PREC_F16, NT); break;
+            switch (nt) {
+                T2I_LIVE_NT(1) T2I_LIVE_NT(2) T2I_LIVE_NT(3) T2I_LIVE_NT(4) T2I_LIVE_NT(5) T2I_LIVE_NT(6) T2I_LIVE_NT(7) T2I_LIVE_NT(8)
+                default: return hipErrorInvalidValue;
+            }
+#undef T2I_LIVE_NT
+#undef T2I_LIVE
+        }
+    }
     t2i_merge_kernel<<<dim3(n, tgs), T2I_TG * 16, 0, s>>>(workspace, o, splits, T, Ci);
     return hipGetLastError();
 }
@@ -1320,6 +1580,24 @@
     return hipGetLastError();
 }
 
+bool threshold_paint_ok(const float* low, int in_h, int in_w, int orig_h, int orig_w, int img_size, const uint8_t* masks,
+                        const uint8_t* seg, const unsigned long long* areas) {
+    static const int fused = [] { const char* v = getenv("SAMRS_PAINT_FUSED"); return (v && atoi(v) == 0) ? 0 : 1; }();
+    return fused && masks && seg && areas && orig_h == in_h && orig_w == in_w && img_size % 4 == 0 && orig_w <= img_size &&
+           orig_h <= img_size && orig_w % 16 == 0 && (((uintptr_t)low | (uintptr_t)masks | (uintptr_t)seg) & 15) == 0;
+}
+hipError_t launch_threshold_paint(const float* low, int n, int h, int w, int img_size, const int32_t* labels, uint8_t* masks,
+                                  uint8_t* seg, unsigned long long* areas, unsigned long long* class_pixels,
+                                  unsigned long long* class_instances, int n_classes, hipStream_t s) {
+    if (n < 1 || !threshold_paint_ok(low, h, w, h, w, img_size, masks, seg, areas) || !labels) return hipErrorInvalidValue;
+    const long hw = (long)h * w;
+    HIP_CHECK_RET(hipMemsetAsync(areas, 0, sizeof(unsigned long long) * n, s));
+    threshold_paint_kernel<<<(int)((hw / 16 + 255) / 256), 256, 0, s>>>(low, img_size / 4, img_size, h, w, labels, n, masks, seg, areas);
+    if (class_pixels || class_instances)
+        class_stats_kernel<<<1, 64, 0, s>>>(areas, labels, n, class_pixels, class_instances, n_classes);
+    return hipGetLastError();
+}
+
 hipError_t launch_select_best(const uint8_t* masks, const float* iou, int n, int nsel, int h, int w, uint8_t* out, float* quality,
                               unsigned long long* areas, hipStream_t s) {
     if (n < 1 || nsel < 1 || h < 1 || w < 1) return hipErrorInvalidValue;
diff --git a/samrs_amd/csrc/engine.hip b/samrs_amd/csrc/engine.hip
--- a/samrs_amd/csrc/engine.hip
+++ b/samrs_amd/csrc/engine.hip
@@ -1336,9 +1336,16 @@
     void* masks;
 };
 
+struct PaintArgs {
+    const int32_t* labels;
+    uint8_t* seg;
+    int64_t *areas, *cpix, *cins;
+    int n_classes;
+};
+
 static int predict_chunk(samrs_engine_t* e, const PredictImage* seg, int n_seg, int n, const float* boxes, const float* point_coords,
                          const int32_t* point_labels, int n_points, const float* mask_input, int multimask,
-                         int return_logits, float* iou_out, float* lowres_out, void* stream);
+                         int return_logits, float* iou_out, float* lowres_out, void* stream, const PaintArgs* paint = nullptr);
 
 static std::string slot_note(int slot) { return " (slot " + std::to_string(slot) + ")"; }
 
@@ -1380,7 +1387,7 @@
 
 static int predict_images(samrs_engine_t* e, const PredictImage* im, int n_img, const float* boxes, const float* point_coords,
                           const int32_t* point_labels, int n_points, const float* mask_input, int multimask, int return_logits,
-                          float* iou_out, float* lowres_out, void* stream) {
+                          float* iou_out, float* lowres_out, void* stream, const PaintArgs* paint = nullptr) {
     const int cap = e->cfg.max_prompts;
     const size_t nsel = multimask ? 3 : 1;
     const int np = point_coords ? n_points : 0;
@@ -1400,11 +1407,14 @@
             seg.push_back(sgm);
         }
         while (first < n_img && im[first].p1 <= off + m) ++first;
+        PaintArgs pa{};
+        if (paint) { pa = *paint; pa.labels += off; if (pa.areas) pa.areas += off; }
         const int rc = predict_chunk(
             e, seg.data(), (int)seg.size(), m, boxes ? boxes + (size_t)off * 4 : nullptr,
             point_coords ? point_coords + (size_t)off * np * 2 : nullptr, point_labels ? point_labels + (size_t)off * np : nullptr,
             n_points, mask_input ? mask_input + (size_t)off * 256 * 256 : nullptr, multimask, return_logits,
-            iou_out ? iou_out + (size_t)off * nsel : nullptr, lowres_out ? lowres_out + (size_t)off * nsel * 256 * 256 : nullptr, stream);
+            iou_out ? iou_out + (size_t)off * nsel : nullptr, lowres_out ? lowres_out + (size_t)off * nsel * 256 * 256 : nullptr, stream,
+            paint ? &pa : nullptr);
         if (rc) return rc;
     }
     return SAMRS_OK;
@@ -1448,7 +1458,7 @@
 
 static int predict_chunk(samrs_engine_t* e, const PredictImage* seg, int n_seg, int n, const float* boxes, const float* point_coords,
                          const int32_t* point_labels, int n_points, const float* mask_input, int multimask,
-                         int return_logits, float* iou_out, float* lowres_out, void* stream) {
+                         int return_logits, float* iou_out, float* lowres_out, void* stream, const PaintArgs* paint) {
     const samrs_config& c = e->cfg;
     if (n < 1 || n > c.max_prompts) return fail(e, SAMRS_ERR_CAPACITY, "n_prompts=%d exceeds max_prompts=%d", n, c.max_prompts);
     hipStream_t s = (hipStream_t)stream;
@@ -1615,6 +1625,20 @@
         CK(e, launch_gemm_et(prec, e->U1, e->up2_w, e->U2, e->up2_b, nullptr, 0, Mi * 4, C / 2, C / 4, false, true, false, s));
         CK(e, launch_mask_product(prec, e->U2, e->HYPER, low, n, g, 4, sel0, nsel, s));
     }
+    if (paint) {
+        const PredictImage& im = seg[0];
+        uint8_t* m = (uint8_t*)im.masks;
+        if (threshold_paint_ok(low, im.in_h, im.in_w, im.orig_h, im.orig_w, c.img_size, m, paint->seg, (unsigned long long*)paint->areas)) {
+            CK(e, launch_threshold_paint(low, n, im.orig_h, im.orig_w, c.img_size, paint->labels, m, paint->seg,
+                                         (unsigned long long*)paint->areas, (unsigned long long*)paint->cpix,
+                                         (unsigned long long*)paint->cins, paint->n_classes, s));
+        } else {
+            CK(e, launch_postprocess(low, n, im.in_h, im.in_w, im.orig_h, im.orig_w, c.img_size, 0, m, s));
+            CK(e, launch_paint(m, paint->labels, n, im.orig_h, im.orig_w, paint->seg, (unsigned long long*)paint->areas,
+                               (unsigned long long*)paint->cpix, (unsigned long long*)paint->cins, paint->n_classes, s));
+        }
+        return SAMRS_OK;
+    }
     for (int k = 0; k < n_seg; ++k)
         if (seg[k].masks)
             CK(e, launch_postprocess(low + (size_t)seg[k].p0 * nsel * 256 * 256, (seg[k].p1 - seg[k].p0) * nsel, seg[k].in_h, seg[k].in_w,
@@ -1630,6 +1654,20 @@
     CK(e, launch_paint(masks, labels, n, h, w, seg, (unsigned long long*)areas, (unsigned long long*)cpix,
                        (unsigned long long*)cins, n_classes, (hipStream_t)stream));
     return SAMRS_OK;
+}
+
+int samrs_predict_paint(samrs_engine_t* e, int slot, int n, const float* boxes, const float* point_coords,
+                        const int32_t* point_labels, int n_points, const float* mask_input, int in_h, int in_w, int orig_h,
+                        int orig_w, uint8_t* masks_out, float* iou_out, float* lowres_out, const int32_t* labels, uint8_t* seg,
+                        int64_t* areas, int64_t* cpix, int64_t* cins, int n_classes, void* stream) {
+    if (!e) return SAMRS_ERR_BAD_ARG;
+    if (n < 1) return fail(e, SAMRS_ERR_BAD_ARG, "n_prompts must be >= 1");
+    if (!masks_out || !labels) return fail(e, SAMRS_ERR_BAD_ARG, "samrs_predict_paint: bad argument");
+    if ((cpix || cins) && !areas) return fail(e, SAMRS_ERR_BAD_ARG, "samrs_predict_paint: class statistics need areas_out");
+    const PredictImage im{slot, 0, n, in_h, in_w, orig_h, orig_w, masks_out};
+    { const int rc = check_predict(e, &im, 1, false, boxes, point_coords, point_labels, n_points, mask_input); if (rc != SAMRS_OK) return rc; }
+    const PaintArgs pa{labels, seg, areas, cpix, cins, n_classes};
+    return predict_images(e, &im, 1, boxes, point_coords, point_labels, n_points, mask_input, 0, 0, iou_out, lowres_out, stream, &pa);
 }
 
 void samrs_debug_set_gemm_variant(int v) { set_gemm_variant(v); }
@@ -2115,6 +2153,11 @@
                         int return_logits, void* out, void* stream) {
     KRET(launch_postprocess(low, n_masks, in_h, in_w, orig_h, orig_w, img_size, return_logits, out, (hipStream_t)stream));
 }
+int samrs_k_threshold_paint(const float* lowres, int n, int h, int w, int img_size, const int32_t* labels, uint8_t* masks_out,
+                            uint8_t* seg, int64_t* areas, void* stream) {
+    KRET(launch_threshold_paint(lowres, n, h, w, img_size, labels, masks_out, seg, (unsigned long long*)areas, nullptr, nullptr, 0,
+                                (hipStream_t)stream));
+}
 int samrs_k_region_labels(const uint8_t* masks, int n, int h, int w, int complement, int32_t* labels_out, void* stream) {
     KRET(launch_region_labels(masks, n, h, w, complement, labels_out, (hipStream_t)stream));
 }
diff --git a/samrs_amd/csrc/kernels.h b/samrs_amd/csrc/kernels.h
--- a/samrs_amd/csrc/kernels.h
+++ b/samrs_amd/csrc/kernels.h
@@ -121,6 +121,11 @@
 hipError_t launch_paint(const uint8_t* masks, const int32_t* labels, int n, int h, int w, uint8_t* seg,
                         unsigned long long* areas, unsigned long long* class_pixels,
                         unsigned long long* class_instances, int n_classes, hipStream_t s);
+bool threshold_paint_ok(const float* low, int in_h, int in_w, int orig_h, int orig_w, int img_size, const uint8_t* masks,
+                        const uint8_t* seg, const unsigned long long* areas);
+hipError_t launch_threshold_paint(const float* low, int n, int h, int w, int img_size, const int32_t* labels, uint8_t* masks,
+                                  uint8_t* seg, unsigned long long* areas, unsigned long long* class_pixels,
+                                  unsigned long long* class_instances, int n_classes, hipStream_t s);
 hipError_t launch_select_best(const uint8_t* masks, const float* iou, int n, int nsel, int h, int w, uint8_t* out, float* quality,
                               unsigned long long* areas, hipStream_t s);
 hipError_t launch_gt_match(const uint8_t* masks, int n, int h, int w, const uint8_t* label_rgb, const uint8_t* colors,
diff --git a/samrs_amd/driver.py b/samrs_amd/driver.py
--- a/samrs_amd/driver.py
+++ b/samrs_amd/driver.py
@@ -10,6 +10,8 @@
 
 import numpy as np
 import torch
+
+PAINT_FUSED = os.environ.get("SAMRS_PAINT_FUSED", "1") != "0"
 
 
 def shard(items: Sequence, rank: int, world: int) -> List:
@@ -467,16 +469,22 @@
         seg = self.seg_dev[b][i] if native else torch.full((H, W), 255, dtype=torch.uint8, device=self.dev)
         kept = []
         for s, e in box_chunks(nb, self.box_batch):
+            fused = pre is None and PAINT_FUSED and not self.min_region_area
             if pre is not None:
                 masks = pre[0][s:e]
             else:
                 tb = self._input_frame_boxes(self.dev_box[b][off + s:off + e], (H, W), in_size)
-                masks, _, _ = eng.predict(b * self.batch + i, tb, None, None, None, False, False, in_size, (H, W))
+                if fused:
+                    masks = eng.predict_paint(b * self.batch + i, tb, self.dev_lab[b][off + s:off + e], seg, in_size, (H, W),
+                                              self.class_pixels, self.class_instances, areas_out=self.area_dev[b][i, s:e])[0]
+                else:
+                    masks, _, _ = eng.predict(b * self.batch + i, tb, None, None, None, False, False, in_size, (H, W))
             if self.min_region_area:
                 eng.clean_masks(masks[:, 0], self.min_region_area, self.region_mode, areas_out=False,
                                 changed_out=self.chg_dev[b][i, s:e])
-            eng.paint(masks[:, 0], self.dev_lab[b][off + s:off + e], seg, self.class_pixels, self.class_instances,
-                      areas_out=self.area_dev[b][i, s:e])
+            if not fused:
+                eng.paint(masks[:, 0], self.dev_lab[b][off + s:off + e], seg, self.class_pixels, self.class_instances,
+                          areas_out=self.area_dev[b][i, s:e])
             if self.rle:
                 eng.rle_encode(masks[:, 0], self.rle_dev[b], self.rle_cur[b], self.rle_tab[b][off + s:off + e])
             if self.keep_masks:
diff --git a/samrs_amd/engine.py b/samrs_amd/engine.py
--- a/samrs_amd/engine.py
+++ b/samrs_amd/engine.py
@@ -69,6 +69,8 @@
     lib.samrs_predict.argtypes = [vp, ip, ip, vp, vp, vp, ip, vp, ip, ip, ip, ip, ip, ip, vp, vp, vp, vp]
     lib.samrs_predict_multi.argtypes = PREDICT_MULTI_ARGTYPES
     lib.samrs_paint.argtypes = [vp, vp, vp, ip, ip, ip, vp, vp, vp, vp, ip, vp]
+    lib.samrs_predict_paint.argtypes = [vp, ip, ip, vp, vp, vp, ip, vp, ip, ip, ip, ip, vp, vp, vp, vp, vp, vp, vp, vp, ip, vp]
+    lib.samrs_predict_paint.restype = ip
     lib.samrs_debug_encoder_prefix.argtypes = [vp, vp, ip, ip, ip, ip, vp, vp]
     lib.samrs_debug_encoder_prefix.restype = ip
     lib.samrs_debug_time_dominant_kernel.argtypes = [vp, ip]
@@ -110,6 +112,8 @@
     lib.samrs_k_window_attention.argtypes = [ip, vp, vp, vp, vp, vp, ip, ip, ip, ip, ip, vp]
     lib.samrs_k_global_attention.argtypes = [ip, vp, vp, vp, vp, ip, ip, ip, ip, vp]
     lib.samrs_k_postprocess.argtypes = [vp, ip, ip, ip, ip, ip, ip, ip, vp, vp]
+    lib.samrs_k_threshold_paint.argtypes = [vp, ip, ip, ip, ip, vp, vp, vp, vp, vp]
+    lib.samrs_k_threshold_paint.restype = ip
     lib.samrs_k_neck_im2col.argtypes = [vp, vp, ip, ip, ip, vp]
     lib.samrs_k_neck_im2col.restype = ip
     lib.samrs_k_gemm_gln.argtypes = [ip, vp, vp, vp, vp, vp, ip, ip, ip, vp, vp, vp]
@@ -623,6 +627,30 @@
                                              areas.data_ptr(), _ptr(class_pixels), _ptr(class_instances), ncls, _stream()))
         return areas
 
+    def predict_paint(self, slot: int, boxes: torch.Tensor, labels: torch.Tensor, seg: torch.Tensor,
+                      input_size: Tuple[int, int], original_size: Tuple[int, int], class_pixels: Optional[torch.Tensor] = None,
+                      class_instances: Optional[torch.Tensor] = None, areas_out: Optional[torch.Tensor] = None):
+        dev = self.device
+        boxes, _, _, _, n = self._prompt_arrays(boxes, None, None, None)
+        if n < 1:
+            raise ValueError("empty prompt batch")
+        oh, ow = int(original_size[0]), int(original_size[1])
+        labels = labels.to(dtype=torch.int32, device=dev).contiguous()
+        assert labels.numel() == n and seg.dtype == torch.uint8 and seg.is_cuda and seg.is_contiguous() and seg.numel() == oh * ow
+        if areas_out is not None:
+            assert areas_out.dtype == torch.int64 and areas_out.is_contiguous() and areas_out.numel() == n and areas_out.is_cuda
+        areas = areas_out if areas_out is not None else torch.empty(n, dtype=torch.int64, device=dev)
+        masks = torch.empty(n, 1, oh, ow, dtype=torch.uint8, device=dev)
+        iou = torch.empty(n, 1, dtype=torch.float32, device=dev)
+        low = torch.empty(n, 1, 256, 256, dtype=torch.float32, device=dev)
+        ncls = 0 if class_pixels is None else class_pixels.numel()
+        with torch.cuda.device(dev):
+            self._check(self.lib.samrs_predict_paint(
+                self.handle, slot, n, boxes.data_ptr(), None, None, 0, None, int(input_size[0]), int(input_size[1]), oh, ow,
+                masks.data_ptr(), iou.data_ptr(), low.data_ptr(), labels.data_ptr(), seg.data_ptr(), areas.data_ptr(),
+                _ptr(class_pixels), _ptr(class_instances), ncls, _stream()))
+        return masks.view(torch.bool), iou, low, areas
+
     def _check_scene(self, rc: int) -> None:
         if rc == ERR_BAD_ARG:
             raise EngineError(self.lib.samrs_last_error(self.handle).decode())
```

Result: no change. 145.0 (median of 6 runs) (+0.7%).
